# r9y9/gantts

Hardware: AMD Instinct MI355X
Metric: acoustic frames/sec per G+D GAN step (B=32,T=512) (higher is better)
Workload: dtype f32; 1 GPU; cfg2: TTS acoustic MLP G 425-512x3-187 + conditioned MLP D 483-256x3-1, Adagrad, MGE+ADV loss, global B=32 T=512 (32 sequences per GPU, strong scaling), fp32, dropout 0.5 (Philox); global_batch=32, per_gpu_batch=32, parallelism=dp1

## Files before the change

gantts_amd/_lib.py:

```python
import ctypes as C
import os

import torch

_HERE = os.path.dirname(os.path.abspath(__file__))
LIB_PATH = os.environ.get("GT_HIP_LIB") or os.path.join(_HERE, "libgantts_hip.so")

GT_OK, GT_ERR_INVALID, GT_ERR_HIP, GT_ERR_STATE, GT_ERR_DIM = 0, 1, 2, 3, 4
ROLE_G, ROLE_D = 0, 1
OPT_LSTM_PERSISTENT, OPT_LSTM_FWD_UNITS, OPT_LSTM_XCD_LOCAL, OPT_MATMUL_BF16, OPT_SPLIT_FIRST_LAYER, OPT_FUSED_OPTIMIZER = 2, 3, 4, 5, 6, 7
OPT_SIDE_OVERLAP, OPT_LSTM_SIDE, OPT_COMM_D_ONE_MSG, OPT_COMM_EARLY_G, OPT_COMM_GROUP, OPT_COMM_FORCE = 8, 9, 10, 11, 12, 13
OPT_LAUNCH_RIDERS, OPT_COMM_CLOSE_INLINE, OPT_POLL_RESULTS = 14, 15, 16
OPT_COMM_TV_IN_SUMS, OPT_COMM_IPC, OPT_FUSED_DSTACK = 17, 18, 19
IPC_HANDLE_BYTES, IPC_MAX_WORLD = 64, 8
PROFILE_SLOTS = 16
LSTM_PATH_SLOTS, LSTM_PATH_STEPS, LSTM_PATH_DECLINED = 34, 32, 33
GEMM_PATH_SLOTS = 588
GEMM_ROUTE_FORWARD, GEMM_ROUTE_FORWARD_SEG, GEMM_ROUTE_BACKWARD_DATA, GEMM_ROUTE_WEIGHT_GRAD, GEMM_ROUTE_WEIGHT_GRAD_SPLIT = 0, 1, 2, 3, 4
ARCH_MLP, ARCH_IN2OUT, ARCH_LSTM, ARCH_SRU, ARCH_IN2OUT_RNN = 0, 1, 2, 3, 4
OPT_ADAGRAD, OPT_ADAM = 0, 1
MAX_STREAMS = 8
COMM_ID_BYTES = 128


class StreamConfig(C.Structure):
    _fields_ = [("n_streams", C.c_int32),
                ("stream_sizes", C.c_int32 * MAX_STREAMS),
                ("has_dynamic_features", C.c_int32 * MAX_STREAMS),
                ("num_windows", C.c_int32),
                ("adversarial_streams", C.c_int32 * MAX_STREAMS),
                ("mask_nth_mgc_for_adv_loss", C.c_int32),
                ("discriminator_linguistic_condition", C.c_int32),
                ("cond_dim", C.c_int32)]


class ModelDesc(C.Structure):
    _fields_ = [("arch", C.c_int32), ("in_dim", C.c_int32), ("out_dim", C.c_int32),
                ("num_hidden", C.c_int32), ("hidden_dim", C.c_int32), ("static_dim", C.c_int32),
                ("dropout", C.c_float), ("last_sigmoid", C.c_int32),
                ("bidirectional", C.c_int32), ("use_relu", C.c_int32),
                ("rnn_dropout", C.c_float), ("reserved_", C.c_int32),
                ("params", C.c_void_p), ("grads", C.c_void_p), ("n_params", C.c_int64)]


class OptimDesc(C.Structure):
    _fields_ = [("kind", C.c_int32), ("lr", C.c_float), ("weight_decay", C.c_float), ("eps", C.c_float),
                ("lr_decay", C.c_float), ("beta1", C.c_float), ("beta2", C.c_float),
                ("max_grad_norm", C.c_float), ("step", C.c_int64),
                ("state0", C.c_void_p), ("state1", C.c_void_p)]


class DResult(C.Structure):
    _fields_ = [("loss_d", C.c_float), ("loss_fake_d", C.c_float), ("loss_real_d", C.c_float),
                ("real_correct_count", C.c_float), ("fake_correct_count", C.c_float), ("grad_norm", C.c_float)]


class GResult(C.Structure):
    _fields_ = [("loss_mse", C.c_float), ("loss_mge", C.c_float), ("loss_adv", C.c_float),
                ("loss_g", C.c_float), ("grad_norm", C.c_float)]


class GemmCase(C.Structure):
    _fields_ = ([(n, C.c_int32) for n in ("route", "prec", "rows", "in_dim", "out_dim", "act", "drop")] + [("p", C.c_float)]
                + [("key0", C.c_uint32), ("key1", C.c_uint32)]
                + [(n, C.c_int32) for n in ("accumulate", "col0", "ncols", "wrap", "cd", "rider", "defer", "ldx", "ldw", "ldy", "ld_dy",
                                            "ldh", "ld_mask", "ld_addm", "ld_adv", "ld_dx")]
                + [(n, C.c_void_p) for n in ("x", "w", "bias", "y", "dy", "h", "mask", "addm", "adv", "dx", "dw", "db")])

# ... 131 lines not shown
```

gantts_amd/csrc/eng_core.hip:

```cpp
#include "engine_internal.hip.h"

using namespace gt;
static thread_local char g_err[512] = "";
int fail(int code, const char* fmt, ...) {
  va_list ap;
  va_start(ap, fmt);
  vsnprintf(g_err, sizeof(g_err), fmt, ap);
  va_end(ap);
  return code;
}
extern "C" const char* gt_last_error(void) { return g_err; }
extern "C" const char* gt_version(void) { return "gantts_hip 0.1 (gfx950, f32 MFMA)"; }

int ensure_dyn_lds(const void* kernel, size_t bytes) {
  static std::mutex mu;
  static std::map<std::pair<const void*, int>, size_t> done;
  int dev = 0;
  HIPCHK(hipGetDevice(&dev));
  std::lock_guard<std::mutex> lk(mu);
  size_t& cur = done[std::make_pair(kernel, dev)];
  if (bytes > cur) {
    HIPCHK(hipFuncSetAttribute(kernel, hipFuncAttributeMaxDynamicSharedMemorySize, (int)bytes));
    cur = bytes;
  }
  return GT_OK;
}

GemmProfiler g_prof;

extern "C" int gt_profile_enable(int on) {
  g_prof.on = on != 0;
  g_prof.only_kind = on >= 2 ? on - 2 : -1;
  return GT_OK;
}
extern "C" int gt_profile_read(double* out_ms, double* out_flops, int64_t* out_count) {
  for (int v = 0; v < GT_PROFILE_SLOTS; ++v) { out_ms[v] = 0; out_flops[v] = 0; out_count[v] = 0; g_prof.last_bytes[v] = 0; }
  for (auto& r : g_prof.recs) {
    if (hipEventSynchronize(r.e1) != hipSuccess) return fail(GT_ERR_HIP, "hipEventSynchronize failed");
    float ms = 0.f;
    if (hipEventElapsedTime(&ms, r.e0, r.e1) != hipSuccess) return fail(GT_ERR_HIP, "hipEventElapsedTime failed");
    int v = r.kind * 2 + (r.bn == 128 ? 1 : 0);
    if (r.kind == 5) v = 8;
    else if (r.kind == 6) v = 12;
    else if (r.kind == 7) v = 14;
    else if (r.kind == GEMM_NT && r.am == GEMM_A_NONE) v = 6;
    else if (r.kind == GEMM_NT && r.am == GEMM_A_LEAKY_PHILOX) v = 7;
    else if (r.kind == GEMM_NT && r.am == GEMM_A_LEAKY_PHILOX_ADDM) v = 9;
    else if (r.kind == GEMM_NT && r.am == GEMM_A_LEAKY_PHILOX_SEG) v = 13;
    else if (r.kind == GEMM_NN && r.am == GEMM_A_NONE) v = 10;
    else if (r.kind == GEMM_NN && r.am == GEMM_A_LEAKY_PHILOX) v = 11;
    if (v < 0 || v >= GT_PROFILE_SLOTS) v = GT_PROFILE_SLOTS - 1;
    out_ms[v] += ms; out_flops[v] += r.flops; out_count[v] += 1; g_prof.last_bytes[v] += r.bytes;
    g_prof.pool.push_back(r.e0); g_prof.pool.push_back(r.e1);
  }
  g_prof.recs.clear();
  return GT_OK;
}
extern "C" int gt_profile_bytes(double* out_bytes) {
  for (int v = 0; v < GT_PROFILE_SLOTS; ++v) out_bytes[v] = g_prof.last_bytes[v];
  return GT_OK;
}

static int upload_ints(const std::vector<int>& v, int** dptr) {
  if (*dptr) { (void)hipFree(*dptr); *dptr = nullptr; }
  if (v.empty()) return GT_OK;
  HIPCHK(hipMalloc((void**)dptr, v.size() * sizeof(int)));
  HIPCHK(hipMemcpy(*dptr, v.data(), v.size() * sizeof(int), hipMemcpyHostToDevice));
  return GT_OK;
}

extern "C" int gt_engine_create(const gt_stream_config* cfg, gt_engine** out) {
  if (!cfg || !out) return fail(GT_ERR_INVALID, "null argument");
  if (cfg->n_streams < 1 || cfg->n_streams > GT_MAX_STREAMS) return fail(GT_ERR_INVALID, "n_streams out of range");
  if (cfg->num_windows < 1 || cfg->num_windows > MLPG_MAXW) return fail(GT_ERR_INVALID, "num_windows must be in [1,%d]", MLPG_MAXW);
  gt_engine* e = new gt_engine();
  e->cfg = *cfg;
  int col = 0, scol_out = 0;
  std::vector<int> static_start, static_size;
  for (int s = 0; s < cfg->n_streams; ++s) {
    const int sz = cfg->stream_sizes[s];
    const bool dyn = cfg->has_dynamic_features[s] != 0;
    const int ss = dyn ? sz / cfg->num_windows : sz;
    static_start.push_back(scol_out);
    static_size.push_back(ss);
    for (int c = 0; c < ss; ++c) {
      e->h_scol.push_back(col + c);
      e->h_sstride.push_back(dyn ? ss : 0);
    }
    col += sz;
    scol_out += ss;
  }
  e->Dout_cfg = col;
  e->Ds = scol_out;
  if (cfg->adversarial_streams[0] < 0) {
    for (int c = 0; c < e->Ds; ++c) e->h_adv_cols.push_back(c);
  } else {
    for (int s = 0; s < cfg->n_streams; ++s)
      if (cfg->adversarial_streams[s])
        for (int c = 0; c < static_size[s]; ++c) e->h_adv_cols.push_back(static_start[s] + c);
    if (cfg->mask_nth_mgc_for_adv_loss > 0) {
      if ((size_t)cfg->mask_nth_mgc_for_adv_loss >= e->h_adv_cols.size()) { delete e; return fail(GT_ERR_INVALID, "mask_nth_mgc_for_adv_loss too large"); }
      e->h_adv_cols.erase(e->h_adv_cols.begin(), e->h_adv_cols.begin() + cfg->mask_nth_mgc_for_adv_loss);
    }
  }
  e->Da = (int)e->h_adv_cols.size();
  e->h_adv_inv.assign(e->Ds, -1);
  for (int j = 0; j < e->Da; ++j) e->h_adv_inv[e->h_adv_cols[j]] = j;
  int r;
// ... 197 lines not shown
  n.step = od->step;
  n.has_opt = true;
  return GT_OK;
}
extern "C" int gt_set_training(gt_engine* e, int role, int training) {
  if (!e || role < 0 || role > 1) return fail(GT_ERR_INVALID, "bad argument");
  e->net[role].training = training != 0;
  return GT_OK;
}
extern "C" int gt_set_lr(gt_engine* e, int role, float lr) {
  if (!e || role < 0 || role > 1 || !e->net[role].has_opt) return fail(GT_ERR_INVALID, "no optimizer bound");
  e->net[role].od.lr = lr;
  return GT_OK;
}
extern "C" int gt_get_optimizer_step(gt_engine* e, int role, int64_t* step) {
  if (!e || role < 0 || role > 1 || !step) return fail(GT_ERR_INVALID, "bad argument");
  *step = e->net[role].step;
  return GT_OK;
}
extern "C" int gt_set_seed(gt_engine* e, uint64_t seed) {
  if (!e) return fail(GT_ERR_INVALID, "null engine");
  e->seed = seed;
  e->step_counter = 0;
  return GT_OK;
}
extern "C" int gt_set_dropout_mask(gt_engine* e, int role, int pass, int layer, const float* mask) {
  if (!e || role < 0 || role > 1 || pass < 0 || pass > 2 || layer < 0 || layer > 15) return fail(GT_ERR_INVALID, "bad argument");
  e->net[role].inj[pass][layer] = mask;
  return GT_OK;
}
extern "C" int gt_set_option(gt_engine* e, int option, int value) {
  if (!e) return fail(GT_ERR_INVALID, "null engine");
  switch (option) {
    case GT_OPT_LSTM_PERSISTENT: e->lstm_persistent = value != 0; return GT_OK;
    case GT_OPT_LSTM_FWD_UNITS: e->lstm_fwd_upc = value; return GT_OK;
    case GT_OPT_LSTM_XCD_LOCAL: e->lstm_xcd_local = value != 0; return GT_OK;
    case GT_OPT_SPLIT_FIRST_LAYER:
      if (e->opt_split_first != (value != 0)) { e->fake_cat_valid = false; e->adv2_fake_ok = false; }
      e->opt_split_first = value != 0;
      return GT_OK;
    case GT_OPT_FUSED_OPTIMIZER: e->opt_fused_optimizer = value != 0; return GT_OK;
    case GT_OPT_SIDE_OVERLAP: e->opt_side_overlap = value != 0; return GT_OK;
    case GT_OPT_LSTM_SIDE: return value ? fail(GT_ERR_INVALID, "GT_OPT_LSTM_SIDE: removed in round 6 (measured: no gain); the value must be 0") : GT_OK;
    case GT_OPT_COMM_D_ONE_MSG: e->opt_comm_d_one_msg = value != 0; return GT_OK;
    case GT_OPT_COMM_EARLY_G: e->opt_comm_early_g = value != 0; return GT_OK;
    case GT_OPT_COMM_GROUP: e->opt_comm_group = value != 0; return GT_OK;
    case GT_OPT_COMM_FORCE: e->opt_comm_force = value != 0; return GT_OK;
    case GT_OPT_COMM_CLOSE_INLINE: e->opt_comm_close_inline = value != 0; return GT_OK;
    case GT_OPT_COMM_IPC: e->opt_comm_ipc = value != 0; return GT_OK;
    case GT_OPT_FUSED_DSTACK: e->opt_fused_dstack = value < 0 ? 0 : value > 2 ? 2 : value; return GT_OK;
    case GT_OPT_COMM_TV_IN_SUMS: e->opt_comm_tv_in_sums = value != 0; return GT_OK;
    case GT_OPT_POLL_RESULTS: e->opt_poll_results = value != 0; return GT_OK;
    case GT_OPT_LAUNCH_RIDERS: e->opt_launch_riders = value != 0; return GT_OK;
    case GT_OPT_MATMUL_BF16:
      if (e->matmul_bf16 != (value != 0)) {
        e->g_pass_valid = false; e->fake_cat_valid = false; e->dcat_b_ok = false; e->adv2_fake_ok = false; e->leak_pending = false; e->cxd_src = nullptr;
        e->d_begin_done = false; e->g_begin_done = false;
      }
      e->matmul_bf16 = value != 0;
      return GT_OK;
  }
  return fail(GT_ERR_INVALID, "unknown option %d", option);
}
GtTuning& gt_tuning() {
  static GtTuning t = [] {
    GtTuning v;
    auto geti = [](const char* n, int d) { const char* s = getenv(n); return s && s[0] ? atoi(s) : d; };
    v.gemm_pair = geti("GT_GEMM_PAIR", v.gemm_pair); v.pair_order = geti("GT_PAIR_ORDER", v.pair_order);
    { const char* s = getenv("GT_GEMM_TILES"); v.gemm_tiles_big = s && !strcmp(s, "big") ? 1 : 0; }
    v.gemm_unaligned = geti("GT_GEMM_UNALIGNED", v.gemm_unaligned); v.tn_wgs = geti("GT_TN_WGS", v.tn_wgs); v.tn_split_wgs = geti("GT_TN_SPLIT_WGS", v.tn_split_wgs); v.split_fused = geti("GT_SPLIT_FUSED", v.split_fused);
    v.b16_tiles = geti("GT_B16_TILES", v.b16_tiles); v.b16_wg_tile = geti("GT_B16_WG_TILE", v.b16_wg_tile); v.b16_dma = geti("GT_B16_DMA", v.b16_dma);
    v.mlpg_fpl = geti("GT_MLPG_FPL", v.mlpg_fpl); v.mlpg_tt = geti("GT_MLPG_TT", v.mlpg_tt); v.sru_lw = geti("GT_SRU_LW", v.sru_lw); v.sru_cs_waves = geti("GT_SRU_CS_WAVES", v.sru_cs_waves); v.leak_rider = geti("GT_LEAK_RIDER", v.leak_rider);
    v.head_vec = geti("GT_HEAD_VEC", v.head_vec);
    v.mlpg_small16 = geti("GT_MLPG_SMALL16", v.mlpg_small16);
    v.lstm_bt = geti("GT_LSTM_BT", v.lstm_bt);
    if (v.lstm_bt != 8 && v.lstm_bt != 16) v.lstm_bt = 0;
    return v;
  }();
  return t;
}
extern "C" int gt_set_tuning(const char* name, int value) {
  if (!name) return fail(GT_ERR_INVALID, "null name");
  GtTuning& t = gt_tuning();
  struct { const char* n; int* p; } tab[] = {
      {"gemm_pair", &t.gemm_pair}, {"pair_order", &t.pair_order}, {"gemm_tiles_big", &t.gemm_tiles_big}, {"gemm_unaligned", &t.gemm_unaligned},
      {"tn_wgs", &t.tn_wgs}, {"tn_split_wgs", &t.tn_split_wgs}, {"split_fused", &t.split_fused}, {"b16_tiles", &t.b16_tiles},
      {"b16_wg_tile", &t.b16_wg_tile}, {"b16_dma", &t.b16_dma}, {"mlpg_fpl", &t.mlpg_fpl}, {"mlpg_tt", &t.mlpg_tt}, {"sru_lw", &t.sru_lw}, {"sru_cs_waves", &t.sru_cs_waves}, {"leak_rider", &t.leak_rider}, {"head_vec", &t.head_vec}, {"mlpg_small16", &t.mlpg_small16}};
  if (!strcmp(name, "lstm_bt")) {
    if (value != 0 && value != 8 && value != 16) return fail(GT_ERR_INVALID, "lstm_bt must be 0 (by shape), 8 or 16, not %d", value);
    t.lstm_bt = value;
    return GT_OK;
  }
  for (auto& e : tab) if (!strcmp(e.n, name)) { *e.p = value; return GT_OK; }
  return fail(GT_ERR_INVALID, "unknown tuning knob '%s'", name);
}
extern "C" int gt_set_x_pitch(gt_engine* e, int ld_generator_input, int ld_condition) {
  if (!e || ld_generator_input < 0 || ld_condition < 0) return fail(GT_ERR_INVALID, "bad argument");
  e->ld_gx = ld_generator_input; e->ld_cx = ld_condition;
  return GT_OK;
}
extern "C" int gt_set_loss_normalizer(gt_engine* e, float tv) {
  if (!e) return fail(GT_ERR_INVALID, "null engine");
  e->tv_override = tv;
  e->tv_dev = nullptr;
  return GT_OK;
}
// ... 87 lines not shown
    return d;
  }
  return philox_site_spec(e, role, pass, layer, e->step_counter, n.d.dropout, half_rows);
}

extern "C" int gt_op_philox_mask(gt_engine* e, int role, int pass, int layer, int64_t steps_ahead, float p, int64_t rows, int cols,
                                 float* mask, void* stream) {
  if (!e || !mask || role < 0 || role > 1 || pass < 0 || pass > 2 || layer < 0 || layer > 15 || rows < 1 || cols < 1 ||
      steps_ahead < 0 || !(p > 0.f && p < 1.f) || rows > 0x7fffffffL)
    return fail(GT_ERR_INVALID, "bad argument");
  const DropoutSpec d = philox_site_spec(e, role, pass, layer, e->step_counter + (uint64_t)steps_ahead, p,
                                         rows == 2L * e->chk_B * e->chk_T ? (long)e->chk_B * e->chk_T : 0L);
  hipLaunchKernelGGL(philox_mask_kernel, dim3(cdiv(rows * cols, 256)), dim3(256), 0, (hipStream_t)stream, d, rows, cols, mask);
  LAUNCH_CHECK();
  return GT_OK;
}

int fault_seen(gt_engine* e) {
  const unsigned int f = e->h_fault ? (e->h_fault[0] | e->h_fault[1]) : 0u;
  if (f & 0xffu)
    return fail(GT_ERR_HIP, "persistent LSTM kernel fault %u: a workgroup timed out waiting for its peers (results of that "
                "step are invalid and its optimizer updates were skipped; gt_clear_faults() re-arms the engine, "
                "GT_OPT_LSTM_PERSISTENT=0 / GT_LSTM_STEPS=1 selects the per-step kernels)", f);
  if (f) return fail(GT_ERR_HIP, "device fault word 0x%x: results of that step are invalid", f);
  return GT_OK;
}
extern "C" int gt_clear_faults(gt_engine* e, void* stream) {
  if (!e) return fail(GT_ERR_INVALID, "null engine");
  HIPCHK(hipStreamSynchronize((hipStream_t)stream));
  HIPCHK(hipDeviceSynchronize());
  HIPCHK(hipMemset(e->d_fault, 0, 64));
  if (e->opt_bar.p) { HIPCHK(hipMemset(e->opt_bar.p, 0, 64)); e->opt_bar_count = 0; }
  for (int r = 0; r < 2; ++r) { e->net[r].step -= (long)e->h_fault[2 + r]; if (e->net[r].step < 0) e->net[r].step = 0; }
  for (int i = 0; i < 4; ++i) e->h_fault[i] = 0;
  e->g_pass_valid = false; e->leak_pending = false; e->fake_cat_valid = false; e->adv2_fake_ok = false; e->cxd_src = nullptr;
  e->d_begin_done = e->g_begin_done = false; e->early_done = false;
  return GT_OK;
}
extern "C" int gt_lstm_path_counts(gt_engine* e, int64_t* counts, int reset) {
  if (!e) return fail(GT_ERR_INVALID, "null engine");
  if (counts) memcpy(counts, e->lstm_paths, sizeof(e->lstm_paths));
  if (reset) memset(e->lstm_paths, 0, sizeof(e->lstm_paths));
  return GT_OK;
}
extern "C" int gt_check_faults(gt_engine* e, void* stream) {
  if (!e) return fail(GT_ERR_INVALID, "null engine");
  HIPCHK(hipMemcpyAsync(e->h_fault, e->d_fault, sizeof(unsigned int), hipMemcpyDeviceToHost, (hipStream_t)stream));
  HIPCHK(hipStreamSynchronize((hipStream_t)stream));
  return fault_seen(e);
}
int check_common(gt_engine* e, int B, int T) {
  if (!e) return fail(GT_ERR_INVALID, "null engine");
  tl_gemm_prec = e->matmul_bf16 ? PREC_BF16 : PREC_F32;
  if (B < 1 || T < 1) return fail(GT_ERR_INVALID, "B and T must be positive");
  if ((long)B * T > 0x3fffffffL) return fail(GT_ERR_INVALID, "B*T too large");
  e->chk_B = B; e->chk_T = T;
  return GT_OK;
}
```

gantts_amd/csrc/eng_gemm_f32.hip:

```cpp
#include "engine_internal.hip.h"
#include <atomic>

using namespace gt;
int launch_gemm_nt(const GemmArgs& g, int bm, int bn, hipStream_t s);
int launch_gemm_nn(const GemmArgs& g, int bm, int bn, hipStream_t s);
int launch_gemm_tn(const GemmArgs& g, int bm, int bn, int nslab, hipStream_t s);
int launch_gemm_pair(const GemmArgs& nn_in, const GemmArgs& tn_in, int nslab, hipStream_t s);
int launch_gemm_tn_pair(const GemmArgs& g1_in, const GemmArgs& g2_in, int nslab1, int nslab2, hipStream_t s, const GemmArgs* rider, bool* rode);
int gemm_cu_count() {
  static std::map<int, int> cus;
  int dev = 0;
  if (hipGetDevice(&dev) != hipSuccess) return 256;
  auto it = cus.find(dev);
  if (it != cus.end()) return it->second;
  hipDeviceProp_t prop;
  const int n = hipGetDeviceProperties(&prop, dev) == hipSuccess ? prop.multiProcessorCount : 256;
  cus[dev] = n;
  return n;
}
thread_local int tl_gemm_prec = PREC_F32;

static std::atomic<int64_t> g_gemm_paths[GT_GEMM_PATH_SLOTS];
void gemm_path_count(int slot) { g_gemm_paths[slot].fetch_add(1, std::memory_order_relaxed); }
extern "C" int gt_gemm_path_counts(int64_t* counts, int reset) {
  for (int i = 0; i < GT_GEMM_PATH_SLOTS; ++i) {
    const int64_t v = reset ? g_gemm_paths[i].exchange(0, std::memory_order_relaxed) : g_gemm_paths[i].load(std::memory_order_relaxed);
    if (counts) counts[i] = v;
  }
  return GT_OK;
}

static int pick_bn(int N) { return (cdiv(N, 64) * 64 < cdiv(N, 128) * 128) ? 64 : 128; }

static int gemm_tile_mode() { return gt_tuning().gemm_tiles_big; }
static bool gemm_unaligned_ok() { return gt_tuning().gemm_unaligned != 0; }
bool gemm_vec_ok(const float* p, int ld, bool k_contiguous) {
  if (k_contiguous && gemm_unaligned_ok()) return true;
  return (ld % 4 == 0) && (((uintptr_t)p) % 16 == 0);
}
bool gemm_wide_store_ok(int kind, const GemmArgs& g) {
  if (kind == GEMM_TN) return false;
  if (gemm_unaligned_ok()) return true;
  return (g.ldc % 4 == 0) && (((uintptr_t)g.C) % 16 == 0) &&
         (kind != GEMM_NN || g.act == ACT_NONE || ((g.ldh % 4 == 0) && (((uintptr_t)g.H) % 16 == 0)));
}
bool gemm_small_tiles_ok() { return gemm_tile_mode() == 0; }


int launch_gemm(int kind, const GemmArgs& g, int nslab, hipStream_t s) {
  if (g.M <= 0 || g.N <= 0 || g.K <= 0) return fail(GT_ERR_INVALID, "empty GEMM");
  const int bn = pick_bn(g.N);
  const bool vec = gemm_vec_ok(g.A, g.lda, kind != GEMM_TN) && gemm_vec_ok(g.B, g.ldb, kind == GEMM_NT);
  if (kind != GEMM_TN && vec && g.M > 64 && gemm_small_tiles_ok())
    return kind == GEMM_NT ? launch_gemm_nt(g, 64, 64, s) : launch_gemm_nn(g, 64, 64, s);
  bool small = false;
  if (kind != GEMM_TN && g.M > 64) {
    const long t128 = (long)cdiv(g.M, 128) * cdiv(g.N, bn), t64 = (long)cdiv(g.M, 64) * cdiv(g.N, bn);
    const double c128 = (double)cdiv(t128, 512), c64 = 0.55 * (double)cdiv(t64, bn == 64 ? 1024 : 768);
    small = c64 < c128;
  }
  switch (kind) {
    case GEMM_NT:
      if (small) return bn == 64 ? launch_gemm_nt(g, 64, 64, s) : launch_gemm_nt(g, 64, 128, s);
      return bn == 64 ? launch_gemm_nt(g, 128, 64, s) : launch_gemm_nt(g, 128, 128, s);
    case GEMM_NN:
      if (small) return bn == 64 ? launch_gemm_nn(g, 64, 64, s) : launch_gemm_nn(g, 64, 128, s);
      return bn == 64 ? launch_gemm_nn(g, 128, 64, s) : launch_gemm_nn(g, 128, 128, s);
    default:
      if (g.n_tiles_m == 64) return launch_gemm_tn(g, 64, 64, nslab, s);
      return bn == 64 ? launch_gemm_tn(g, 128, 64, nslab, s) : launch_gemm_tn(g, 128, 128, nslab, s);
  }
}

// ... 211 lines not shown
```

gantts_amd/csrc/eng_gemm_f32_pair.hip:

```cpp
#include "gemm_f32_launch.hip.h"

int launch_gemm_pair(const GemmArgs& nn_in, const GemmArgs& tn_in, int nslab, hipStream_t s) {
  GemmArgs nn = nn_in, tn = tn_in;
  nn.wide_store = gemm_wide_store_ok(GEMM_NN, nn) ? 1 : 0;
  tn.wide_store = 0;
  nn.n_tiles_m = cdiv(nn.M, 64); nn.n_tiles_n = cdiv(nn.N, 64);
  tn.n_tiles_m = cdiv(tn.M, 64); tn.n_tiles_n = cdiv(tn.N, 64);
  const int n1 = nn.n_tiles_m * nn.n_tiles_n, n2 = tn.n_tiles_m * tn.n_tiles_n * nslab;
  const bool bf16 = tl_gemm_prec == PREC_BF16;
  const size_t lds = bf16 ? std::max(gemm_lds_bytes<GEMM_NN, 64, 64, PREC_BF16>(), gemm_lds_bytes<GEMM_TN, 64, 64, PREC_BF16>())
                          : std::max(gemm_lds_bytes<GEMM_NN, 64, 64>(), gemm_lds_bytes<GEMM_TN, 64, 64>());
  const int am = bf16 ? GEMM_A_RUNTIME : (nn.act == ACT_NONE ? GEMM_A_NONE : ((nn.act == ACT_LEAKY_DROPOUT && nn.drop.mode == DROP_PHILOX) ? GEMM_A_LEAKY_PHILOX : GEMM_A_RUNTIME));
  const void* kern = bf16 ? (const void*)gemm_pair_kernel<PREC_BF16> : (am == GEMM_A_NONE ? (const void*)gemm_pair_kernel<PREC_F32, GEMM_A_NONE> :
                     (am == GEMM_A_LEAKY_PHILOX ? (const void*)gemm_pair_kernel<PREC_F32, GEMM_A_LEAKY_PHILOX> : (const void*)gemm_pair_kernel<PREC_F32>));
  CHK(ensure_dyn_lds(kern, lds));
  GemmProfiler::Rec rec;
  if (g_prof.wants(5)) {
    rec.kind = 5; rec.bn = 64; rec.am = -1; rec.flops = 2.0 * nn.M * nn.N * nn.K + 2.0 * tn.M * tn.N * tn.K;
    rec.bytes = gemm_algorithmic_bytes(GEMM_NN, nn) + gemm_algorithmic_bytes(GEMM_TN, tn);
    rec.e0 = g_prof.get(); rec.e1 = g_prof.get();
    HIPCHK(hipEventRecord(rec.e0, s));
  }
  const int tn_first = gt_tuning().pair_order;
  const int grid = n1 + n2;
  gemm_path_count(GEMM_PATH_PAIR + (bf16 ? 3 : am == GEMM_A_NONE ? 0 : am == GEMM_A_LEAKY_PHILOX ? 1 : 2));
  if (bf16) hipLaunchKernelGGL(gemm_pair_kernel<PREC_BF16>, dim3(grid), dim3(GEMM_THREADS), lds, s, nn, tn, n1, tn_first);
  else if (am == GEMM_A_NONE) hipLaunchKernelGGL((gemm_pair_kernel<PREC_F32, GEMM_A_NONE>), dim3(grid), dim3(GEMM_THREADS), lds, s, nn, tn, n1, tn_first);
  else if (am == GEMM_A_LEAKY_PHILOX) hipLaunchKernelGGL((gemm_pair_kernel<PREC_F32, GEMM_A_LEAKY_PHILOX>), dim3(grid), dim3(GEMM_THREADS), lds, s, nn, tn, n1, tn_first);
  else      hipLaunchKernelGGL(gemm_pair_kernel<PREC_F32>, dim3(grid), dim3(GEMM_THREADS), lds, s, nn, tn, n1, tn_first);
  LAUNCH_CHECK();
  if (g_prof.wants(5)) { HIPCHK(hipEventRecord(rec.e1, s)); g_prof.recs.push_back(rec); }
  return GT_OK;
}

int launch_gemm_tn_pair(const GemmArgs& g1_in, const GemmArgs& g2_in, int nslab1, int nslab2, hipStream_t s, const GemmArgs* rider, bool* rode) {
  GemmArgs g1 = g1_in, g2 = g2_in, g3;
  memset(&g3, 0, sizeof(g3));
  int n3 = 0;
  if (rode) *rode = false;
  if (rider && rider->act == ACT_NONE && !rider->accumulate && rider->M > 0 && gemm_vec_ok(rider->A, rider->lda, true) && tl_gemm_prec == PREC_F32 &&
      gemm_small_tiles_ok()) {
    g3 = *rider;
    g3.wide_store = gemm_wide_store_ok(GEMM_NN, g3) ? 1 : 0;
    g3.n_tiles_m = cdiv(g3.M, 64); g3.n_tiles_n = cdiv(g3.N, 64);
    n3 = g3.n_tiles_m * g3.n_tiles_n;
    if (rode) *rode = true;
  }
  g1.wide_store = g2.wide_store = 0;
  g1.n_tiles_m = cdiv(g1.M, 64); g1.n_tiles_n = cdiv(g1.N, 64);
  g2.n_tiles_m = cdiv(g2.M, 64); g2.n_tiles_n = cdiv(g2.N, 64);
  const int n1 = g1.n_tiles_m * g1.n_tiles_n * nslab1, n2 = g2.n_tiles_m * g2.n_tiles_n * nslab2;
  const size_t lds = std::max(gemm_lds_bytes<GEMM_TN, 64, 64>(), gemm_lds_bytes<GEMM_NN, 64, 64>());
  CHK(ensure_dyn_lds((const void*)gemm_tn_pair_kernel<PREC_F32>, lds));
  GemmProfiler::Rec rec;
  if (g_prof.wants(6)) {
    rec.kind = 6; rec.bn = 64; rec.am = -1; rec.flops = 2.0 * g1.M * g1.N * g1.K + 2.0 * g2.M * g2.N * g2.K + (n3 ? 2.0 * g3.M * g3.N * g3.K : 0.0);
    rec.bytes = gemm_algorithmic_bytes(GEMM_TN, g1) + 4.0 * (double)g1.M * g1.K + gemm_algorithmic_bytes(GEMM_TN, g2) + (n3 ? gemm_algorithmic_bytes(GEMM_NN, g3) : 0.0);
    rec.e0 = g_prof.get(); rec.e1 = g_prof.get();
    HIPCHK(hipEventRecord(rec.e0, s));
  }
  gemm_path_count(GEMM_PATH_TN_PAIR + (n3 > 0 ? 1 : 0));
  hipLaunchKernelGGL(gemm_tn_pair_kernel<PREC_F32>, dim3(n1 + n2 + n3), dim3(GEMM_THREADS), lds, s, g1, g2, n1, g3, n3);
  LAUNCH_CHECK();
  if (g_prof.wants(6)) { HIPCHK(hipEventRecord(rec.e1, s)); g_prof.recs.push_back(rec); }
  return GT_OK;
}
```

gantts_amd/csrc/eng_step.hip:

```cpp
#include "engine_internal.hip.h"
#include "dstack_f32.hip.h"

using namespace gt;
int ensure_band(gt_engine* e, const float* R, int T, hipStream_t s) {
  MlpgCache& m = e->mlpg;
  ++m.tick;
  for (auto* b : m.entries)
    if (b->R == R && b->T == T) { b->last_use = m.tick; m.cur = b; return GT_OK; }
  const int nW = e->cfg.num_windows;
  CHK(m.tmp.ensure((size_t)(2 * T - 1) * sizeof(float)));
  hipLaunchKernelGGL(mlpg_offset_max_kernel, dim3(2 * T - 1), dim3(256), 0, s, R, T, nW, m.tmp.as<float>());
  LAUNCH_CHECK();
  std::vector<float> off(2 * T - 1);
  HIPCHK(hipMemcpyAsync(off.data(), m.tmp.p, off.size() * sizeof(float), hipMemcpyDeviceToHost, s));
  HIPCHK(hipStreamSynchronize(s));
  float peak = 0.f;
  for (float v : off) peak = fmaxf(peak, v);
  if (!(peak > 0.f) || !isfinite(peak)) return fail(GT_ERR_INVALID, "MLPG matrix R is empty or not finite");
  int kb = 0;
  for (int o = -(T - 1); o <= T - 1; ++o)
    if (off[o + T - 1] > 1e-9f * peak) kb = std::max(kb, abs(o));
  if (kb > 63 || (kb > 48 && kb > T / 4))
    return fail(GT_ERR_INVALID, "MLPG matrix R is not banded (half-width %d of T=%d): only window sets whose "
                "R = (W^T W)^-1 W^T decays (hparams.py:22-26) are supported", kb, T);
// ... 12 lines not shown
  CHK(b->band.ensure((size_t)T * nW * nb * sizeof(float)));
  hipLaunchKernelGGL(mlpg_extract_band_kernel, dim3(cdiv((long)T * nW * nb, 256)), dim3(256), 0, s, R, T, nW, kb, b->band.as<float>());
  LAUNCH_CHECK();
  b->R = R; b->T = T; b->kb = kb; b->last_use = m.tick;
  m.cur = b;
  return GT_OK;
}
extern "C" int gt_invalidate_mlpg_cache(gt_engine* e) {
  if (!e) return fail(GT_ERR_INVALID, "null engine");
  HIPCHK(hipDeviceSynchronize());
  e->mlpg.clear();
  return GT_OK;
}

static int mlpg_tile_frames(gt_engine* e, int B, int T) {
  (void)e;
  const int tt = gt_tuning().mlpg_tt;
  if (tt == 16) return 16;
  if (tt == 0 && gt_tuning().mlpg_small16 && (long)B * cdiv(T, 32) * 2 <= gemm_cu_count()) return 16;
  return 32;
}
int mlpg_forward(gt_engine* e, const float* y, int ldy, const int* scol, const int* sstride, int Ds,
                 float* ys, int ldys, int B, int T, hipStream_t s) {
  const int nW = e->cfg.num_windows, kb = e->mlpg.cur->kb;
  auto lds_of = [&](int tt) { return ((size_t)(tt + 2 * kb) * nW * MLPG_CC + (size_t)tt * nW * (2 * kb + 1 + 2 * MLPG_PAD)) * sizeof(float); };
  const int tt = mlpg_tile_frames(e, B, T);
  const size_t lds = lds_of(tt);
  dim3 grid(B * cdiv(T, tt), cdiv(Ds, MLPG_CC));
  const int fpl = gt_tuning().mlpg_fpl;
#define GT_MLPG_FWD(F, TTV) { CHK(ensure_dyn_lds((const void*)mlpg_forward_kernel<F, TTV>, lds)); \
    hipLaunchKernelGGL((mlpg_forward_kernel<F, TTV>), grid, dim3(MLPG_THREADS), lds, s, y, ldy, e->mlpg.cur->band.as<float>(), kb, nW, scol, sstride, Ds, ys, ldys, B, T); }
  if (tt == 16) GT_MLPG_FWD(2, 16)
  else { if (fpl == 1) GT_MLPG_FWD(1, 32) else if (fpl == 2) GT_MLPG_FWD(2, 32) else GT_MLPG_FWD(4, 32) }
#undef GT_MLPG_FWD
  LAUNCH_CHECK();
  return GT_OK;
}
int mlpg_backward(gt_engine* e, const float* gs, int ldgs, const int* scol, const int* sstride, int Ds,
                  float* gy, int ldgy, int B, int T, float mse_w, const float* yhat, const float* ytgt, int ldt,
                  const float* mask, hipStream_t s) {
  const int nW = e->cfg.num_windows, kb = e->mlpg.cur->kb;
  auto lds_of = [&](int tt) { return ((size_t)(tt + 2 * kb) * MLPG_CC + (size_t)(tt + 2 * kb) * nW * (2 * kb + 1 + 2 * MLPG_PAD)) * sizeof(float); };
  const int tt = mlpg_tile_frames(e, B, T);
  const size_t lds = lds_of(tt);
  dim3 grid(B * cdiv(T, tt), cdiv(Ds, MLPG_CC));
  const int fpl = gt_tuning().mlpg_fpl;
#define GT_MLPG_BWD(F, TTV) { CHK(ensure_dyn_lds((const void*)mlpg_backward_kernel<F, TTV>, lds)); \
    hipLaunchKernelGGL((mlpg_backward_kernel<F, TTV>), grid, dim3(MLPG_THREADS), lds, s, gs, ldgs, e->mlpg.cur->band.as<float>(), kb, nW, scol, sstride, Ds, \
                       gy, ldgy, B, T, mse_w, yhat, ytgt, ldt, mask, e->sc()); }
  if (tt == 16) GT_MLPG_BWD(2, 16)
  else { if (fpl == 1) GT_MLPG_BWD(1, 32) else if (fpl == 2) GT_MLPG_BWD(2, 32) else GT_MLPG_BWD(4, 32) }
#undef GT_MLPG_BWD
  LAUNCH_CHECK();
  return GT_OK;
}

static int stage_injected(gt_engine* e, int role, int layer, const int* passes, int npass, long rows_each, int width,
                          const float** out, hipStream_t s) {
  Net& n = e->net[role];
  *out = nullptr;
  if (!n.training || n.d.dropout <= 0.f) return GT_OK;
  bool any = false, all = true;
  for (int i = 0; i < npass; ++i) { any |= n.inj[passes[i]][layer] != nullptr; all &= n.inj[passes[i]][layer] != nullptr; }
  if (!any) return GT_OK;
  if (!all) return fail(GT_ERR_INVALID, "injected dropout masks must be given for every pass of a step or for none");
  if (npass == 1) { *out = n.inj[passes[0]][layer]; return GT_OK; }
  const size_t per_layer = (size_t)npass * rows_each * width * sizeof(float);
  CHK(e->dmask.ensure(per_layer * n.d.num_hidden));
  float* base = (float*)((char*)e->dmask.p + per_layer * layer);
  for (int i = 0; i < npass; ++i)
    HIPCHK(hipMemcpyAsync(base + (size_t)i * rows_each * width, n.inj[passes[i]][layer], (size_t)rows_each * width * sizeof(float),
                          hipMemcpyDeviceToDevice, s));
  *out = base;
  return GT_OK;
}

struct FirstSplit {
  const float* x; int ldx; int cd;
  const float* xp; int ldxp;
  const float* adv; int ld_adv;
  long wrap;
};
static int pitched_rows(gt_engine* e, int slot, const float* p, int ld, int cols, long rows, const float** out, int* ldo, hipStream_t s) {
  if (gemm_vec_ok(p, ld)) { *out = p; *ldo = ld; return GT_OK; }
  gt_engine::Pitched& P = e->pitched[slot];
  const int ldp = (cols + 3) & ~3;
  if (!(P.src == p && P.ld == ld && P.cols == cols && P.rows == rows && P.step == e->step_counter)) {
    CHK(P.buf.ensure((size_t)rows * ldp * sizeof(float)));
    hipLaunchKernelGGL(repitch_kernel, dim3(cdiv(rows * (ldp / 4), 256)), dim3(256), 0, s, p, ld, cols, rows, P.buf.as<float>(), ldp);
    LAUNCH_CHECK();
    P.src = p; P.ld = ld; P.cols = cols; P.rows = rows; P.step = e->step_counter;
  }
  *out = P.buf.as<float>(); *ldo = ldp;
  return GT_OK;
}

static int stack_forward(gt_engine* e, int role, const float* in, int ld_in, long rows, std::vector<Scratch>& acts,
                         const int* passes, int npass, long rows_each, std::vector<DropoutSpec>& specs, hipStream_t s,
                         const FirstSplit* fs = nullptr, int max_layers = 1 << 30 ) {
  Net& n = e->net[role];
  specs.resize(n.hidden.size());
  const float* cur = in;
  int ld = ld_in;
  for (size_t l = 0; l < n.hidden.size(); ++l) {
    const Lin& L = n.hidden[l];
    CHK(acts[l].ensure((size_t)rows * L.out * sizeof(float)));
// ... 277 lines not shown
      hipLaunchKernelGGL(gather_cols_kernel, dim3(cdiv(N * G.d.out_dim, 256)), dim3(256), 0, s, y_hat, G.d.out_dim, 0,
                         (const int*)nullptr, y_hat_static, G.d.out_dim, 0, (int)N, G.d.out_dim);
      LAUNCH_CHECK();
    }
  }
  return GT_OK;
}

extern "C" int gt_apply_generator(gt_engine* e, const float* x, const float* R, int B, int T, float* y_hat,
                                  float* y_hat_static, void* stream) {
  CHK(check_common(e, B, T));
  Net& G = e->net[GT_ROLE_G];
  if (!G.bound) return fail(GT_ERR_STATE, "generator not bound");
  if (!x || !y_hat || !y_hat_static) return fail(GT_ERR_INVALID, "null tensor");
  hipStream_t s = (hipStream_t)stream;
  CHK(fault_seen(e));
  e->step_counter++;
  e->B = B; e->T = T; e->N = (long)B * T;
  e->g_pass_valid = false;
  e->fake_cat_valid = false; e->dcat_b_ok = false; e->adv2_fake_ok = false; e->cxd_src = nullptr;
  e->tv_mask = nullptr; e->tv_inflight = false;
  CHK(generator_forward(e, x, R, B, T, y_hat, y_hat_static, true, s, e->g_specs));
  e->last_x = e->gx_dense_on ? e->gx_dense.as<float>() : x;
  e->last_yhat = y_hat; e->last_yhs = y_hat_static;
  e->g_pass_valid = true;
  return GT_OK;
}

int cond_dim(gt_engine* e) {
  if (!e->cfg.discriminator_linguistic_condition) return 0;
  if (e->cfg.cond_dim > 0) return e->cfg.cond_dim;
  return e->net[GT_ROLE_D].bound ? e->net[GT_ROLE_D].d.in_dim - e->Da : 0;
}
static int d_in_dim(gt_engine* e) { return e->Da + cond_dim(e); }

static int build_cat(gt_engine* e, const float* x, const float* feats, int ld_feats, long row0, long N, int ldc, hipStream_t s) {
  float* dst = e->dcat.as<float>() + row0 * ldc;
  int off = 0;
  if (e->cfg.discriminator_linguistic_condition) {
    if (!x) return fail(GT_ERR_INVALID, "discriminator_linguistic_condition is set but x is null");
    const int cd = cond_dim(e);
    if (cd <= 0) return fail(GT_ERR_DIM, "discriminator in_dim too small for linguistic conditioning");
    hipLaunchKernelGGL(gather_cols_kernel, dim3(cdiv(N * cd, 256)), dim3(256), 0, s, x, cd, 0, (const int*)nullptr, dst, ldc, 0,
                       (int)N, cd);
    LAUNCH_CHECK();
    off = cd;
  }
  hipLaunchKernelGGL(gather_cols_kernel, dim3(cdiv(N * e->Da, 256)), dim3(256), 0, s, feats, ld_feats, 0, e->d_adv_cols, dst, ldc,
                     off, (int)N, e->Da);
  LAUNCH_CHECK();
  return GT_OK;
}

static int head_finalize(gt_engine* e, int mode, int nblk, int K, bool w, hipStream_t s, StepResults* early_res, int* defer_scalars, unsigned ticket) {
  Net& D = e->net[GT_ROLE_D];
  if (defer_scalars && !w) { *defer_scalars = nblk; return GT_OK; }
  const int cgw = (w && nblk >= 512) ? 16 : 64;
  const int n_dw = cdiv(K, cgw), extra = cgw == 16 ? 1 : 0;
  hipLaunchKernelGGL(d_head_finalize_kernel, dim3(n_dw + extra), dim3(1024), 0, s, e->headp.as<HeadPartials>(), e->headw.as<float>(),
                     nblk, K, mode, e->sc(), w ? D.last.dW : (float*)nullptr, w ? D.last.db : (float*)nullptr, D.grads_dirty ? 1 : 0,
                     early_res, ticket ? e->ticket_dev() : (unsigned*)nullptr, ticket, cgw, extra ? n_dw : 0);
  LAUNCH_CHECK();
  return GT_OK;
}

static bool d_fused_ok(gt_engine* e, bool b16, long rows) {
  Net& D = e->net[GT_ROLE_D];
  if (e->opt_fused_dstack < 2 && dstack_panels(rows) < gemm_cu_count()) return false;
  if (!e->opt_fused_dstack || b16 || D.d.arch != GT_ARCH_MLP || tl_gemm_prec != PREC_F32 || !dstack_hidden_ok(D.d.hidden_dim)) return false;
  if (D.hidden.empty() || (int)D.hidden.size() > DS_MAXL || D.last.out != 1 || e->Da < 1 || e->Da > 64) return false;
  for (size_t l = 0; l < D.hidden.size(); ++l)
    if (D.hidden[l].out != D.d.hidden_dim || (l > 0 && D.hidden[l].in != D.d.hidden_dim)) return false;
  return true;
}
static int run_dstack(gt_engine* e, int mode, long rows, long n_real, const float* mask, long n_mask, float eps, bool want_grad,
                      float* gadv, hipStream_t s, StepResults* early_res, int* defer_scalars, const double* tv_dev, unsigned ticket, bool unit_tv) {
  Net& D = e->net[GT_ROLE_D];
  const int H = D.d.hidden_dim, L = (int)D.hidden.size();
  const int nblk = dstack_panels(rows);
  CHK(e->headp.ensure((size_t)nblk * sizeof(HeadPartials)));
  CHK(e->dout.ensure((size_t)rows * sizeof(float)));
  DStackArgs a;
  memset(&a, 0, sizeof(a));
  a.mode = mode; a.L = L; a.rows = (int)rows; a.n_real = (int)n_real;
  a.H0 = e->d_act[0].as<float>();
  for (int l = 0; l < L; ++l) {
    a.W[l] = D.hidden[l].W; a.b[l] = D.hidden[l].b; a.drop[l] = e->d_specs[l];
    if (a.drop[l].mode == DROP_BUFFER && a.drop[l].ld_mask != H) return fail(GT_ERR_INVALID, "injected dropout mask pitch");
  }
  a.w_last = D.last.W; a.b_last = D.last.b; a.mask = mask; a.n_mask = (int)n_mask; a.eps = eps; a.unit_tv = unit_tv ? 1 : 0; a.tv_dev = tv_dev;
  a.sc = e->sc(); a.want_grad = want_grad ? 1 : 0; a.Dout = e->dout.as<float>(); a.hp = e->headp.as<HeadPartials>();
  if (mode == DSTACK_D_STEP) {
    for (int l = 1; l + 1 < L; ++l) a.Hout[l] = e->d_act[l].as<float>();
    a.dZtop = e->dzA.as<float>();
    if (want_grad) { CHK(e->headw.ensure((size_t)nblk * H * sizeof(float))); a.dw_partial = e->headw.as<float>(); }
  } else {
    a.W0 = D.hidden[0].W; a.ldw0 = D.hidden[0].in; a.col0 = cond_dim(e); a.Da = e->Da; a.gadv = gadv; a.ld_gadv = e->Da;
    if (want_grad && !gadv) return fail(GT_ERR_INVALID, "fused discriminator stack: no gradient buffer");
  }
  CHK(launch_dstack(a, H, s));
  return head_finalize(e, mode == DSTACK_D_STEP ? HEAD_D_STEP : HEAD_G_ADV, nblk, H, mode == DSTACK_D_STEP && want_grad, s, early_res, defer_scalars, ticket);
}

static int run_head(gt_engine* e, int mode, const void* H, int K, long n_rows, long n_real, const float* mask, long n_mask,
                    float eps, bool want_grad, float* dH, const DropoutSpec& spec, bool want_w, hipStream_t s,
                    StepResults* early_res = nullptr, int h_ld = 0, B16Img* dz_img = nullptr, bool dz_t = false,
                    int* defer_scalars = nullptr ,
                    const double* tv_dev = nullptr ,
                    unsigned ticket = 0 ,
                    bool unit_tv = false ,
                    bool has_act = true ) {
// ... 276 lines not shown
  CHK(e->dzA.ensure((size_t)2 * N * std::max(H, 1) * sizeof(float)));
  CHK(e->dzB.ensure((size_t)2 * N * std::max(H, 1) * sizeof(float)));
  const bool plain_early = e->early && !comm_on(e), comm_early = e->early && comm_on(e);
  if (tv_side) CHK(side_join(e, s));
  const unsigned d_ticket = plain_early ? take_ticket(e) : 0;
  const double* head_tv = nullptr;
  if (unnorm) {
    e->tv_mask = mask; e->tv_n = N; e->tv_ovr = e->tv_override;
  } else if (comm_on(e) && e->opt_launch_riders && e->tv_inflight && !tv_known) {
    CHK(comm_tv_join(e, s));
    head_tv = e->comm_tv.as<double>();
    e->tv_mask = mask; e->tv_n = N; e->tv_ovr = e->tv_override;
  } else CHK(ensure_tv(e, mask, N, s));
  if (b16 && tr) CHK(e->dz_b[0].ensure(2 * N, H, true));
  if (d_rec)
    CHK(run_head(e, HEAD_D_STEP, (const void*)rec_top, H, 2 * N, N, mask, N, eps, tr, e->dl_dout.as<float>(), no_drop(), true, s,
                 plain_early ? early_res_target(e) : nullptr, 0, nullptr, true, nullptr, head_tv, d_ticket, unnorm, false));
  else if (fused)
    CHK(run_dstack(e, DSTACK_D_STEP, 2 * N, N, mask, N, eps, tr, nullptr, s, plain_early ? early_res_target(e) : nullptr, nullptr, head_tv, d_ticket, unnorm));
  else
  CHK(run_head(e, HEAD_D_STEP, b16 ? (const void*)e->d_actb.back().r() : (const void*)e->d_act.back().as<float>(), H, 2 * N, N, mask, N, eps, tr,
               e->dzA.as<float>(), e->d_specs.back(), true, s, plain_early ? early_res_target(e) : nullptr, b16 ? e->d_actb.back().ld : 0,
               (b16 && tr) ? &e->dz_b[0] : nullptr, true, nullptr, head_tv, d_ticket, unnorm));
  e->early_done = false;
  if (plain_early) CHK(post_early_results(e, s, d_ticket));
  if (comm_early) CHK(comm_early_results(e, GT_ROLE_D, unnorm ? &e->sc()->tv_sum : &e->sc()->s_real, unnorm ? 5 : 4, 0.f, 0.f, 0.f, s));
  if (tr) {
    CHK(comm_grads_ready(e, GT_ROLE_D, D.last.dW, (long)D.last.in * D.last.out + D.last.out, s));
    Net& G = e->net[GT_ROLE_G];
    const bool want_leak = G.bound && G.d.grads && e->g_pass_valid && y_hat_static == e->last_yhs && e->N == N;
    if (want_leak && e->leak_pending)
      return fail(GT_ERR_STATE, "update_discriminator called twice without optimizer_g.zero_grad() (train.py:538)");
    float* leak = nullptr;
    if (want_leak) { CHK(e->leak.ensure((size_t)N * e->Da * sizeof(float))); leak = e->leak.as<float>(); }
    const int col0 = cond_dim(e);
    if (d_rec) {
      float* dx0 = nullptr;
      if (leak) { CHK(e->d_dx0.ensure((size_t)2 * N * K0 * sizeof(float))); dx0 = e->d_dx0.as<float>(); }
      CHK(lstm_stack_backward(e, GT_ROLE_D, e->dcat.as<float>(), ldc, 2 * B, T, passes, 2, true, dx0, s));
      if (leak) {
        hipLaunchKernelGGL(gather_cols_kernel, dim3(cdiv(N * e->Da, 256)), dim3(256), 0, s, dx0 + N * K0, K0, col0, (const int*)nullptr, leak, e->Da, 0,
                           (int)N, e->Da);
        LAUNCH_CHECK();
      }
    } else if (b16) {
      CHK(stack_backward_b16(e, GT_ROLE_D, e->dcat_b.t(), e->dcat_b.ldt, 2 * N, e->d_actb, e->d_specs, 0, true, leak, e->Da, col0, e->Da, N, N, s));
    } else {
      CHK(stack_backward(e, GT_ROLE_D, split ? nullptr : e->dcat.as<float>(), ldc, 2 * N, e->d_act, e->d_specs, e->dzA.as<float>(),
                         e->dzB.as<float>(), true, leak, e->Da, col0, e->Da, N, N, s, split ? &fs : nullptr));
    }
    D.grads_dirty = true;
    if (want_leak) { e->leak_pending = true; e->leak_unnorm = unnorm; }
  }
  CHK(comm_finish_step(e, GT_ROLE_D, tr, &e->sc()->s_real, comm_early ? 0 : 4, s));
  e->d_begin_done = true;
  return GT_OK;
}

static void fill_d_result(const StepResults* h, gt_d_result* out) {
  out->loss_d = h->loss_d; out->loss_fake_d = h->loss_fake_d; out->loss_real_d = h->loss_real_d;
  out->real_correct_count = h->real_correct; out->fake_correct_count = h->fake_correct;
  out->grad_norm = h->gnorm_d;
}
static void fill_g_result(const StepResults* h, gt_g_result* out) {
  out->loss_mse = h->loss_mse; out->loss_mge = h->loss_mge; out->loss_adv = h->loss_adv;
  out->loss_g = h->loss_g; out->grad_norm = h->gnorm_g;
}

extern "C" int gt_update_discriminator_end(gt_engine* e, int train, gt_d_result* out, void* stream) {
  if (!e) return fail(GT_ERR_INVALID, "null argument");
  if (!e->d_begin_done) return fail(GT_ERR_STATE, "gt_update_discriminator_end without _begin");
  hipStream_t s = (hipStream_t)stream;
  e->d_begin_done = false;
  if (!out) {
    if (e->early_done) return fail(GT_ERR_STATE, "deferred results are a split-phase feature");
    if (train) CHK(optimizer_step(e, GT_ROLE_D, &e->sc()->gnorm2_d, s));
    hipLaunchKernelGGL(finalize_d_kernel, dim3(1), dim3(1), 0, s, e->sc(), e->res(), train ? 0 : 1);
    LAUNCH_CHECK();
    return post_deferred_results(e, GT_ROLE_D, s);
  }
  if (e->early_done) {
    if (train) CHK(optimizer_step(e, GT_ROLE_D, &e->sc()->gnorm2_d, s));
    CHK(wait_early_results(e));
    e->early_done = false;
  } else {
    if (train) CHK(optimizer_step(e, GT_ROLE_D, &e->sc()->gnorm2_d, s));
    hipLaunchKernelGGL(finalize_d_kernel, dim3(1), dim3(1), 0, s, e->sc(), e->res(), train ? 0 : 1);
    LAUNCH_CHECK();
    CHK(fetch_results(e, s));
  }
  fill_d_result(e->h_res, out);
  return GT_OK;
}
extern "C" int gt_update_discriminator_result(gt_engine* e, gt_d_result* out) {
  if (!e || !out) return fail(GT_ERR_INVALID, "null argument");
  if (!e->def_pending[GT_ROLE_D]) return fail(GT_ERR_STATE, "no deferred discriminator result pending");
  HIPCHK(hipEventSynchronize(e->ev_def[GT_ROLE_D]));
  e->def_pending[GT_ROLE_D] = false;
  fill_d_result(e->h_def[GT_ROLE_D], out);
  return GT_OK;
}

extern "C" int gt_update_discriminator(gt_engine* e, const float* x, const float* y_static, const float* y_hat_static,
                                       const float* mask, int B, int T, int train, float eps, gt_d_result* out, void* stream) {
  if (!e) return fail(GT_ERR_INVALID, "null engine");
  e->early = true;
  int r = gt_update_discriminator_begin(e, x, y_static, y_hat_static, mask, B, T, train, eps, stream);
  e->early = false;
  if (r != GT_OK) { e->early_done = false; e->d_unnorm = false; e->ticket_wait = 0; return r; }
  return gt_update_discriminator_end(e, train, out, stream);
}

static int sum_sqerr(gt_engine* e, const float* a, int lda, const float* b, int ldb, const float* mask, long rows, int D,
                     double* out, float* g, int ldg, float gscale, hipStream_t s, int* deferred_blocks = nullptr) {
  const int nblk = (int)std::min<long>(1024, cdiv(rows * D, RED_THREADS * 4));
  CHK(e->partial.ensure(4096 * sizeof(double)));
  double* part = e->partial.as<double>() + 1024;
  hipLaunchKernelGGL(masked_sqerr_kernel, dim3(nblk), dim3(RED_THREADS), 0, s, a, lda, b, ldb, mask, rows, D, part, g, ldg, gscale, e->sc());
  LAUNCH_CHECK();
  if (deferred_blocks) { *deferred_blocks = nblk; return GT_OK; }
  hipLaunchKernelGGL(sum_partials_kernel, dim3(1), dim3(256), 0, s, part, nblk, out);
  LAUNCH_CHECK();
  return GT_OK;
}

static int generator_backward(gt_engine* e, const float* x, const float* y, const float* y_hat, const float* mask,
                              float mse_w, hipStream_t s) {
  Net& G = e->net[GT_ROLE_G];
  const long N = e->N;
  const int B = e->B, T = e->T, Do = G.d.out_dim;
  const bool mlp_body = !(has_lstm_body(G.d.arch) || G.d.arch == GT_ARCH_SRU);
  const int ldgy = mlp_body && (is_i2o(G.d.arch) || e->g_used_mlpg) ? (Do + 3) & ~3 : Do;
  CHK(e->gy.ensure((size_t)N * ldgy * sizeof(float)));
  float* gy = e->gy.as<float>();
  const float* gs = e->gs.as<float>();
  if (is_i2o(G.d.arch)) {
    const int sd = G.d.static_dim;
    if (G.d.arch == GT_ARCH_IN2OUT_RNN) mse_w = 0.f;
    CHK(e->dgx.ensure((size_t)N * sd * sizeof(float)));
    CHK(e->dtz.ensure((size_t)N * sd * sizeof(float)));
    hipLaunchKernelGGL(highway_backward_kernel, dim3(cdiv(N * sd, 256)), dim3(256), 0, s, gs, sd, e->tx.as<float>(), sd,
                       e->gx.as<float>(), sd, e->dgx.as<float>(), sd, e->dtz.as<float>(), sd, N, sd);
    LAUNCH_CHECK();
    CHK(linear_backward_weight(e->dtz.as<float>(), sd, x, G.d.in_dim, N, sd, sd, G.gate.dW, G.gate.db, G.grads_dirty, e->slabs,
                               e->colp, s, &e->sdefer[GT_ROLE_G]));
    CHK(comm_grads_ready(e, GT_ROLE_G, G.gate.dW, (long)sd * sd + sd, s));
    CHK(mlpg_backward(e, e->dgx.as<float>(), sd, e->d_scol_i2o, e->d_sstride_i2o, sd, gy, ldgy, B, T, mse_w, y_hat, y, Do, mask, s));
  } else if (e->g_used_mlpg) {
    CHK(mlpg_backward(e, gs, e->Ds, e->d_scol, e->d_sstride, e->Ds, gy, ldgy, B, T, mse_w, y_hat, y, Do, mask, s));
  } else {
    if (mse_w != 0.f) CHK(sum_sqerr(e, y_hat, Do, y, Do, mask, N, Do, &e->sc()->s_mse, gy, Do, mse_w, s));
    hipLaunchKernelGGL(slab_reduce_kernel, dim3(cdiv(N * Do, 256)), dim3(256), 0, s, gs, 0L, 1, N * Do, gy, mse_w != 0.f ? 1 : 0);
    LAUNCH_CHECK();
  }
  if (G.d.last_sigmoid && !is_i2o(G.d.arch)) {
    hipLaunchKernelGGL(sigmoid_grad_kernel, dim3(cdiv(N * Do, 256)), dim3(256), 0, s, gy, ldgy, y_hat, Do, N, Do);
    LAUNCH_CHECK();
  }
  if (has_lstm_body(G.d.arch) || G.d.arch == GT_ARCH_SRU) {
    CHK(has_lstm_body(G.d.arch) ? lstm_backward(e, x, gy, B, T, s) : sru_backward(e, x, gy, B, T, s));
    G.grads_dirty = true;
    return GT_OK;
  }
  if (use_b16(e, GT_ROLE_G)) {
    const int H = G.d.hidden_dim;
    CHK(e->gy_b.ensure(N, Do, true));
    CHK(cast_transpose(gy, ldgy, N, Do, e->gy_b.r(), e->gy_b.ld, e->gy_b.t(), e->gy_b.ldt, nullptr, false, &e->colp, s));
    B16Img& top = e->g_actb.back();
    CHK(weight_grad_b16(e->gy_b.t(), e->gy_b.ldt, top.t(), top.ldt, N, Do, G.last.in, G.last.dW, G.last.db, G.grads_dirty, e->slabs, s,
                        &e->sdefer[GT_ROLE_G]));
    CHK(comm_grads_ready(e, GT_ROLE_G, G.last.dW, (long)Do * G.last.in + Do, s));
    const LinShadow& ws = e->wsh[GT_ROLE_G][G.hidden.size()];
    CHK(e->dz_b[0].ensure(N, H, true));
    GemmB16Args g = b16_args();
    g.A = e->gy_b.r(); g.lda = e->gy_b.ld; g.B = ws.wt.as<__bf16>(); g.ldb = ws.ldwt; g.M = (int)N; g.N = H; g.K = Do;
    g.epi = B16_BWD_DATA; g.act = ACT_LEAKY_DROPOUT; g.H = top.r(); g.ldh = top.ld; g.drop = e->g_specs.back();
    g.Cb = e->dz_b[0].r(); g.ldcb = e->dz_b[0].ld; g.CbT = e->dz_b[0].t(); g.ldcbt = (int)e->dz_b[0].ldt;
    CHK(launch_gemm_b16(g, 1, s));
    CHK(stack_backward_b16(e, GT_ROLE_G, e->xin_b.t(), e->xin_b.ldt, N, e->g_actb, e->g_specs, 0, true, nullptr, 0, 0, 0, 0, 0, s));
    G.grads_dirty = true;
    return GT_OK;
  }
  const Lin& Lt = G.hidden.back();
  const int H = G.d.hidden_dim;
  CHK(e->dzA.ensure((size_t)2 * N * H * sizeof(float)));
  CHK(e->dzB.ensure((size_t)2 * N * H * sizeof(float)));
  const GemmArgs nn_last = backward_data_args(gy, ldgy, G.last.W, G.last.in, 0, e->dzA.as<float>(), H, N, Do, H, ACT_LEAKY_DROPOUT,
                                              e->g_act.back().as<float>(), H, e->g_specs.back());
  bool rode = false;
  CHK(linear_backward_weight(gy, ldgy, e->g_act.back().as<float>(), Lt.out, N, Do, G.last.in, G.last.dW, G.last.db, G.grads_dirty,
                             e->slabs, e->colp, s, &e->sdefer[GT_ROLE_G], &nn_last, &rode));
  CHK(comm_grads_ready(e, GT_ROLE_G, G.last.dW, (long)Do * G.last.in + Do, s));
  if (!rode) CHK(launch_gemm(GEMM_NN, nn_last, 1, s));
  const float* xin = x;
  int ldxin = gx_pitch(e);
  if (!gemm_vec_ok(x, ldxin) && tl_gemm_prec == PREC_F32) {
    if (e->fake_cat_valid && e->fake_cat_x == x && e->cfg.discriminator_linguistic_condition && cond_dim(e) == G.d.in_dim && e->dcat.p) {
      ldxin = (d_in_dim(e) + 3) & ~3;
      xin = e->dcat.as<float>() + N * ldxin;
    } else {
      const int slot = (e->pitched[0].src == x && e->pitched[0].ld == gx_pitch(e) && e->pitched[0].cols == G.d.in_dim && e->pitched[0].step == e->step_counter) ? 0 : 1;
      CHK(pitched_rows(e, slot, x, gx_pitch(e), G.d.in_dim, N, &xin, &ldxin, s));
    }
  }
  CHK(stack_backward(e, GT_ROLE_G, xin, ldxin, N, e->g_act, e->g_specs, e->dzA.as<float>(), e->dzB.as<float>(), true,
                     nullptr, 0, 0, 0, 0, 0, s));
  G.grads_dirty = true;
  return GT_OK;
}

extern "C" int gt_update_generator_begin(gt_engine* e, const float* x, const float* y, const float* y_hat, const float* y_static,
                                         const float* y_hat_static, float adv_w, const float* mask, int B, int T, int train,
                                         float mse_w, float mge_w, float eps, void* stream) {
  CHK(check_common(e, B, T));
  Net& G = e->net[GT_ROLE_G];
  Net& D = e->net[GT_ROLE_D];
  if (!G.bound) return fail(GT_ERR_STATE, "generator not bound");
  if (!y || !y_hat || !y_static || !y_hat_static || !mask) return fail(GT_ERR_INVALID, "null tensor");
  hipStream_t s = (hipStream_t)stream;
  const long N = (long)B * T;
  const bool tr = train != 0;
  if (tr) {
    if (!e->g_pass_valid || y_hat != e->last_yhat || y_hat_static != e->last_yhs || N != e->N)
      return fail(GT_ERR_STATE, "update_generator(phase=\"train\") needs the y_hat / y_hat_static returned by the last apply_generator");
    if (!G.d.grads) return fail(GT_ERR_STATE, "phase == \"train\" but the generator was bound without grads");
  }
  const int Do = G.d.out_dim;
  const int Ds = is_i2o(G.d.arch) ? G.d.static_dim : e->Ds;
  if (comm_on(e) && tr && G.grads_dirty)
    return fail(GT_ERR_STATE, "data-parallel step: optimizer_g.zero_grad() must precede update_generator");
  { SlabDefer& sd = e->sdefer[GT_ROLE_G]; sd.jobs.n = 0; sd.blocks = 0; sd.used = 0; sd.active = e->early && tr && G.has_opt; }
  CHK(ensure_tv(e, mask, N, s));
  const bool direct = !is_i2o(G.d.arch) && !e->g_used_mlpg;
  const bool early_fold = e->early && !comm_on(e) && !(tr && direct && mse_w != 0.f);
  int mse_blocks = 0, mge_pre_blocks = 0;
  const bool mse_side = early_fold && e->opt_side_overlap && adv_w > 0.f;
  const bool riders = early_fold && e->opt_launch_riders && !mse_side;
  const bool riders_dp = e->early && comm_on(e) && e->opt_launch_riders && !(tr && direct && mse_w != 0.f);
  if (riders || riders_dp) {
    mse_blocks = (int)std::min<long>(1024, cdiv(N * Do, RED_THREADS * 4));
    mge_pre_blocks = (int)std::min<long>(1024, cdiv(N * Ds, RED_THREADS * 4));
    CHK(e->partial.ensure(4096 * sizeof(double)));
    hipLaunchKernelGGL(g_losses_kernel, dim3(mse_blocks + mge_pre_blocks), dim3(RED_THREADS), 0, s, y_hat, Do, y, Do, Do, mse_blocks,
                       e->partial.as<double>() + 1024, y_hat_static, Ds, y_static, Ds, Ds, e->partial.as<double>(), mask, N);
    LAUNCH_CHECK();
  } else if (!(tr && direct && mse_w != 0.f)) {
    if (mse_side) CHK(side_fork(e, s));
    CHK(sum_sqerr(e, y_hat, Do, y, Do, mask, N, Do, &e->sc()->s_mse, nullptr, 0, 0.f, mse_side ? e->side : s, early_fold ? &mse_blocks : nullptr));
  }
  e->g_has_adv = adv_w > 0.f;
  float* gadv = nullptr;
  int head_blocks = 0;
  if (adv_w > 0.f) {
    if (!D.bound) return fail(GT_ERR_STATE, "adv_w > 0 but no discriminator bound");
    if (D.d.in_dim != d_in_dim(e)) return fail(GT_ERR_DIM, "discriminator in_dim mismatch");
    const int K0 = D.d.in_dim, ldc = (K0 + 3) & ~3;
    const int passes[1] = {2};
    const bool b16 = use_b16(e, GT_ROLE_D);
    const float* cat = nullptr;
    const bool split = d_split_ok(e, x, b16);
    if (!split) CHK(dense_cx(e, &x, N, s));
    FirstSplit fs;
    memset(&fs, 0, sizeof(fs));
    if (split) {
      e->ld_adv2 = (e->Da + 3) & ~3;
      CHK(e->adv2.ensure((size_t)2 * N * e->ld_adv2 * sizeof(float)));
      float* fake = e->adv2.as<float>() + N * e->ld_adv2;
      if (!(e->adv2_fake_ok && e->adv2_yhs == y_hat_static)) {
        hipLaunchKernelGGL(build_adv_kernel, dim3(cdiv(N * (e->ld_adv2 / 4), 256)), dim3(256), 0, s, y_hat_static, y_hat_static, Ds, e->d_adv_cols, e->Da,
                           fake, e->ld_adv2, N, N, (const float*)nullptr, 0, 0.f, (StepScalars*)nullptr, (double*)nullptr);
        LAUNCH_CHECK();
        e->adv2_fake_ok = true; e->adv2_yhs = y_hat_static;
      }
      fs.x = x; fs.ldx = cx_pitch(e); fs.cd = cond_dim(e); fs.adv = fake; fs.ld_adv = e->ld_adv2; fs.wrap = N;
    } else if (!b16) {
      CHK(e->dcat.ensure((size_t)2 * N * ldc * sizeof(float)));
      if (!(e->fake_cat_valid && e->fake_cat_x == x && e->fake_cat_yhs == y_hat_static)) {
        CHK(build_cat(e, x, y_hat_static, Ds, N, N, ldc, s));
        e->fake_cat_valid = true; e->fake_cat_x = x; e->fake_cat_yhs = y_hat_static;
      }
      cat = e->dcat.as<float>() + N * ldc;
    }
    const bool d_rec = has_lstm_body(D.d.arch);
    const bool fused = !d_rec && d_fused_ok(e, b16, N);
    const float* rec_top = nullptr;
    int rec_ld = 0;
    if (d_rec) {
      CHK(lstm_check_lengths(e, B, T));
      CHK(lstm_stack_forward(e, GT_ROLE_D, cat, ldc, B, T, passes, 1, s, &rec_top, &rec_ld));
    } else
    if (b16) {
      CHK(e->dcat_b.ensure(2 * N, K0, false));
      if (!(e->dcat_b_ok && e->dcat_b_x == x && e->dcat_b_yhs == y_hat_static)) {
        if (e->cfg.discriminator_linguistic_condition && (!x || cond_dim(e) <= 0))
          return fail(GT_ERR_INVALID, "discriminator_linguistic_condition is set but x is null");
        CatSrc src;
        src.x = x; src.cd = cond_dim(e); src.fa = y_hat_static; src.fb = y_hat_static; src.ldf = Ds; src.idx = e->d_adv_cols; src.N = N; src.row_off = N;
        hipLaunchKernelGGL(cat_cast_transpose_kernel, dim3(cdiv(N, 64), cdiv(K0, 64)), dim3(256), 0, s, src, N, K0,
                           e->dcat_b.r() + N * e->dcat_b.ld, e->dcat_b.ld, (__bf16*)nullptr, 0L);
        LAUNCH_CHECK();
        e->dcat_b_ok = true; e->dcat_b_x = x; e->dcat_b_yhs = y_hat_static;
      }
      CHK(refresh_shadows(e, GT_ROLE_D, false, s));
      CHK(stack_forward_b16(e, GT_ROLE_D, e->dcat_b.r() + N * e->dcat_b.ld, e->dcat_b.ld, N, e->d_actb, passes, 1, N, e->d_specs, false, s));
    } else {
      CHK(stack_forward(e, GT_ROLE_D, cat, ldc, N, e->d_act, passes, 1, N, e->d_specs, s, split ? &fs : nullptr, fused ? 1 : 1 << 30));
    }
    const int H = d_rec ? rec_ld : D.d.hidden_dim;
    CHK(e->dzA.ensure((size_t)2 * N * H * sizeof(float)));
    CHK(e->dzB.ensure((size_t)2 * N * H * sizeof(float)));
    if (b16 && tr) CHK(e->dz_b[0].ensure(N, H, false));
    if (fused) {
      if (tr) { CHK(e->gadv.ensure((size_t)N * e->Da * sizeof(float))); gadv = e->gadv.as<float>(); }
      CHK(run_dstack(e, DSTACK_G_ADV, N, N, mask, N, eps, tr, gadv, s, nullptr, riders || riders_dp ? &head_blocks : nullptr, nullptr, 0, false));
    } else
    if (d_rec) {
      CHK(e->dl_dout.ensure((size_t)2 * N * H * sizeof(float)));
      CHK(run_head(e, HEAD_G_ADV, (const void*)rec_top, H, N, N, mask, N, eps, tr, e->dl_dout.as<float>(), no_drop(), false, s, nullptr, 0, nullptr,
                   false, riders || riders_dp ? &head_blocks : nullptr, nullptr, 0, false, false));
    } else
    CHK(run_head(e, HEAD_G_ADV, b16 ? (const void*)e->d_actb.back().r() : (const void*)e->d_act.back().as<float>(), H, N, N, mask, N, eps, tr,
                 e->dzA.as<float>(), e->d_specs.back(), false, s, nullptr, b16 ? e->d_actb.back().ld : 0, (b16 && tr) ? &e->dz_b[0] : nullptr, false,
                 riders || riders_dp ? &head_blocks : nullptr));
    if (tr && !fused) {
      CHK(e->gadv.ensure((size_t)N * e->Da * sizeof(float)));
      gadv = e->gadv.as<float>();
      const int col0 = cond_dim(e);
      if (d_rec) {
        CHK(e->d_dx0.ensure((size_t)2 * N * K0 * sizeof(float)));
        float* dx0 = e->d_dx0.as<float>();
        CHK(lstm_stack_backward(e, GT_ROLE_D, cat, ldc, B, T, passes, 1, false, dx0, s));
        hipLaunchKernelGGL(gather_cols_kernel, dim3(cdiv(N * e->Da, 256)), dim3(256), 0, s, dx0, K0, col0, (const int*)nullptr, gadv, e->Da, 0, (int)N,
                           e->Da);
        LAUNCH_CHECK();
      } else if (b16) {
        CHK(stack_backward_b16(e, GT_ROLE_D, nullptr, 0, N, e->d_actb, e->d_specs, 0, false, gadv, e->Da, col0, e->Da, 0, N, s));
      } else {
        CHK(stack_backward(e, GT_ROLE_D, cat, ldc, N, e->d_act, e->d_specs, e->dzA.as<float>(), e->dzB.as<float>(), false, gadv,
                           e->Da, col0, e->Da, 0, N, s));
      }
    }
  }
  const bool early_ok = e->early && !(tr && direct && mse_w != 0.f);
  const bool early_now = early_ok && !comm_on(e), comm_early = early_ok && comm_on(e) && e->opt_comm_early_g;
  int mge_blocks = 0;
  e->early_done = false;
  {
    const int nblk = (int)std::min<long>(1024, cdiv(N * Ds, RED_THREADS * 4));
    CHK(e->partial.ensure(4096 * sizeof(double)));
    float* gs = nullptr;
    if (tr) { CHK(e->gs.ensure((size_t)N * Ds * sizeof(float))); gs = e->gs.as<float>(); }
    const float* leak = (tr && e->leak_pending) ? e->leak.as<float>() : nullptr;
    GFinalize fin;
    memset(&fin, 0, sizeof(fin));
    const bool rid = riders || riders_dp;
    if (rid) {
      fin.on = 1; fin.sc = e->sc(); fin.out = riders ? early_res_target(e) : (StepResults*)nullptr; fin.adv_w = adv_w; fin.mse_w = mse_w; fin.mge_w = mge_w;
      fin.has_adv = e->g_has_adv ? 1 : 0;
      fin.part_mge = e->partial.as<double>(); fin.n_mge = mge_pre_blocks;
      fin.part_mse = e->partial.as<double>() + 1024; fin.n_mse = mse_blocks;
      fin.hp = head_blocks ? e->headp.as<HeadPartials>() : (const HeadPartials*)nullptr; fin.n_hp = head_blocks;
      if (riders) { fin.ticket_value = take_ticket(e); fin.ticket = fin.ticket_value ? e->ticket_dev() : (unsigned*)nullptr; }
    }
    if (tr || !rid)
      hipLaunchKernelGGL(static_grad_kernel, dim3(nblk + (rid ? 1 : 0)), dim3(RED_THREADS), 0, s, y_hat_static, Ds,
                         y_static, Ds, mask, N, Ds, mge_w, e->d_adv_inv, leak, e->Da, gadv, e->Da, adv_w, gs, Ds,
                         rid ? (double*)nullptr : e->partial.as<double>(), e->sc(), fin, leak && e->leak_unnorm ? 1 : 0);
    else
      hipLaunchKernelGGL(finalize_g_rider_kernel, dim3(1), dim3(RED_THREADS), 0, s, fin);
    LAUNCH_CHECK();
    mge_blocks = nblk;
    if (riders) CHK(post_early_results(e, s, fin.ticket_value));
    else if (!early_now && !riders_dp) {
      hipLaunchKernelGGL(sum_partials_kernel, dim3(1), dim3(256), 0, s, e->partial.as<double>(), nblk, &e->sc()->s_mge);
      LAUNCH_CHECK();
    }
  }
  if (mse_side && mse_blocks) CHK(side_join(e, s));
  if (early_now && !riders) {
    hipLaunchKernelGGL(finalize_g_kernel, dim3(1), dim3(256), 0, s, e->sc(), early_res_target(e), adv_w, mse_w, mge_w, e->g_has_adv ? 1 : 0, 1,
                       (const double*)e->partial.as<double>(), mge_blocks,
                       mse_blocks ? (const double*)(e->partial.as<double>() + 1024) : (const double*)nullptr, mse_blocks);
    LAUNCH_CHECK();
    CHK(post_early_results(e, s));
  }
  if (comm_early) CHK(comm_early_results(e, GT_ROLE_G, &e->sc()->s_adv, 3, adv_w, mse_w, mge_w, s));
  if (tr) {
    CHK(generator_backward(e, e->last_x, y, y_hat, mask, mse_w, s));
    e->leak_pending = false; e->leak_unnorm = false;
  }
  CHK(comm_finish_step(e, GT_ROLE_G, tr, &e->sc()->s_adv, comm_early ? 0 : 3, s));
  e->g_begin_done = true;
  return GT_OK;
}

extern "C" int gt_update_generator_end(gt_engine* e, int train, float adv_w, float mse_w, float mge_w, gt_g_result* out,
                                       void* stream) {
  if (!e) return fail(GT_ERR_INVALID, "null argument");
  if (!e->g_begin_done) return fail(GT_ERR_STATE, "gt_update_generator_end without _begin");
  hipStream_t s = (hipStream_t)stream;
  e->g_begin_done = false;
  if (!out) {
    if (e->early_done) return fail(GT_ERR_STATE, "deferred results are a split-phase feature");
    if (train) CHK(optimizer_step(e, GT_ROLE_G, &e->sc()->gnorm2_g, s));
    hipLaunchKernelGGL(finalize_g_kernel, dim3(1), dim3(1), 0, s, e->sc(), e->res(), adv_w, mse_w, mge_w, e->g_has_adv ? 1 : 0,
                       train ? 0 : 1, (const double*)nullptr, 0, (const double*)nullptr, 0);
    LAUNCH_CHECK();
    return post_deferred_results(e, GT_ROLE_G, s);
  }
  if (e->early_done) {
    if (train) CHK(optimizer_step(e, GT_ROLE_G, &e->sc()->gnorm2_g, s));
    CHK(wait_early_results(e));
    e->early_done = false;
  } else {
    if (train) CHK(optimizer_step(e, GT_ROLE_G, &e->sc()->gnorm2_g, s));
    hipLaunchKernelGGL(finalize_g_kernel, dim3(1), dim3(1), 0, s, e->sc(), e->res(), adv_w, mse_w, mge_w, e->g_has_adv ? 1 : 0,
                       train ? 0 : 1, (const double*)nullptr, 0, (const double*)nullptr, 0);
    LAUNCH_CHECK();
    CHK(fetch_results(e, s));
  }
  fill_g_result(e->h_res, out);
  return fault_seen(e);
}
extern "C" int gt_update_generator_result(gt_engine* e, gt_g_result* out) {
  if (!e || !out) return fail(GT_ERR_INVALID, "null argument");
  if (!e->def_pending[GT_ROLE_G]) return fail(GT_ERR_STATE, "no deferred generator result pending");
  HIPCHK(hipEventSynchronize(e->ev_def[GT_ROLE_G]));
  e->def_pending[GT_ROLE_G] = false;
  fill_g_result(e->h_def[GT_ROLE_G], out);
  return GT_OK;
}

extern "C" int gt_update_generator(gt_engine* e, const float* x, const float* y, const float* y_hat, const float* y_static,
                                   const float* y_hat_static, float adv_w, const float* mask, int B, int T, int train,
                                   float mse_w, float mge_w, float eps, gt_g_result* out, void* stream) {
  if (!e) return fail(GT_ERR_INVALID, "null engine");
  e->early = true;
  int r = gt_update_generator_begin(e, x, y, y_hat, y_static, y_hat_static, adv_w, mask, B, T, train, mse_w, mge_w, eps, stream);
  e->early = false;
  if (r != GT_OK) { e->early_done = false; return r; }
  return gt_update_generator_end(e, train, adv_w, mse_w, mge_w, out, stream);
}

extern "C" int gt_flush_generator_grads(gt_engine* e, void* stream) {
  if (!e) return fail(GT_ERR_INVALID, "null engine");
  Net& G = e->net[GT_ROLE_G];
  if (!G.bound || !G.d.grads || !e->g_pass_valid) return fail(GT_ERR_STATE, "no generator pass to back-propagate");
  hipStream_t s = (hipStream_t)stream;
  tl_gemm_prec = e->matmul_bf16 ? PREC_BF16 : PREC_F32;
  CHK(fault_seen(e));
  { SlabDefer& sd = e->sdefer[GT_ROLE_G]; sd.active = false; sd.jobs.n = 0; sd.blocks = 0; sd.used = 0; }
  const long N = e->N;
  const int Ds = is_i2o(G.d.arch) ? G.d.static_dim : e->Ds;
  CHK(e->gs.ensure((size_t)N * Ds * sizeof(float)));
  HIPCHK(hipMemsetAsync(e->gs.p, 0, (size_t)N * Ds * sizeof(float), s));
  if (e->leak_pending) {
    std::vector<int>& cols = e->h_adv_cols;
    for (int j = 0; j < e->Da; ++j) {
      hipLaunchKernelGGL(gather_cols_kernel, dim3(cdiv(N, 256)), dim3(256), 0, s, e->leak.as<float>(), e->Da, j, (const int*)nullptr,
                         e->gs.as<float>(), Ds, cols[j], (int)N, 1);
    }
    if (e->leak_unnorm) hipLaunchKernelGGL(scale_by_inv_tv_kernel, dim3(cdiv(N * Ds, 256)), dim3(256), 0, s, e->gs.as<float>(), N * Ds, e->sc());
    LAUNCH_CHECK();
  }
  CHK(generator_backward(e, e->last_x, e->last_yhat, e->last_yhat, (const float*)nullptr, 0.f, s));
  e->leak_pending = false; e->leak_unnorm = false;
  HIPCHK(hipStreamSynchronize(s));
  return GT_OK;
}

extern "C" int gt_model_forward(gt_engine* e, int role, const float* x, const float* R, int B, int T, float* out, float* out2,
                                void* stream) {
  CHK(check_common(e, B, T));
  if (role < 0 || role > 1 || !e->net[role].bound) return fail(GT_ERR_STATE, "model not bound");
  if (!x || !out) return fail(GT_ERR_INVALID, "null tensor");
  hipStream_t s = (hipStream_t)stream;
  Net& n = e->net[role];
  const long N = (long)B * T;
  e->step_counter++;
  std::vector<DropoutSpec> specs;
  if (role == GT_ROLE_G && is_i2o(n.d.arch)) {
    if (!out2) return fail(GT_ERR_INVALID, "In2OutHighwayNet forward returns two tensors");
    e->g_pass_valid = false;
    return generator_forward(e, x, R, B, T, out, out2, false, s, specs);
  }
  const int pass0d[1] = {0};
  if (n.d.arch == GT_ARCH_LSTM || n.d.arch == GT_ARCH_SRU) {
    if (role != GT_ROLE_G) {
      if (n.d.arch != GT_ARCH_LSTM) return fail(GT_ERR_INVALID, "the discriminator slot takes MLP and LSTMRNN networks");
      CHK(lstm_check_lengths(e, B, T));
      const float* top = nullptr;
      int ld = 0;
      CHK(lstm_stack_forward(e, role, x, n.d.in_dim, B, T, pass0d, 1, s, &top, &ld));
      return linear_forward(top, ld, n.last.W, n.last.in, n.last.b, out, n.d.out_dim, N, n.last.in, n.last.out,
                            n.d.last_sigmoid ? ACT_SIGMOID : ACT_NONE, no_drop(), s);
    }
    e->g_pass_valid = false;
    return n.d.arch == GT_ARCH_LSTM ? lstm_forward(e, x, B, T, out, s) : sru_forward(e, x, B, T, out, s);
  }
  const int pass0[1] = {0};
  auto& acts = role == GT_ROLE_G ? e->g_act : e->d_act;
  if (role == GT_ROLE_G) e->g_pass_valid = false;
// ... 19 lines not shown
```

gantts_amd/csrc/engine_internal.hip.h:

```cpp
#pragma once
#include <hip/hip_runtime.h>
#include <math.h>
#include <stdarg.h>
#include <stdio.h>
#include <stdlib.h>
#include <string.h>
#include <algorithm>
#include <map>
#include <mutex>
#include <string>
#include <vector>

#pragma GCC visibility push(default)
#include "../../include/gantts_hip.h"
#pragma GCC visibility pop
#include "frame_kernels.hip.h"
#include "gemm_f32.hip.h"
#include "gemm_bf16s.hip.h"

using namespace gt;

int fail(int code, const char* fmt, ...);
#define HIPCHK(expr)                                                                         \
  do {                                                                                       \
    hipError_t _e = (expr);                                                                  \
    if (_e != hipSuccess)                                                                    \
      return fail(GT_ERR_HIP, "%s failed: %s (%s:%d)", #expr, hipGetErrorString(_e), __FILE__, __LINE__); \
  } while (0)
#define CHK(expr)            \
  do {                       \
    int _r = (expr);         \
    if (_r != GT_OK) return _r; \
  } while (0)
#define LAUNCH_CHECK() HIPCHK(hipGetLastError())

static inline bool env_flag(const char* name, bool dflt) { const char* v = getenv(name); return v && v[0] ? v[0] != '0' : dflt; }
static inline int cdiv(long a, long b) { return (int)((a + b - 1) / b); }
static inline int pad8(long n) { return (int)((n + 7) & ~7L); }

int ensure_dyn_lds(const void* kernel, size_t bytes);
int gemm_cu_count();

struct GtTuning {
  int gemm_pair = 1;
  int pair_order = 1;
  int gemm_tiles_big = 0;
  int gemm_unaligned = 1;
  int tn_wgs = 512;
  int split_fused = 1;
  int tn_split_wgs = 1024;
  int b16_tiles = 0;
  int b16_wg_tile = 0;
  int b16_dma = 1;
  int mlpg_fpl = 2;
  int head_vec = 0;
  int mlpg_small16 = 0;
  int mlpg_tt = 0;
  int leak_rider = 1;
  int sru_cs_waves = 0;
  int sru_lw = 2;
  int lstm_bt = 0;
};
GtTuning& gt_tuning();

struct GemmProfiler {
  bool on = false;
  int only_kind = -1;
  bool wants(int kind) const { return on && (only_kind < 0 || only_kind == kind); }
  struct Rec { int kind, bn, am; double flops, bytes; hipEvent_t e0, e1; };
  double last_bytes[GT_PROFILE_SLOTS] = {};
  std::vector<Rec> recs;
  std::vector<hipEvent_t> pool;
  hipEvent_t get() {
    if (!pool.empty()) { hipEvent_t e = pool.back(); pool.pop_back(); return e; }
    hipEvent_t e; (void)hipEventCreate(&e); return e;
  }
};
extern GemmProfiler g_prof;

struct Scratch {
  void* p = nullptr;
  size_t bytes = 0;
  int ensure(size_t need) {
    if (need <= bytes) return GT_OK;
    if (p) { HIPCHK(hipDeviceSynchronize()); HIPCHK(hipFree(p)); p = nullptr; bytes = 0; }
    const size_t cap = need + need / 8;
    HIPCHK(hipMalloc(&p, cap));
    bytes = cap;
    return GT_OK;
  }
  void release() { if (p) { (void)hipFree(p); p = nullptr; bytes = 0; } }
  template <typename T> T* as() const { return (T*)p; }
};

struct SlabDefer {
  Scratch pool;
  size_t used = 0;
  SlabJobs jobs;
  int blocks = 0;
  bool active = false;
  SlabDefer() { jobs.n = 0; jobs.pad_ = 0; }
};

struct Lin { float *W, *b, *dW, *db; int in, out; };
struct B16Img {
  Scratch rm, tr;
  int ld = 0; long ldt = 0;
  __bf16* r() { return rm.as<__bf16>(); }
  __bf16* t() { return tr.as<__bf16>(); }
  int ensure(long rows, int cols, bool want_t) {
    ld = pad8(cols); ldt = pad8(rows);
    CHK(rm.ensure((size_t)rows * ld * 2 + 64));
    if (want_t) CHK(tr.ensure((size_t)cols * ldt * 2 + 64));
    return GT_OK;
  }
  void release() { rm.release(); tr.release(); }
};
struct LinShadow { Scratch w, wt; int ldw = 0, ldwt = 0; };
static inline bool is_i2o(int arch) { return arch == GT_ARCH_IN2OUT || arch == GT_ARCH_IN2OUT_RNN; }
static inline bool has_lstm_body(int arch) { return arch == GT_ARCH_LSTM || arch == GT_ARCH_IN2OUT_RNN; }
struct LstmDirP { float *Wih, *Whh, *bih, *bhh, *dWih, *dWhh, *dbih, *dbhh; };
struct LstmLayerP { int in; LstmDirP d[2]; };
struct SruLayerP { int in, k; float *W, *b, *dW, *db; };

struct Net {
  bool bound = false;
  gt_model_desc d;
  std::vector<Lin> hidden;
  Lin last, gate;
  std::vector<LstmLayerP> lstm;
  std::vector<SruLayerP> sru;
// ... 47 lines not shown
  bool early = false, early_done = false;
  hipEvent_t ev_res = nullptr;
  unsigned ticket_next = 0, ticket_wait = 0;
  unsigned* ticket_dev() { return h_res_dev ? (unsigned*)((char*)h_res_dev + 64) : nullptr; }
  volatile unsigned* ticket_host() { return (volatile unsigned*)((char*)h_res + 64); }
  StepResults* h_def[2] = {nullptr, nullptr}; hipEvent_t ev_def[2] = {nullptr, nullptr}; bool def_pending[2] = {false, false};
  std::vector<DropoutSpec> g_specs, d_specs;
  std::vector<Scratch> l_xproj, l_gates, l_cst, l_out, l_outd;
  Scratch i2o_gout;
  Scratch l_state, l_dout, l_hshift;
  std::vector<Scratch> dl_xproj, dl_gates, dl_cst, dl_out, dl_outd;
  Scratch dl_dout, dl_hshift, d_dx0;
  Scratch l_xch;
  struct GtComm* comm = nullptr;
  struct GtIpc* ipc = nullptr;
  bool opt_comm_ipc = env_flag("GT_COMM_IPC", true);
  int dp_rank = 0, dp_world = 1;
  int chk_B = 0, chk_T = 0;
  std::vector<std::pair<long, long>> comm_done[2];
  std::vector<std::pair<long, long>> comm_pending[2];
  Scratch comm_tv;
  bool tv_inflight = false;
  std::vector<B16Img> g_actb, d_actb;
  B16Img xin_b, dcat_b, gy_b, dz_b[2], fwd_b;
  std::vector<B16Img> l_in_b;
  std::vector<B16Img> s_in_b;
  B16Img s_du_b;
  std::vector<LinShadow> ssh;
  std::vector<B16Img> l_dg_b;
  B16Img l_hs_b;
  hipStream_t side = nullptr;
  hipEvent_t ev_side_go = nullptr, ev_side_done = nullptr;
  std::vector<LinShadow> lsh;
  bool dcat_b_ok = false;
  const float* dcat_b_x = nullptr; const float* dcat_b_yhs = nullptr;
  std::vector<LinShadow> wsh[2];
  SlabDefer sdefer[2];
  Scratch d_pre;
  Scratch adv2; int ld_adv2 = 0;
  bool adv2_fake_ok = false; const float* adv2_yhs = nullptr;
  struct Pitched { Scratch buf; const float* src = nullptr; int ld = 0, cols = 0; long rows = 0; uint64_t step = ~0ULL; };
  Pitched pitched[2];
  int opt_fused_dstack = getenv("GT_FUSED_DSTACK") ? atoi(getenv("GT_FUSED_DSTACK")) : 1;
  bool opt_split_first = env_flag("GT_D_SPLIT", true);
  bool opt_fused_optimizer = env_flag("GT_OPT_FUSED", false);
  bool opt_side_overlap = env_flag("GT_SIDE_OVERLAP", false);
  bool opt_comm_d_one_msg = env_flag("GT_COMM_D_ONE_MSG", true), opt_comm_early_g = env_flag("GT_COMM_EARLY_G", true),
       opt_comm_group = env_flag("GT_COMM_GROUP", false), opt_comm_force = getenv("GT_COMM_FORCE_COLLECTIVES") != nullptr;
  bool opt_comm_close_inline = env_flag("GT_COMM_CLOSE_INLINE", true);
  bool opt_comm_tv_in_sums = env_flag("GT_COMM_TV_IN_SUMS", true);
  bool d_unnorm = false, leak_unnorm = false;
  bool opt_poll_results = env_flag("GT_POLL_RESULTS", true);
  bool opt_launch_riders = env_flag("GT_LAUNCH_RIDERS", true);
  int ld_gx = 0, ld_cx = 0;
  Scratch gx_dense, cx_dense;
  bool gx_dense_on = false;
  const float* cxd_src = nullptr; uint64_t cxd_step = ~0ull; long cxd_rows = 0; int cxd_ld = 0, cxd_cols = 0;
  Scratch opt_bar; unsigned long long opt_bar_count = 0;
  Scratch w0pad[2];
  unsigned int* h_fault_dev = nullptr;
  unsigned int* d_fault = nullptr;
  unsigned int* h_fault = nullptr;
  bool lstm_persistent = getenv("GT_LSTM_STEPS") == nullptr;
  int lstm_fwd_upc = 0;
  bool lstm_xcd_local = getenv("GT_LSTM_NO_XCD_LOCAL") == nullptr;
  int64_t lstm_paths[GT_LSTM_PATH_SLOTS] = {};
  bool matmul_bf16 = false;
  static constexpr int LEN_RING = 4;
  int* len_host[LEN_RING] = {nullptr, nullptr, nullptr, nullptr};
  Scratch len_dev[LEN_RING];
  hipEvent_t len_ev[LEN_RING] = {nullptr, nullptr, nullptr, nullptr};
  int len_cap = 0, len_slot = -1;
  int* d_lengths() { return len_slot < 0 ? nullptr : len_dev[len_slot].as<int>(); }
  std::vector<Scratch> s_wt;
  std::vector<Scratch> s_u, s_h, s_c, s_xdrop, s_xmask;
  Scratch s_du, s_dx, s_dbias;
  std::vector<int> h_lengths;
  StepScalars* sc() { return scal.as<StepScalars>(); }
  StepResults* res() { return (StepResults*)((char*)scal.p + 256); }
};


int check_common(gt_engine* e, int B, int T);
int fault_seen(gt_engine* e);
gt::DropoutSpec philox_site_spec(gt_engine* e, int role, int pass, int layer, uint64_t step, float p, long half_rows = 0);
gt::DropoutSpec drop_spec(gt_engine* e, int role, int pass, int layer, const float* stacked_mask, int ld, long half_rows = 0);

extern thread_local int tl_gemm_prec;
enum { GEMM_PATH_PAIR = 576, GEMM_PATH_TN_PAIR = 580, GEMM_PATH_REDUCE4 = 582, GEMM_PATH_REDUCE = 583, GEMM_PATH_REDUCE_SMALL = 584,
       GEMM_PATH_COLSUM_PARTIAL = 585, GEMM_PATH_COLSUM_FINALIZE = 586, GEMM_PATH_REDUCE_MULTI = 587 };
static_assert(GEMM_PATH_REDUCE_MULTI + 1 == GT_GEMM_PATH_SLOTS, "gt_gemm_path_counts slots");
constexpr int gemm_path_slot(int kind, int bm, int bn, bool va, bool vb, int prec, int amode) {
  return (((((kind * 2 + (bm == 128)) * 2 + (bn == 128)) * 2 + va) * 2 + vb) * 2 + (prec == gt::PREC_BF16)) * 6 + (amode + 1);
}
void gemm_path_count(int slot);
bool gemm_vec_ok(const float* p, int ld, bool k_contiguous = false);
bool gemm_wide_store_ok(int kind, const gt::GemmArgs& g);
bool gemm_small_tiles_ok();
namespace gt { struct DStackArgs; }
bool dstack_hidden_ok(int hidden_dim);
int dstack_panels(long rows);
int launch_dstack(const gt::DStackArgs& a, int hidden_dim, hipStream_t s);
gt::DropoutSpec no_drop();
int launch_gemm(int kind, const gt::GemmArgs& g, int nslab, hipStream_t s);
int linear_forward(const float* X, int ldx, const float* W, int ldw, const float* b, float* Y, int ldy,
                   long rows, int in, int out, int act, const gt::DropoutSpec& drop, hipStream_t s);
gt::GemmArgs backward_data_args(const float* dZ, int lddz, const float* W, int ldw, int col0, float* dX, int lddx,
                                long rows, int out, int ncols, int act_prev, const float* H, int ldh, const gt::DropoutSpec& drop);
int linear_backward_data(const float* dZ, int lddz, const float* W, int ldw, int col0, float* dX, int lddx,
                         long rows, int out, int ncols, int act_prev, const float* H, int ldh, const gt::DropoutSpec& drop, hipStream_t s);
int slab_defer_flush(SlabDefer& d, hipStream_t s);
int linear_backward_weight(const float* dZ, int lddz, const float* X, int ldx, long rows, int out, int in,
                           float* dW, float* db, bool accumulate, Scratch& slabs, Scratch& colp, hipStream_t s,
                           SlabDefer* defer = nullptr, const gt::GemmArgs* ride_along = nullptr, bool* rode = nullptr);

int linear_backward_weight_split(const float* dZ, int lddz, long rows, long wrap, const float* xp, int ldxp, int cd,
                                 const float* adv, int ld_adv, int Da, int out, float* dW, float* db, bool accumulate,
                                 Scratch& slabs, hipStream_t s, SlabDefer* defer, const GemmArgs* rider = nullptr, bool* rode = nullptr);

gt::GemmB16Args b16_args();
int launch_gemm_b16(const gt::GemmB16Args& g, int nslab, hipStream_t s, int tile = 0);
int cast_transpose(const float* in, int ld_in, long rows, int cols, __bf16* out, int ldo, __bf16* outT, long ldt,
                   float* colsum, bool colsum_accumulate, Scratch* colp, hipStream_t s);
int cast_transpose(const __bf16* in, int ld_in, long rows, int cols, __bf16* out, int ldo, __bf16* outT, long ldt,
                   float* colsum, bool colsum_accumulate, Scratch* colp, hipStream_t s);
int weight_grad_b16(const __bf16* dZT, long lddzt, const __bf16* XT, long ldxt, long rows, int out, int in, float* dW, float* db,
                    bool accumulate, Scratch& slabs, hipStream_t s, SlabDefer* defer = nullptr);

int ensure_band(gt_engine* e, const float* R, int T, hipStream_t s);
int mlpg_forward(gt_engine* e, const float* y, int ldy, const int* scol, const int* sstride, int Ds,
                 float* ys, int ldys, int B, int T, hipStream_t s);
int mlpg_backward(gt_engine* e, const float* gs, int ldgs, const int* scol, const int* sstride, int Ds,
                  float* gy, int ldgy, int B, int T, float mse_w, const float* yhat, const float* ytgt, int ldt,
                  const float* mask, hipStream_t s);
int post_early_results(gt_engine* e, hipStream_t s, unsigned ticket = 0);
int cond_dim(gt_engine* e);

struct GtComm {
  void* comm = nullptr;
  int rank = 0, world = 1;
  hipStream_t stream = nullptr;
// ... 31 lines not shown
```

gantts_amd/csrc/frame_kernels.hip.h:

```cpp
#pragma once
#include <hip/hip_runtime.h>
#include <stdint.h>
#include "gemm_f32.hip.h"

namespace gt {

constexpr int RED_THREADS = 256;

__device__ __forceinline__ float wave_sum(float v) {
#pragma unroll
  for (int o = 32; o > 0; o >>= 1) v += __shfl_xor(v, o, 64);
  return v;
}
__device__ __forceinline__ double wave_sum_d(double v) {
#pragma unroll
  for (int o = 32; o > 0; o >>= 1) v += __shfl_xor(v, o, 64);
  return v;
}
__device__ __forceinline__ float block_sum(float v, float* sh) {
  v = wave_sum(v);
  const int lane = threadIdx.x & 63, w = threadIdx.x >> 6;
  __syncthreads();
  if (lane == 0) sh[w] = v;
  __syncthreads();
  float r = 0.f;
  if (threadIdx.x == 0) for (int i = 0; i < (int)(blockDim.x >> 6); ++i) r += sh[i];
  return r;
}
__device__ __forceinline__ double block_sum_d(double v, double* sh) {
  v = wave_sum_d(v);
  const int lane = threadIdx.x & 63, w = threadIdx.x >> 6;
  __syncthreads();
  if (lane == 0) sh[w] = v;
  __syncthreads();
  double r = 0.0;
  if (threadIdx.x == 0) for (int i = 0; i < (int)(blockDim.x >> 6); ++i) r += sh[i];
  return r;
}

__device__ __forceinline__ bool dropout_keep(const DropoutSpec& d, int row, int col) {
  if (d.mode == DROP_PHILOX) return philox_keep_spec(d, row, col);
  if (d.mode == DROP_BUFFER) return d.mask[(long)row * d.ld_mask + col] != 0.f;
  return true;
}

static __global__ void philox_mask_kernel(const DropoutSpec d, long rows, int cols, float* __restrict__ mask) {
  const long e = (long)blockIdx.x * blockDim.x + threadIdx.x;
  if (e >= rows * cols) return;
  const int r = (int)(e / cols), c = (int)(e - (long)r * cols);
  mask[e] = philox_keep_spec(d, r, c) ? 1.f : 0.f;
}

struct StepScalars {
  float tv;
  float inv_tv;
  double tv_sum;
  double s_real, s_fake;
  double n_real_ok, n_fake_ok;
  double s_adv;
  double s_mge, s_mse;
  double gnorm2_d, gnorm2_g;
};
struct StepResults {
  float loss_d, loss_fake_d, loss_real_d, real_correct, fake_correct;
  float loss_mse, loss_mge, loss_adv, loss_g;
  float gnorm_d, gnorm_g, tv;
};
__device__ __forceinline__ void publish_ticket(unsigned* ticket, unsigned value) {
  if (!ticket) return;
  __threadfence_system();
  __hip_atomic_store(ticket, value, __ATOMIC_RELEASE, __HIP_MEMORY_SCOPE_SYSTEM);
}

__device__ __forceinline__ double mask_total_body(const float* __restrict__ mask, int n, double* sh ) {
  float p[8];
#pragma unroll
  for (int u = 0; u < 8; ++u) p[u] = 0.f;
  const int bd = blockDim.x;
  int i = threadIdx.x;
  if ((reinterpret_cast<uintptr_t>(mask) & 15) == 0) {
    const f32x4* m4 = reinterpret_cast<const f32x4*>(mask);
    const int n4 = n >> 2;
    int j = threadIdx.x;
    for (; j + 7 * bd < n4; j += 8 * bd) {
      f32x4 v[8];
#pragma unroll
      for (int u = 0; u < 8; ++u) v[u] = m4[j + u * bd];
#pragma unroll
      for (int u = 0; u < 8; ++u) p[u] += (v[u][0] + v[u][1]) + (v[u][2] + v[u][3]);
// ... 256 lines not shown
        float v[8];
#pragma unroll
        for (int q = 0; q < 8; ++q) {
          const long row = (long)t0 * nW + tw0 + q * nwv;
          const float x = band[min(row, src_rows - 1) * nb + jc];
          v[q] = (j_ok && row < src_rows) ? x : 0.f;
        }
#pragma unroll
        for (int q = 0; q < 8; ++q) {
          const int tw = tw0 + q * nwv;
          if (tw < nrow) sb[tw * nbp + jp] = v[q];
        }
      }
    }
  }
  __syncthreads();
  static_assert(FPL >= 1 && FPL <= MLPG_PAD + 1, "the band rows are padded for at most MLPG_PAD + 1 frames per lane");
  if (threadIdx.x >= TT * 32 / FPL) return;
  const int cp = threadIdx.x & 31, fg = threadIdx.x >> 5;
  const int tl0 = fg * FPL;
  float acc[FPL][2];
#pragma unroll
  for (int i = 0; i < FPL; ++i) acc[i][0] = acc[i][1] = 0.f;
  const int ntap = (FPL - 1) + nb;
  for (int w = 0; w < nW; ++w) {
    const float* dcol = sm + (tl0 * nW + w) * MLPG_CC + 2 * cp;
    const float* cf = sb + (tl0 * nW + w) * nbp + MLPG_PAD;
#pragma unroll 8
    for (int j0 = 0; j0 < ntap; ++j0) {
      const float2 d = *reinterpret_cast<const float2*>(dcol + j0 * nW * MLPG_CC);
#pragma unroll
      for (int i = 0; i < FPL; ++i) {
        const float cfi = cf[i * nW * nbp + j0 - i];
        acc[i][0] = fmaf(cfi, d.x, acc[i][0]);
        acc[i][1] = fmaf(cfi, d.y, acc[i][1]);
      }
    }
  }
#pragma unroll
  for (int q = 0; q < 2; ++q) {
    const int c = 2 * cp + q;
    if (c >= nc) continue;
    const bool pass = sstride[c0 + c] == 0;
#pragma unroll
    for (int i = 0; i < FPL; ++i) {
      const int t = t0 + tl0 + i;
      if (t >= T) continue;
      const float out = pass ? sm[((tl0 + i + kb) * nW + 0) * MLPG_CC + c] : acc[i][q];
      ys[((long)b * T + t) * ldys + c0 + c] = out;
    }
  }
}

template <int FPL, int TT = MLPG_TT>
__global__ __launch_bounds__(MLPG_THREADS) __attribute__((amdgpu_waves_per_eu(FPL <= 2 ? 8 : 4)))
void mlpg_backward_kernel(
    const float* __restrict__ gs, int ldgs, const float* __restrict__ band, int kb, int nW,
    const int* __restrict__ scol, const int* __restrict__ sstride, int Ds,
    float* __restrict__ gy, int ldgy, int B, int T,
    float mse_w, const float* __restrict__ yhat, const float* __restrict__ ytgt, int ldt,
    const float* __restrict__ mask, const StepScalars* __restrict__ sc) {
  extern __shared__ __attribute__((aligned(16))) float sm[];
  const int nb = 2 * kb + 1, nbp = nb + 2 * MLPG_PAD;
  const int tiles_t = (T + TT - 1) / TT;
  const int b = blockIdx.x / tiles_t, t0 = (blockIdx.x % tiles_t) * TT;
  const int c0 = blockIdx.y * MLPG_CC;
  const int nc = min(MLPG_CC, Ds - c0);
  const int rows = TT + 2 * kb;
  float* sb = sm + rows * MLPG_CC;
  const float* gb = gs + (long)b * T * ldgs;
  const int lane = threadIdx.x & 63, wv = threadIdx.x >> 6, nwv = MLPG_THREADS / 64;
  float vb0[16];
  {
    const long src_rows = (long)T * nW, base = (long)(t0 - kb) * nW;
    const int jc = min(max(lane - MLPG_PAD, 0), nb - 1);
#pragma unroll
    for (int q = 0; q < 16; ++q) vb0[q] = band[min(max(base + wv + q * nwv, 0L), src_rows - 1) * nb + jc];
  }
  {
    const bool c_ok = lane < nc;
    const int ccl = c_ok ? c0 + lane : c0;
    for (int r0 = wv; r0 < rows; r0 += 8 * nwv) {
      float v[8];
#pragma unroll
      for (int q = 0; q < 8; ++q) {
        const int t = t0 - kb + r0 + q * nwv;
        const int tc = min(max(t, 0), T - 1);
        const float x = gb[(long)tc * ldgs + ccl];
        v[q] = (c_ok && t >= 0 && t < T) ? x : 0.f;
      }
#pragma unroll
      for (int q = 0; q < 8; ++q) {
        const int r = r0 + q * nwv;
        if (r < rows) sm[r * MLPG_CC + lane] = v[q];
      }
    }
  }
  {
    const int nrow = rows * nW;
    const long src_rows = (long)T * nW, base = (long)(t0 - kb) * nW;
    if (lane < nbp) {
      const int j = lane - MLPG_PAD;
      const bool j_ok = j >= 0 && j < nb;
#pragma unroll
      for (int q = 0; q < 16; ++q) {
        const int rw = wv + q * nwv;
        const long row = base + rw;
        if (rw < nrow) sb[rw * nbp + lane] = (j_ok && row >= 0 && row < src_rows) ? vb0[q] : 0.f;
      }
    }
    for (int jp = lane; jp < nbp; jp += 64) {
      const int j = jp - MLPG_PAD;
      const bool j_ok = j >= 0 && j < nb;
      const int jc = min(max(j, 0), nb - 1);
      for (int rw0 = jp == lane ? wv + 16 * nwv : wv; rw0 < nrow; rw0 += 8 * nwv) {
        float v[8];
#pragma unroll
        for (int q = 0; q < 8; ++q) {
          const long row = base + rw0 + q * nwv;
          const float x = band[min(max(row, 0L), src_rows - 1) * nb + jc];
          v[q] = (j_ok && row >= 0 && row < src_rows) ? x : 0.f;
        }
#pragma unroll
        for (int q = 0; q < 8; ++q) {
          const int rw = rw0 + q * nwv;
          if (rw < nrow) sb[rw * nbp + jp] = v[q];
        }
      }
    }
  }
  __syncthreads();
  static_assert(FPL >= 1 && FPL <= MLPG_PAD + 1, "the band rows are padded for at most MLPG_PAD + 1 frames per lane");
  if (threadIdx.x >= TT * 32 / FPL) return;
  const int cp = threadIdx.x & 31, fg = threadIdx.x >> 5;
  const int tl0 = fg * FPL;
  float acc[MLPG_MAXW][FPL][2];
#pragma unroll
  for (int w = 0; w < MLPG_MAXW; ++w)
#pragma unroll
    for (int i = 0; i < FPL; ++i) acc[w][i][0] = acc[w][i][1] = 0.f;
  const int ntap = (FPL - 1) + nb;
  const float* drow = sm + tl0 * MLPG_CC + 2 * cp;
  const float* cfrow = sb + (long)tl0 * nW * nbp + MLPG_PAD + (nb - 1);
#pragma unroll 4
  for (int j0 = 0; j0 < ntap; ++j0) {
    const float2 d = *reinterpret_cast<const float2*>(drow + j0 * MLPG_CC);
    const float* cf = cfrow + (long)j0 * nW * nbp - j0;
#pragma unroll
    for (int w = 0; w < MLPG_MAXW; ++w) {
      if (w >= nW) break;
#pragma unroll
      for (int i = 0; i < FPL; ++i) {
        const float cfi = cf[w * nbp + i];
        acc[w][i][0] = fmaf(cfi, d.x, acc[w][i][0]);
        acc[w][i][1] = fmaf(cfi, d.y, acc[w][i][1]);
      }
    }
  }
  const float msk_scale = mse_w != 0.f ? 2.f * mse_w * sc->inv_tv : 0.f;
#pragma unroll
  for (int q = 0; q < 2; ++q) {
    const int c = 2 * cp + q;
    if (c >= nc) continue;
    const int col0 = scol[c0 + c], st = sstride[c0 + c];
#pragma unroll
    for (int i = 0; i < FPL; ++i) {
      const int tp = t0 + tl0 + i;
      if (tp >= T) continue;
      const long row = (long)b * T + tp;
      const float m = msk_scale != 0.f ? mask[row] : 0.f;
#pragma unroll
      for (int w = 0; w < MLPG_MAXW; ++w) {
        if (w >= nW || (st == 0 && w > 0)) break;
        float out = st == 0 ? sm[(tl0 + i + kb) * MLPG_CC + c] : acc[w][i][q];
        const int col = col0 + w * st;
        if (msk_scale != 0.f) out += msk_scale * (yhat[row * ldt + col] * m - ytgt[row * ldt + col] * m) * m;
        gy[row * ldgy + col] = out;
      }
    }
  }
}

__device__ __forceinline__ double masked_sqerr_body(
    const float* __restrict__ a, int lda, const float* __restrict__ b, int ldb,
    const float* __restrict__ mask, long rows, int D, float* __restrict__ g, int ldg, float gs, int blk, int nblk) {
  double acc = 0.0;
  const long total = rows * D;
  const long stride = (long)nblk * blockDim.x;
  const long sr = stride / D;
  const int sd = (int)(stride - sr * D);
  long e = (long)blk * blockDim.x + threadIdx.x;
  long r = e / D;
  int d = (int)(e - r * D);
  for (; e < total; e += 4 * stride) {
    long rr[4];
    int dd[4];
    bool ok[4];
#pragma unroll
    for (int u = 0; u < 4; ++u) {
      rr[u] = r; dd[u] = d; ok[u] = e + u * stride < total;
      r += sr; d += sd;
      if (d >= D) { d -= D; ++r; }
    }
    float m[4], av[4], bv[4];
#pragma unroll
    for (int u = 0; u < 4; ++u) {
      m[u] = ok[u] ? mask[rr[u]] : 0.f; av[u] = ok[u] ? a[rr[u] * lda + dd[u]] : 0.f; bv[u] = ok[u] ? b[rr[u] * ldb + dd[u]] : 0.f;
    }
#pragma unroll
    for (int u = 0; u < 4; ++u) {
      if (!ok[u]) continue;
      const float diff = av[u] * m[u] - bv[u] * m[u];
      acc += (double)diff * (double)diff;
      if (g) g[rr[u] * ldg + dd[u]] = gs * diff * m[u];
    }
  }
  return acc;
}
static __global__ __launch_bounds__(RED_THREADS) void masked_sqerr_kernel(
    const float* __restrict__ a, int lda, const float* __restrict__ b, int ldb,
    const float* __restrict__ mask, long rows, int D, double* __restrict__ partial,
    float* __restrict__ g, int ldg, float gscale, const StepScalars* __restrict__ sc) {
  __shared__ double sh[16];
  const float gs = g ? 2.f * gscale * sc->inv_tv : 0.f;
  const double acc = masked_sqerr_body(a, lda, b, ldb, mask, rows, D, g, ldg, gs, blockIdx.x, gridDim.x);
  const double tot = block_sum_d(acc, sh);
  if (threadIdx.x == 0) partial[blockIdx.x] = tot;
}
static __global__ __launch_bounds__(RED_THREADS) void g_losses_kernel(
    const float* __restrict__ a1, int lda1, const float* __restrict__ b1, int ldb1, int D1, int n1, double* __restrict__ partial1,
    const float* __restrict__ a2, int lda2, const float* __restrict__ b2, int ldb2, int D2, double* __restrict__ partial2,
    const float* __restrict__ mask, long rows) {
  __shared__ double sh[16];
// ... 203 lines not shown
  __shared__ float shw[1024];
  __shared__ double shd[16];
  const int nparts = (int)blockDim.x / cgw;
  const int kl = threadIdx.x % cgw, part = threadIdx.x / cgw;
  const int k = blockIdx.x * cgw + kl;
  if (dw) {
    float sa[16];
#pragma unroll
    for (int u = 0; u < 16; ++u) sa[u] = 0.f;
    if (k < K) {
      int i = part;
      for (; i + 15 * nparts < nblk; i += 16 * nparts) {
#pragma unroll
        for (int u = 0; u < 16; ++u) sa[u] += dw_partial[(long)(i + nparts * u) * K + k];
      }
      for (; i < nblk; i += nparts) sa[0] += dw_partial[(long)i * K + k];
    }
#pragma unroll
    for (int u = 0; u < 8; ++u) sa[u] += sa[u + 8];
#pragma unroll
    for (int u = 0; u < 4; ++u) sa[u] += sa[u + 4];
    shw[part * cgw + kl] = (sa[0] + sa[1]) + (sa[2] + sa[3]);
    __syncthreads();
    if (part == 0 && k < K) {
      float tot = 0.f;
      for (int q = 0; q < nparts; ++q) tot += shw[q * cgw + kl];
      dw[k] = accumulate ? dw[k] + tot : tot;
    }
  }
  if ((int)blockIdx.x == scal_blk) {
    double v[5] = {0, 0, 0, 0, 0};
    for (int i = threadIdx.x; i < nblk; i += blockDim.x) {
      v[0] += hp[i].s_real; v[1] += hp[i].s_fake; v[2] += hp[i].n_real_ok; v[3] += hp[i].n_fake_ok; v[4] += hp[i].db;
    }
    double r[5];
    for (int q = 0; q < 5; ++q) r[q] = block_sum_d(v[q], shd);
    if (threadIdx.x == 0) {
      if (mode == HEAD_D_STEP) {
        sc->s_real = r[0]; sc->s_fake = r[1]; sc->n_real_ok = r[2]; sc->n_fake_ok = r[3];
        if (early_res) {
          const float T = sc->tv;
          const float lr = -((float)r[0]) / T, lf = -((float)r[1]) / T;
          early_res->loss_real_d = lr; early_res->loss_fake_d = lf; early_res->loss_d = lr + lf;
          early_res->real_correct = (float)r[2]; early_res->fake_correct = (float)r[3];
          early_res->gnorm_d = 0.f; early_res->tv = T;
          publish_ticket(ticket, ticket_value);
        }
      } else sc->s_adv = r[0];
      if (db) db[0] = accumulate ? db[0] + (float)r[4] : (float)r[4];
    }
  }
}


struct GFinalize {
  int on;
  StepScalars* sc;
  StepResults* out;
  float adv_w, mse_w, mge_w;
  int has_adv;
  const double* part_mge; int n_mge;
  const double* part_mse; int n_mse;
  const HeadPartials* hp; int n_hp;
  unsigned* ticket; unsigned ticket_value;
};
__device__ __forceinline__ void finalize_g_body(StepScalars* sc, StepResults* out, float adv_w, float mse_w, float mge_w, int has_adv,
                                                int zero_gnorm, const double* __restrict__ part_mge, int n_mge,
                                                const double* __restrict__ part_mse, int n_mse,
                                                const HeadPartials* __restrict__ hp, int n_hp, double* shp ,
                                                unsigned* ticket = nullptr, unsigned ticket_value = 0) {
  if (part_mge || part_mse || hp) {
    if (part_mge) {
      double v = 0.0;
      for (int i = threadIdx.x; i < n_mge; i += blockDim.x) v += __builtin_nontemporal_load(part_mge + i);
      const double t = block_sum_d(v, shp);
      if (threadIdx.x == 0) sc->s_mge = t;
    }
    if (part_mse) {
      double v = 0.0;
      for (int i = threadIdx.x; i < n_mse; i += blockDim.x) v += __builtin_nontemporal_load(part_mse + i);
      const double t = block_sum_d(v, shp);
      if (threadIdx.x == 0) sc->s_mse = t;
    }
    if (hp) {
      double v = 0.0;
      for (int i = threadIdx.x; i < n_hp; i += blockDim.x) v += hp[i].s_real;
      const double t = block_sum_d(v, shp);
      if (threadIdx.x == 0) sc->s_adv = t;
    }
    __syncthreads();
  }
  if (threadIdx.x || !out) return;
  const float T = sc->tv;
  const float mse = (float)sc->s_mse / T, mge = (float)sc->s_mge / T;
  const float adv = has_adv ? -((float)sc->s_adv) / T : 0.f;
  out->loss_mse = mse; out->loss_mge = mge; out->loss_adv = adv;
  out->loss_g = (mse_w * mse + mge_w * mge) + adv_w * adv;
  out->gnorm_g = zero_gnorm ? 0.f : (float)sqrt(sc->gnorm2_g); out->tv = T;
  publish_ticket(ticket, ticket_value);
}

static __global__ __launch_bounds__(RED_THREADS) void static_grad_kernel(
    const float* __restrict__ yhs, int ld1, const float* __restrict__ ys, int ld2,
    const float* __restrict__ mask, long rows, int Ds, float mge_w,
    const int* __restrict__ adv_inv , const float* __restrict__ leak, int ldl,
    const float* __restrict__ gadv, int lda, float adv_w,
    float* __restrict__ gs, int ldg, double* __restrict__ partial, StepScalars* __restrict__ sc, const GFinalize fin,
    int leak_unnorm ) {
  __shared__ double sh[16];
  int nblk = gridDim.x;
  const int blk = blockIdx.x;
  if (fin.on) {
    if (blockIdx.x == gridDim.x - 1) {
      finalize_g_body(fin.sc, fin.out, fin.adv_w, fin.mse_w, fin.mge_w, fin.has_adv, 1, fin.part_mge, fin.n_mge, fin.part_mse, fin.n_mse,
                      fin.hp, fin.n_hp, sh, fin.ticket, fin.ticket_value);
      return;
    }
    --nblk;
  }
  double acc = 0.0;
  const long total = rows * Ds;
  const float sc2 = 2.f * mge_w * sc->inv_tv;
  const float leak_s = leak_unnorm ? sc->inv_tv : 1.f;
  const long stride = (long)nblk * blockDim.x;
  const long sr = stride / Ds;
  const int sd = (int)(stride - sr * Ds);
  long e = (long)blk * blockDim.x + threadIdx.x;
  long r = e / Ds;
  int c = (int)(e - r * Ds);
  for (; e + 3 * stride < total; e += 4 * stride) {
    long rr[4];
    int cc[4];
#pragma unroll
    for (int u = 0; u < 4; ++u) {
      if (c >= Ds) { c -= Ds; ++r; }
      rr[u] = r; cc[u] = c;
      r += sr; c += sd;
    }
    float m[4], yv[4], tv[4], lk[4], ga[4];
    int jj[4];
#pragma unroll
    for (int u = 0; u < 4; ++u) {
      m[u] = mask[rr[u]]; yv[u] = yhs[rr[u] * ld1 + cc[u]]; tv[u] = ys[rr[u] * ld2 + cc[u]];
      jj[u] = (gs && adv_inv) ? adv_inv[cc[u]] : -1;
    }
#pragma unroll
    for (int u = 0; u < 4; ++u) {
      lk[u] = (jj[u] >= 0 && leak) ? leak[rr[u] * ldl + jj[u]] : 0.f;
      ga[u] = (jj[u] >= 0 && gadv) ? gadv[rr[u] * lda + jj[u]] : 0.f;
    }
#pragma unroll
    for (int u = 0; u < 4; ++u) {
      const float diff = yv[u] * m[u] - tv[u] * m[u];
      if (partial) acc += (double)diff * (double)diff;
      if (gs) {
        float v = sc2 * diff * m[u];
        if (jj[u] >= 0) {
          if (leak) v += leak_s * lk[u];
          if (gadv) v += adv_w * ga[u];
        }
        gs[rr[u] * ldg + cc[u]] = v;
      }
    }
  }
  for (; e < total; e += stride, r += sr, c += sd) {
    if (c >= Ds) { c -= Ds; ++r; }
    const float m = mask[r];
    const float diff = yhs[r * ld1 + c] * m - ys[r * ld2 + c] * m;
    if (partial) acc += (double)diff * (double)diff;
    if (gs) {
      float v = sc2 * diff * m;
      const int j = adv_inv ? adv_inv[c] : -1;
      if (j >= 0) {
        if (leak) v += leak_s * leak[r * ldl + j];
        if (gadv) v += adv_w * gadv[r * lda + j];
      }
      gs[r * ldg + c] = v;
    }
  }
  if (partial) {
    const double tot = block_sum_d(acc, sh);
    if (threadIdx.x == 0) partial[blk] = tot;
  }
}

static __global__ __launch_bounds__(RED_THREADS) void finalize_g_rider_kernel(const GFinalize fin) {
  __shared__ double sh[16];
  finalize_g_body(fin.sc, fin.out, fin.adv_w, fin.mse_w, fin.mge_w, fin.has_adv, 1, fin.part_mge, fin.n_mge, fin.part_mse, fin.n_mse,
                  fin.hp, fin.n_hp, sh, fin.ticket, fin.ticket_value);
}

static __global__ void scale_by_inv_tv_kernel(float* __restrict__ g, long n, const StepScalars* __restrict__ sc) {
  const long i = (long)blockIdx.x * blockDim.x + threadIdx.x;
  if (i < n) g[i] *= sc->inv_tv;
}

static __global__ __launch_bounds__(256) void sum_partials_kernel(const double* __restrict__ partial, int n, double* __restrict__ out) {
  __shared__ double sh[16];
  double v = 0.0;
  for (int i = threadIdx.x; i < n; i += blockDim.x) v += partial[i];
  const double tot = block_sum_d(v, sh);
  if (threadIdx.x == 0) *out = tot;
}

static __global__ __launch_bounds__(256) void colsum_partial_kernel(const float* __restrict__ X, int ldx, long rows, int cols,
                                                             int rows_per_blk, float* __restrict__ partial) {
  __shared__ float sh[4][64];
  const int cl = threadIdx.x & 63, rl = threadIdx.x >> 6;
  const int c = blockIdx.y * 64 + cl;
  const long r0 = (long)blockIdx.x * rows_per_blk;
  const long r1 = min(rows, r0 + rows_per_blk);
  float s = 0.f;
  if (c < cols) for (long r = r0 + rl; r < r1; r += 4) s += X[r * ldx + c];
  sh[rl][cl] = s;
  __syncthreads();
  if (rl == 0 && c < cols) partial[(long)blockIdx.x * cols + c] = (sh[0][cl] + sh[1][cl]) + (sh[2][cl] + sh[3][cl]);
}
static __global__ void colsum_finalize_kernel(const float* __restrict__ partial, int nblk, int cols, float* __restrict__ out, int accumulate) {
  const int c = blockIdx.x * blockDim.x + threadIdx.x;
  if (c >= cols) return;
  float s = 0.f;
  for (int i = 0; i < nblk; ++i) s += partial[(long)i * cols + c];
  out[c] = accumulate ? out[c] + s : s;
}

__device__ __forceinline__ void slab_reduce4_body(int blk, const float* __restrict__ slabs, long slab_stride, int nslab, long n4,
                                                  float* __restrict__ out, int accumulate,
                                                  const float* __restrict__ bslabs, int nb, float* __restrict__ bout, int main_blocks) {
  if (blk >= main_blocks) {
    const int c = (blk - main_blocks) * blockDim.x + threadIdx.x;
    if (c >= nb) return;
    float s0 = 0.f, s1 = 0.f, s2 = 0.f, s3 = 0.f;
    int k = 0;
    for (; k + 4 <= nslab; k += 4) {
      s0 += bslabs[(long)k * nb + c];       s1 += bslabs[(long)(k + 1) * nb + c];
      s2 += bslabs[(long)(k + 2) * nb + c]; s3 += bslabs[(long)(k + 3) * nb + c];
    }
    for (; k < nslab; ++k) s0 += bslabs[(long)k * nb + c];
    const float tot = (s0 + s1) + (s2 + s3);
    bout[c] = accumulate ? bout[c] + tot : tot;
    return;
  }
// ... 440 lines not shown
```

gantts_amd/csrc/gemm_f32.hip.h:

```cpp
#pragma once
#include <hip/hip_runtime.h>
#include <stdint.h>
#include <type_traits>

namespace gt {

typedef float f32x16 __attribute__((ext_vector_type(16)));
typedef float f32x4 __attribute__((ext_vector_type(4)));
typedef __bf16 bf16x8 __attribute__((ext_vector_type(8)));
typedef __bf16 bf16x4 __attribute__((ext_vector_type(4)));

struct __attribute__((packed, aligned(4))) F4U { float v[4]; };
__device__ __forceinline__ f32x4 ld4u(const float* p) {
  const F4U t = *reinterpret_cast<const F4U*>(p);
  f32x4 r; r[0] = t.v[0]; r[1] = t.v[1]; r[2] = t.v[2]; r[3] = t.v[3];
  return r;
}
__device__ __forceinline__ void st4u(float* p, const f32x4& r) {
  F4U t; t.v[0] = r[0]; t.v[1] = r[1]; t.v[2] = r[2]; t.v[3] = r[3];
  *reinterpret_cast<F4U*>(p) = t;
}

enum GemmPrec { PREC_F32 = 0, PREC_BF16 = 1 };
constexpr int GEMM_KP = 40;
// ... 672 lines not shown
#pragma unroll
    for (int i = 0; i < TM; ++i)
#pragma unroll
      for (int j = 0; j < TN_; ++j)
#pragma unroll
        for (int r = 0; r < 16; ++r) v += acc[i][j][r];
    g.C[(long)(m0 + wm * WM + l31) * g.ldc + n0 + wn * WN + half] = v;
    return;
  }
#endif
  if constexpr (KIND == GEMM_NT && AMODE == GEMM_A_LEAKY_PHILOX_SEG) {
    const int nh = g.dual_rows > 0 ? 2 : 1;
    f32x16 acc0[TM][TN_];
    if (nh > 1) {
#pragma unroll
      for (int i = 0; i < TM; ++i)
#pragma unroll
        for (int j = 0; j < TN_; ++j) acc0[i][j] = acc[i][j];
    }
    for (int h = 0; h < nh; ++h) {
      if (h > 0) {
        __syncthreads();
#pragma unroll
        for (int i = 0; i < TM; ++i)
#pragma unroll
          for (int j = 0; j < TN_; ++j) acc[i][j] = acc0[i][j];
      }
#pragma unroll
      for (int u = 0; u < UA; ++u) {
        int kk, mm; a_pos(u, kk, mm);
        offA[u] = (uint32_t)min(m0 + mm, mclamp) * (uint32_t)g.lda_seg + (uint32_t)kk;
      }
      pA = g.A_seg + (long)h * g.dual_rows * g.lda_seg;
      pB = g.B_seg;
      k_begin = 0; k_end = g.K_seg;
      nk = (k_end + GEMM_BK - 1) / GEMM_BK;
      has_tail = (k_end % GEMM_BK) != 0;
      gemm_kloop_prio(true);
      prologue();
      k_loop();
      gemm_kloop_prio(false);
      gemm_store_tile<KIND, BM, BN, PREC, BKT, AMODE>(g, slab, m0 + h * g.dual_rows, n0, acc, smem, nh > 1 ? (h + 1) * g.dual_rows : g.M);
    }
    return;
  }
  gemm_store_tile<KIND, BM, BN, PREC, BKT, AMODE>(g, slab, m0, n0, acc, smem, g.M);
}

__device__ __forceinline__ int gemm_xcd_order(int bid, int nwg) {
  const int q = nwg >> 3, r = nwg & 7, xcd = bid & 7, idx = bid >> 3;
  return (xcd < r ? xcd * (q + 1) : r * (q + 1) + (xcd - r) * q) + idx;
}

template <int PREC, int AMODE = GEMM_A_RUNTIME>
__global__ __launch_bounds__(GEMM_THREADS, 4) void gemm_pair_kernel(const GemmArgs g1, const GemmArgs g2, const int n1, const int tn_first) {
  extern __shared__ __attribute__((aligned(16))) float smem[];
  int bid = blockIdx.x;
  const int n2 = (int)gridDim.x - n1;
  const bool is_nn = tn_first ? bid >= n2 : bid < n1;
  if (is_nn) {
    bid = gemm_xcd_order(tn_first ? bid - n2 : bid, n1);
    const int tile_m = bid / g1.n_tiles_n, tile_n = bid - tile_m * g1.n_tiles_n;
    gemm_tile<GEMM_NN, 64, 64, true, true, PREC, 32, AMODE>(g1, 0, tile_m, tile_n, smem);
  } else {
    bid = gemm_xcd_order(tn_first ? bid : bid - n1, n2);
    const int tiles_mn = g2.n_tiles_m * g2.n_tiles_n;
    const int slab = bid / tiles_mn, t = bid - slab * tiles_mn;
    const int tile_m = t / g2.n_tiles_n, tile_n = t - tile_m * g2.n_tiles_n;
    gemm_tile<GEMM_TN, 64, 64, true, true, PREC>(g2, slab, tile_m, tile_n, smem);
  }
}

template <int PREC>
__global__ __launch_bounds__(GEMM_THREADS, 4) void gemm_tn_pair_kernel(const GemmArgs g1, const GemmArgs g2, const int n1, const GemmArgs g3, const int n3) {
  extern __shared__ __attribute__((aligned(16))) float smem[];
  int bid = blockIdx.x;
  if (bid >= (int)gridDim.x - n3) {
    bid -= (int)gridDim.x - n3;
    gemm_tile<GEMM_NN, 64, 64, true, false, PREC, 32, GEMM_A_NONE>(g3, 0, bid / g3.n_tiles_n, bid % g3.n_tiles_n, smem);
    return;
  }
  const int n2 = (int)gridDim.x - n3 - n1;
  if (bid >= n2) {
    bid = gemm_xcd_order(bid - n2, n1);
    const int tiles_mn = g1.n_tiles_m * g1.n_tiles_n;
    const int slab = bid / tiles_mn, t = bid - slab * tiles_mn;
    gemm_tile<GEMM_TN, 64, 64, true, true, PREC, 32, GEMM_A_TN_SUM2>(g1, slab, t / g1.n_tiles_n, t % g1.n_tiles_n, smem);
  } else {
    bid = gemm_xcd_order(bid, n2);
    const int tiles_mn = g2.n_tiles_m * g2.n_tiles_n;
    const int slab = bid / tiles_mn, t = bid - slab * tiles_mn;
    gemm_tile<GEMM_TN, 64, 64, true, true, PREC>(g2, slab, t / g2.n_tiles_n, t % g2.n_tiles_n, smem);
  }
}

#ifndef GT_SEG_WGS
#define GT_SEG_WGS 4
#endif
template <int BM, int BN, int AMODE> constexpr int gemm_min_wgs() { return (BM == 64 && BN == 64 && AMODE == GEMM_A_LEAKY_PHILOX_SEG) ? GT_SEG_WGS : 2; }
template <int KIND, int BM, int BN, bool VA, bool VB, int PREC = PREC_F32, int BKT = 32, int AMODE = GEMM_A_RUNTIME>
__global__ __launch_bounds__(GEMM_THREADS, (gemm_min_wgs<BM, BN, AMODE>())) void gemm_f32_kernel(const GemmArgs g) {
  extern __shared__ __attribute__((aligned(16))) float smem[];
  const int bid = gemm_xcd_order(blockIdx.x, gridDim.x);
  const int tiles_mn = g.n_tiles_m * g.n_tiles_n;
  const int slab = bid / tiles_mn;
  const int t = bid - slab * tiles_mn;
  const int tile_m = t / g.n_tiles_n, tile_n = t - tile_m * g.n_tiles_n;
  gemm_tile<KIND, BM, BN, VA, VB, PREC, BKT, AMODE>(g, slab, tile_m, tile_n, smem);
}

}
```

gantts_amd/csrc/gemm_f32_launch.hip.h:

```cpp
#pragma once
#include "engine_internal.hip.h"

static double gemm_algorithmic_bytes(int kind, const GemmArgs& g) {
  double b = 4.0 * ((double)g.M * g.K + (double)g.K * g.N + (double)g.M * g.N);
  if (kind == GEMM_NN && g.act != ACT_NONE && g.H) b += 4.0 * (double)g.M * g.N;
  return b;
}
template <int KIND, int BM, int BN, bool VA, bool VB, int PREC, int AM>
static int launch_gemm_impl(GemmArgs g, int nslab, hipStream_t s) {
  const size_t lds = gemm_lds_bytes<KIND, BM, BN, PREC>();
  CHK(ensure_dyn_lds((const void*)gemm_f32_kernel<KIND, BM, BN, VA, VB, PREC, 32, AM>, lds));
  g.n_tiles_m = cdiv(g.M, BM);
  g.n_tiles_n = cdiv(g.N, BN);
  const int grid = g.n_tiles_m * g.n_tiles_n * nslab;
  if (grid <= 0) return GT_OK;
  GemmProfiler::Rec rec;
  if (g_prof.wants(KIND)) {
    rec.kind = KIND; rec.bn = BN; rec.am = AM; rec.flops = 2.0 * g.M * g.N * g.K; rec.bytes = gemm_algorithmic_bytes(KIND, g);
    if (g.K_seg > 0) {
      const double halves = g.dual_rows > 0 ? 2.0 : 1.0;
      rec.flops += 2.0 * halves * g.M * g.N * g.K_seg;
      rec.bytes += 4.0 * (halves * g.M * g.K_seg + (double)g.K_seg * g.N + (halves - 1.0) * g.M * g.N);
    }
    rec.e0 = g_prof.get(); rec.e1 = g_prof.get();
    HIPCHK(hipEventRecord(rec.e0, s));
  }
  gemm_path_count(gemm_path_slot(KIND, BM, BN, VA, VB, PREC, AM));
  hipLaunchKernelGGL((gemm_f32_kernel<KIND, BM, BN, VA, VB, PREC, 32, AM>), dim3(grid), dim3(GEMM_THREADS), lds, s, g);
  LAUNCH_CHECK();
  if (g_prof.wants(KIND)) { HIPCHK(hipEventRecord(rec.e1, s)); g_prof.recs.push_back(rec); }
  return GT_OK;
}
template <int KIND, int BM, int BN, bool VA, bool VB, int PREC>
static int launch_gemm_t(const GemmArgs& g, int nslab, hipStream_t s) {
  if (g.K_seg > 0) {
    if constexpr (KIND == GEMM_NT && BM == 64 && BN == 64 && VA && VB && PREC == PREC_F32) {
      if (g.act == ACT_LEAKY_DROPOUT && g.drop.mode == DROP_PHILOX && g.addm == nullptr)
        return launch_gemm_impl<KIND, BM, BN, VA, VB, PREC, GEMM_A_LEAKY_PHILOX_SEG>(g, nslab, s);
    }
    return fail(GT_ERR_INVALID, "segmented forward product: float32, 64 x 64 tiles, 16-byte loadable operands, LeakyReLU + Philox only");
  }
  if constexpr (KIND != GEMM_TN && BM == 64 && BN == 64 && VA && VB && PREC == PREC_F32) {
    if (g.addm == nullptr) {
      if (g.act == ACT_NONE) return launch_gemm_impl<KIND, BM, BN, VA, VB, PREC, GEMM_A_NONE>(g, nslab, s);
      if (g.act == ACT_LEAKY_DROPOUT && g.drop.mode == DROP_PHILOX) return launch_gemm_impl<KIND, BM, BN, VA, VB, PREC, GEMM_A_LEAKY_PHILOX>(g, nslab, s);
    } else if constexpr (KIND == GEMM_NT) {
      if (g.act == ACT_LEAKY_DROPOUT && g.drop.mode == DROP_PHILOX) return launch_gemm_impl<KIND, BM, BN, VA, VB, PREC, GEMM_A_LEAKY_PHILOX_ADDM>(g, nslab, s);
    }
  }
  if constexpr (KIND == GEMM_TN) {
    if (g.A2 != nullptr) {
      if constexpr (BM == 64 && BN == 64 && VA && VB && PREC == PREC_F32) return launch_gemm_impl<KIND, BM, BN, VA, VB, PREC, GEMM_A_TN_SUM2>(g, nslab, s);
      else return fail(GT_ERR_INVALID, "weight gradient with a summed operand needs 64 x 64 tiles and 16-byte loadable operands");
    }
  } else if (g.A2 != nullptr) {
    return fail(GT_ERR_INVALID, "summed A operand: weight gradients only");
  }
  if (g.addm != nullptr && KIND != GEMM_NT) return fail(GT_ERR_INVALID, "added matrix: forward products only");
  return launch_gemm_impl<KIND, BM, BN, VA, VB, PREC, GEMM_A_RUNTIME>(g, nslab, s);
}
template <int KIND, int BM, int BN>
static int launch_gemm_v(const GemmArgs& g_in, int nslab, hipStream_t s) {
  GemmArgs g = g_in;
  g.wide_store = gemm_wide_store_ok(KIND, g) ? 1 : 0;
  const bool va = gemm_vec_ok(g.A, g.lda, KIND != GEMM_TN);
  const bool vb = gemm_vec_ok(g.B, g.ldb, KIND == GEMM_NT);
  if (tl_gemm_prec == PREC_BF16) {
    if (va && vb) return launch_gemm_t<KIND, BM, BN, true, true, PREC_BF16>(g, nslab, s);
    if (va) return launch_gemm_t<KIND, BM, BN, true, false, PREC_BF16>(g, nslab, s);
    if (vb) return launch_gemm_t<KIND, BM, BN, false, true, PREC_BF16>(g, nslab, s);
    return launch_gemm_t<KIND, BM, BN, false, false, PREC_BF16>(g, nslab, s);
  }
  if (va && vb) return launch_gemm_t<KIND, BM, BN, true, true, PREC_F32>(g, nslab, s);
  if (va) return launch_gemm_t<KIND, BM, BN, true, false, PREC_F32>(g, nslab, s);
  if (vb) return launch_gemm_t<KIND, BM, BN, false, true, PREC_F32>(g, nslab, s);
  return launch_gemm_t<KIND, BM, BN, false, false, PREC_F32>(g, nslab, s);
}
```

gantts_amd/engine.py:

```python
import ctypes as C
import weakref

import numpy as np
import torch

from . import _lib as L
from ._lib import check, lib, ptr


def stream_config_from_hp(hp):
    cfg = L.StreamConfig()
    ss = list(hp.stream_sizes)
    hd = list(hp.has_dynamic_features) if hp.has_dynamic_features is not None else [False] * len(ss)
    if len(ss) > L.MAX_STREAMS:
        raise ValueError("at most %d streams are supported" % L.MAX_STREAMS)
    cfg.n_streams = len(ss)
    for i, (s, d) in enumerate(zip(ss, hd)):
        cfg.stream_sizes[i] = int(s)
        cfg.has_dynamic_features[i] = int(bool(d))
    cfg.num_windows = len(hp.windows)
    adv = getattr(hp, "adversarial_streams", None)
    if adv is None:
        cfg.adversarial_streams[0] = -1
    else:
# ... 149 lines not shown

    def comm_trace_read(self):
        import numpy as np
        n = C.c_int()
        check(lib.gt_comm_trace_read(self._h, None, 0, C.byref(n)))
        out = np.zeros((max(n.value, 1), 5), dtype=np.float64)
        check(lib.gt_comm_trace_read(self._h, out.ctypes.data_as(C.POINTER(C.c_double)), n.value, C.byref(n)))
        return out[:n.value]

    def comm_info(self):
        r, w = C.c_int(), C.c_int()
        check(lib.gt_comm_info(self._h, C.byref(r), C.byref(w)))
        return r.value, w.value

    def check_faults(self):
        check(lib.gt_check_faults(self._h, L.current_stream()))

    def lstm_path_counts(self, reset=False):
        out = (C.c_int64 * L.LSTM_PATH_SLOTS)()
        check(lib.gt_lstm_path_counts(self._h, out, 1 if reset else 0))
        return list(out)

    def clear_faults(self):
        check(lib.gt_clear_faults(self._h, L.current_stream()))

    def invalidate_mlpg_cache(self):
        check(lib.gt_invalidate_mlpg_cache(self._h))

    def optimizer_step_count(self, role):
        n = C.c_int64()
        check(lib.gt_get_optimizer_step(self._h, role, C.byref(n)))
        return n.value

    def zero_grad(self, role):
        check(lib.gt_zero_grad(self._h, role))

    def set_seed(self, seed):
        check(lib.gt_set_seed(self._h, C.c_uint64(int(seed))))

    def philox_mask(self, role, pass_index, layer, p, rows, cols, steps_ahead=1):
        m = torch.empty(rows, cols, device="cuda", dtype=torch.float32)
        check(lib.gt_op_philox_mask(self._h, role, pass_index, layer, int(steps_ahead), float(p), int(rows), int(cols),
                                    ptr(m), L.current_stream()))
        return m

    def set_option(self, name, value):
        opts = {"lstm_persistent": L.OPT_LSTM_PERSISTENT,
                "lstm_fwd_units": L.OPT_LSTM_FWD_UNITS, "lstm_xcd_local": L.OPT_LSTM_XCD_LOCAL,
                "matmul_bf16": L.OPT_MATMUL_BF16, "split_first_layer": L.OPT_SPLIT_FIRST_LAYER,
                "fused_optimizer": L.OPT_FUSED_OPTIMIZER, "side_overlap": L.OPT_SIDE_OVERLAP, "lstm_side": L.OPT_LSTM_SIDE,
                "comm_d_one_msg": L.OPT_COMM_D_ONE_MSG, "comm_early_g": L.OPT_COMM_EARLY_G, "comm_group": L.OPT_COMM_GROUP,
                "comm_force": L.OPT_COMM_FORCE, "launch_riders": L.OPT_LAUNCH_RIDERS,
                "comm_close_inline": L.OPT_COMM_CLOSE_INLINE, "poll_results": L.OPT_POLL_RESULTS,
                "comm_tv_in_sums": L.OPT_COMM_TV_IN_SUMS, "comm_ipc": L.OPT_COMM_IPC, "fused_dstack": L.OPT_FUSED_DSTACK}
        if name not in opts:
            raise ValueError("unknown engine option %r" % (name,))
        check(lib.gt_set_option(self._h, opts[name], int(value)))
        if name == "matmul_bf16":
            self._opt_bf16 = bool(value)

    def set_loss_normalizer(self, tv):
        if isinstance(tv, torch.Tensor) and tv.is_cuda:
            if tv.dtype != torch.float64 or tv.numel() != 1:
                raise ValueError("device loss normaliser must be a 1-element float64 tensor")
            self._keep["tv"] = tv
            check(lib.gt_set_loss_normalizer_device(self._h, ptr(tv)))
        else:
            self._keep.pop("tv", None)
            check(lib.gt_set_loss_normalizer(self._h, float(tv)))

    def set_lengths(self, lengths, B, T):
        if lengths is None:
            vals = [T] * B
        elif isinstance(lengths, torch.Tensor):
            vals = [int(v) for v in lengths.detach().cpu().view(-1).tolist()]
        else:
            vals = [int(v) for v in lengths]
        if len(vals) != B:
            raise RuntimeError("lengths has %d entries for a batch of %d sequences" % (len(vals), B))
        arr = (C.c_int64 * B)(*vals)
        check(lib.gt_set_lengths(self._h, arr, B, L.current_stream()))

    def apply_generator(self, model_g, x, R, lengths=None):
        x, ld = _check_x(x, "x", model_g.in_dim)
        self._set_pitch(gx=ld)
        B, T, _ = x.shape
        model_g._check_masks(B, T)
        self.bind_model(L.ROLE_G, model_g, with_grads=True)
        if getattr(model_g, "needs_lengths", False):
            self.set_lengths(lengths, B, T)
        static_w = model_g.static_dim if model_g.include_parameter_generation() else self.static_dim
        y_hat = torch.empty(B, T, model_g.out_dim, device=x.device, dtype=torch.float32)
        y_hat_static = torch.empty(B, T, static_w, device=x.device, dtype=torch.float32)
        if R is not None:
            R = _check_frames(R, "R")
            if R.dim() != 2 or R.size(0) != T or R.size(1) != self.num_windows * T:
                raise RuntimeError("R must be (T, num_windows*T) = (%d, %d), got %s" % (T, self.num_windows * T, tuple(R.shape)))
        check(lib.gt_apply_generator(self._h, ptr(x), ptr(R), B, T, ptr(y_hat), ptr(y_hat_static), L.current_stream()))
        self._keep["g"] = (x, R, y_hat, y_hat_static)
        y_hat._gt_engine = y_hat_static._gt_engine = self
        return y_hat, y_hat_static

    def _set_pitch(self, gx=None, cx=None):
        if gx is not None:
            self._ld_gx = gx
        if cx is not None:
            self._ld_cx = cx
# ... 272 lines not shown
```

include/gantts_hip.h:

```cpp
#ifndef GANTTS_HIP_H_
#define GANTTS_HIP_H_

#include <stdint.h>

#ifdef __cplusplus
extern "C" {
#endif

#define GT_OK 0
#define GT_ERR_INVALID 1
#define GT_ERR_HIP 2
#define GT_ERR_STATE 3
#define GT_ERR_DIM 4

#define GT_ROLE_G 0
#define GT_ROLE_D 1

#define GT_ARCH_MLP 0
#define GT_ARCH_IN2OUT 1
#define GT_ARCH_LSTM 2
#define GT_ARCH_SRU 3
#define GT_ARCH_IN2OUT_RNN 4

#define GT_OPT_ADAGRAD 0
// ... 52 lines not shown

const char* gt_last_error(void);
const char* gt_version(void);
int gt_engine_create(const gt_stream_config* cfg, gt_engine** out);
void gt_engine_destroy(gt_engine* e);

int gt_bind_model(gt_engine* e, int role, const gt_model_desc* desc);
int gt_bind_optimizer(gt_engine* e, int role, const gt_optim_desc* desc);
int gt_set_training(gt_engine* e, int role, int training);
int gt_set_lr(gt_engine* e, int role, float lr);
int gt_get_optimizer_step(gt_engine* e, int role, int64_t* step);
int gt_set_seed(gt_engine* e, uint64_t seed);
int gt_set_dropout_mask(gt_engine* e, int role, int pass, int layer, const float* mask);
int gt_op_philox_mask(gt_engine* e, int role, int pass, int layer, int64_t steps_ahead, float p, int64_t rows, int cols,
                      float* mask, void* stream);

int gt_set_lengths(gt_engine* e, const int64_t* lengths_host, int B, void* stream);
int gt_invalidate_mlpg_cache(gt_engine* e);

int gt_zero_grad(gt_engine* e, int role);

int gt_apply_generator(gt_engine* e, const float* x, const float* R, int B, int T,
                       float* y_hat, float* y_hat_static, void* stream);

int gt_update_discriminator(gt_engine* e, const float* x, const float* y_static, const float* y_hat_static,
                            const float* mask, int B, int T, int train, float eps,
                            gt_d_result* out, void* stream);

int gt_update_generator(gt_engine* e, const float* x, const float* y, const float* y_hat,
                        const float* y_static, const float* y_hat_static, float adv_w,
                        const float* mask, int B, int T, int train, float mse_w, float mge_w, float eps,
                        gt_g_result* out, void* stream);

int gt_set_loss_normalizer(gt_engine* e, float tv_global);
int gt_set_loss_normalizer_device(gt_engine* e, const double* tv_global_dev);
#define GT_OPT_LSTM_PERSISTENT 2
#define GT_OPT_LSTM_FWD_UNITS 3
#define GT_OPT_LSTM_XCD_LOCAL 4
#define GT_OPT_MATMUL_BF16 5
#define GT_OPT_SPLIT_FIRST_LAYER 6
#define GT_OPT_FUSED_OPTIMIZER 7
#define GT_OPT_SIDE_OVERLAP 8
#define GT_OPT_LSTM_SIDE 9
#define GT_OPT_COMM_D_ONE_MSG 10
#define GT_OPT_COMM_EARLY_G 11
#define GT_OPT_COMM_GROUP 12
#define GT_OPT_COMM_FORCE 13
#define GT_OPT_LAUNCH_RIDERS 14
#define GT_OPT_COMM_CLOSE_INLINE 15
#define GT_OPT_POLL_RESULTS 16
#define GT_OPT_COMM_TV_IN_SUMS 17
#define GT_OPT_COMM_IPC 18
#define GT_OPT_FUSED_DSTACK 19
int gt_set_option(gt_engine* e, int option, int value);
int gt_set_tuning(const char* name, int value);
int gt_set_x_pitch(gt_engine* e, int ld_generator_input, int ld_condition);
int gt_check_faults(gt_engine* e, void* stream);
#define GT_LSTM_PATH_SLOTS 34
int gt_lstm_path_counts(gt_engine* e, int64_t* counts, int reset);
int gt_clear_faults(gt_engine* e, void* stream);
#define GT_COMM_ID_BYTES 128
int gt_comm_unique_id(void* id_out);
int gt_comm_init(gt_engine* e, int rank, int world, const void* id);
int gt_comm_destroy(gt_engine* e);
int gt_comm_info(gt_engine* e, int* rank, int* world);
int gt_comm_trace(gt_engine* e, int enable);
int gt_comm_trace_read(gt_engine* e, double* out, int max_records, int* n_records);
#define GT_IPC_HANDLE_BYTES 64
#define GT_IPC_MAX_WORLD 8
int gt_comm_ipc_export(gt_engine* e, void* handle_out);
int gt_comm_ipc_attach(gt_engine* e, int rank, int world, const void* handles);
int gt_comm_ipc_messages(gt_engine* e, long long* n);
int gt_set_shard(gt_engine* e, int rank, int world);

int gt_update_discriminator_begin(gt_engine* e, const float* x, const float* y_static, const float* y_hat_static,
                                  const float* mask, int B, int T, int train, float eps, void* stream);
int gt_update_discriminator_end(gt_engine* e, int train, gt_d_result* out, void* stream);
int gt_update_generator_begin(gt_engine* e, const float* x, const float* y, const float* y_hat,
                              const float* y_static, const float* y_hat_static, float adv_w,
                              const float* mask, int B, int T, int train, float mse_w, float mge_w, float eps,
                              void* stream);
int gt_update_generator_end(gt_engine* e, int train, float adv_w, float mse_w, float mge_w,
                            gt_g_result* out, void* stream);
int gt_update_discriminator_result(gt_engine* e, gt_d_result* out);
int gt_update_generator_result(gt_engine* e, gt_g_result* out);
int gt_scalar_buffer(gt_engine* e, double** dev_ptr, int* n_doubles);

int gt_model_forward(gt_engine* e, int role, const float* x, const float* R, int B, int T,
                     float* out, float* out2, void* stream);

int gt_flush_generator_grads(gt_engine* e, void* stream);

int gt_op_sequence_mask(const int64_t* lengths, int B, int T, float* mask, void* stream);
int gt_op_masked_mse(const float* input, const float* target, const float* mask, int B, int T, int D,
                     float* loss_out, float* grad_input, void* stream);
int gt_op_pad_sequences(const float* ragged, int D, const int64_t* start, const int64_t* len, int B, int T, float* out, int ld_out,
                        void* stream);
int gt_op_gather_cols(const float* in, int ld_in, const int32_t* idx, int n_idx, float* out, int ld_out,
                      int out_col_offset, int64_t rows, void* stream);
typedef struct gt_distortion_sums {
  double s_mcd;
  double s_bap;
  double s_f0;
  double n_voiced;
  double n_vuv_err;
  double s_mse;
// ... 64 lines not shown
```

Before: 12.80 million frames/s.

## Fold small tail kernels into neighbouring GEMM and MLPG launches

Introduces a deferred 'tail' descriptor that lets small follow-up kernels ride as extra workgroups inside an adjacent launch. The D head finalisation is appended to the next f32 pair-GEMM grid, the G loss reductions ride on the segmented leaky-Philox GEMM, and the static-gradient assembly plus the G finalisation are fused into the MLPG backward kernel, so the gs buffer is never materialised. The aim is to cut launch count and launch gaps in a launch-bound step. Because the riders are independent blocks inside the same grid, correctness depends on them not needing ordering against the GEMM tiles. Any tail that is not consumed is launched separately as a fallback.

```diff
diff --git a/gantts_amd/_lib.py b/gantts_amd/_lib.py
--- a/gantts_amd/_lib.py
+++ b/gantts_amd/_lib.py
@@ -11,9 +11,10 @@
 OPT_LSTM_PERSISTENT, OPT_LSTM_FWD_UNITS, OPT_LSTM_XCD_LOCAL, OPT_MATMUL_BF16, OPT_SPLIT_FIRST_LAYER, OPT_FUSED_OPTIMIZER = 2, 3, 4, 5, 6, 7
 OPT_SIDE_OVERLAP, OPT_LSTM_SIDE, OPT_COMM_D_ONE_MSG, OPT_COMM_EARLY_G, OPT_COMM_GROUP, OPT_COMM_FORCE = 8, 9, 10, 11, 12, 13
 OPT_LAUNCH_RIDERS, OPT_COMM_CLOSE_INLINE, OPT_POLL_RESULTS = 14, 15, 16
-OPT_COMM_TV_IN_SUMS, OPT_COMM_IPC, OPT_FUSED_DSTACK = 17, 18, 19
+OPT_COMM_TV_IN_SUMS, OPT_COMM_IPC, OPT_FUSED_DSTACK, OPT_TAIL_FOLD = 17, 18, 19, 20
 IPC_HANDLE_BYTES, IPC_MAX_WORLD = 64, 8
 PROFILE_SLOTS = 16
+PROFILE_TAIL_FOLD = 8
 LSTM_PATH_SLOTS, LSTM_PATH_STEPS, LSTM_PATH_DECLINED = 34, 32, 33
 GEMM_PATH_SLOTS = 588
 GEMM_ROUTE_FORWARD, GEMM_ROUTE_FORWARD_SEG, GEMM_ROUTE_BACKWARD_DATA, GEMM_ROUTE_WEIGHT_GRAD, GEMM_ROUTE_WEIGHT_GRAD_SPLIT = 0, 1, 2, 3, 4
diff --git a/gantts_amd/csrc/eng_core.hip b/gantts_amd/csrc/eng_core.hip
--- a/gantts_amd/csrc/eng_core.hip
+++ b/gantts_amd/csrc/eng_core.hip
@@ -54,6 +54,8 @@
     g_prof.pool.push_back(r.e0); g_prof.pool.push_back(r.e1);
   }
   g_prof.recs.clear();
+  if (g_prof.only_kind >= 8 && g_prof.only_kind <= 10) out_count[GT_PROFILE_SLOTS - 1] = g_prof.tail_fold_launches;
+  g_prof.tail_fold_launches = 0;
   return GT_OK;
 }
 extern "C" int gt_profile_bytes(double* out_bytes) {
@@ -357,6 +359,7 @@
     case GT_OPT_COMM_TV_IN_SUMS: e->opt_comm_tv_in_sums = value != 0; return GT_OK;
     case GT_OPT_POLL_RESULTS: e->opt_poll_results = value != 0; return GT_OK;
     case GT_OPT_LAUNCH_RIDERS: e->opt_launch_riders = value != 0; return GT_OK;
+    case GT_OPT_TAIL_FOLD: e->opt_tail_fold = value != 0; return GT_OK;
     case GT_OPT_MATMUL_BF16:
       if (e->matmul_bf16 != (value != 0)) {
         e->g_pass_valid = false; e->fake_cat_valid = false; e->dcat_b_ok = false; e->adv2_fake_ok = false; e->leak_pending = false; e->cxd_src = nullptr;
@@ -550,6 +553,7 @@
 int check_common(gt_engine* e, int B, int T) {
   if (!e) return fail(GT_ERR_INVALID, "null engine");
   tl_gemm_prec = e->matmul_bf16 ? PREC_BF16 : PREC_F32;
+  tl_gemm_tail.n = 0;
   if (B < 1 || T < 1) return fail(GT_ERR_INVALID, "B and T must be positive");
   if ((long)B * T > 0x3fffffffL) return fail(GT_ERR_INVALID, "B*T too large");
   e->chk_B = B; e->chk_T = T;
diff --git a/gantts_amd/csrc/eng_gemm_f32.hip b/gantts_amd/csrc/eng_gemm_f32.hip
--- a/gantts_amd/csrc/eng_gemm_f32.hip
+++ b/gantts_amd/csrc/eng_gemm_f32.hip
@@ -19,6 +19,7 @@
   return n;
 }
 thread_local int tl_gemm_prec = PREC_F32;
+thread_local GemmTail tl_gemm_tail = {};
 
 static std::atomic<int64_t> g_gemm_paths[GT_GEMM_PATH_SLOTS];
 void gemm_path_count(int slot) { g_gemm_paths[slot].fetch_add(1, std::memory_order_relaxed); }
diff --git a/gantts_amd/csrc/eng_gemm_f32_pair.hip b/gantts_amd/csrc/eng_gemm_f32_pair.hip
--- a/gantts_amd/csrc/eng_gemm_f32_pair.hip
+++ b/gantts_amd/csrc/eng_gemm_f32_pair.hip
@@ -22,12 +22,15 @@
     HIPCHK(hipEventRecord(rec.e0, s));
   }
   const int tn_first = gt_tuning().pair_order;
-  const int grid = n1 + n2;
+  GemmTail tail;
+  memset(&tail, 0, sizeof(tail));
+  if (!bf16 && tl_gemm_tail.n > 0 && tl_gemm_tail.kind == GEMM_TAIL_HEAD_FIN && lds >= (1024 + 32) * sizeof(float)) { tail = tl_gemm_tail; tl_gemm_tail.n = 0; tail_fold_count(1); }
+  const int grid = n1 + n2 + tail.n;
   gemm_path_count(GEMM_PATH_PAIR + (bf16 ? 3 : am == GEMM_A_NONE ? 0 : am == GEMM_A_LEAKY_PHILOX ? 1 : 2));
-  if (bf16) hipLaunchKernelGGL(gemm_pair_kernel<PREC_BF16>, dim3(grid), dim3(GEMM_THREADS), lds, s, nn, tn, n1, tn_first);
-  else if (am == GEMM_A_NONE) hipLaunchKernelGGL((gemm_pair_kernel<PREC_F32, GEMM_A_NONE>), dim3(grid), dim3(GEMM_THREADS), lds, s, nn, tn, n1, tn_first);
-  else if (am == GEMM_A_LEAKY_PHILOX) hipLaunchKernelGGL((gemm_pair_kernel<PREC_F32, GEMM_A_LEAKY_PHILOX>), dim3(grid), dim3(GEMM_THREADS), lds, s, nn, tn, n1, tn_first);
-  else      hipLaunchKernelGGL(gemm_pair_kernel<PREC_F32>, dim3(grid), dim3(GEMM_THREADS), lds, s, nn, tn, n1, tn_first);
+  if (bf16) hipLaunchKernelGGL(gemm_pair_kernel<PREC_BF16>, dim3(grid), dim3(GEMM_THREADS), lds, s, nn, tn, n1, tn_first, tail);
+  else if (am == GEMM_A_NONE) hipLaunchKernelGGL((gemm_pair_kernel<PREC_F32, GEMM_A_NONE>), dim3(grid), dim3(GEMM_THREADS), lds, s, nn, tn, n1, tn_first, tail);
+  else if (am == GEMM_A_LEAKY_PHILOX) hipLaunchKernelGGL((gemm_pair_kernel<PREC_F32, GEMM_A_LEAKY_PHILOX>), dim3(grid), dim3(GEMM_THREADS), lds, s, nn, tn, n1, tn_first, tail);
+  else      hipLaunchKernelGGL(gemm_pair_kernel<PREC_F32>, dim3(grid), dim3(GEMM_THREADS), lds, s, nn, tn, n1, tn_first, tail);
   LAUNCH_CHECK();
   if (g_prof.wants(5)) { HIPCHK(hipEventRecord(rec.e1, s)); g_prof.recs.push_back(rec); }
   return GT_OK;
diff --git a/gantts_amd/csrc/eng_step.hip b/gantts_amd/csrc/eng_step.hip
--- a/gantts_amd/csrc/eng_step.hip
+++ b/gantts_amd/csrc/eng_step.hip
@@ -88,6 +88,24 @@
   else { if (fpl == 1) GT_MLPG_BWD(1, 32) else if (fpl == 2) GT_MLPG_BWD(2, 32) else GT_MLPG_BWD(4, 32) }
 #undef GT_MLPG_BWD
   LAUNCH_CHECK();
+  return GT_OK;
+}
+static int mlpg_backward_fold(gt_engine* e, const GsAssemble& ga, const GFinalize& fin, const int* scol, const int* sstride, int Ds,
+                              float* gy, int ldgy, int B, int T, float mse_w, const float* yhat, const float* ytgt, int ldt, hipStream_t s) {
+  const int nW = e->cfg.num_windows, kb = e->mlpg.cur->kb;
+  const int tt = mlpg_tile_frames(e, B, T);
+  const size_t lds = ((size_t)(tt + 2 * kb) * MLPG_CC + (size_t)(tt + 2 * kb) * nW * (2 * kb + 1 + 2 * MLPG_PAD)) * sizeof(float);
+  if (lds < 16 * sizeof(double)) return fail(GT_ERR_STATE, "mlpg_backward_fold: the tile is smaller than the finalisation's workspace");
+  dim3 grid(B * cdiv(T, tt) + (fin.on ? 1 : 0), cdiv(Ds, MLPG_CC));
+  const int fpl = gt_tuning().mlpg_fpl;
+#define GT_MLPG_BWD(F, TTV) { CHK(ensure_dyn_lds((const void*)mlpg_backward_fold_kernel<F, TTV>, lds)); \
+    hipLaunchKernelGGL((mlpg_backward_fold_kernel<F, TTV>), grid, dim3(MLPG_THREADS), lds, s, ga, e->mlpg.cur->band.as<float>(), kb, nW, scol, sstride, Ds, \
+                       gy, ldgy, B, T, mse_w, yhat, ytgt, ldt, e->sc(), fin); }
+  if (tt == 16) GT_MLPG_BWD(2, 16)
+  else { if (fpl == 1) GT_MLPG_BWD(1, 32) else if (fpl == 2) GT_MLPG_BWD(2, 32) else GT_MLPG_BWD(4, 32) }
+#undef GT_MLPG_BWD
+  LAUNCH_CHECK();
+  tail_fold_count(0);
   return GT_OK;
 }
 
@@ -471,11 +489,37 @@
   return GT_OK;
 }
 
+#ifndef GT_TAIL_FOLD_PARTS
+#define GT_TAIL_FOLD_PARTS 7
+#endif
+static int run_tail_leftover(hipStream_t s) {
+  GemmTail& t = tl_gemm_tail;
+  if (t.n <= 0) return GT_OK;
+  if (t.kind == GEMM_TAIL_HEAD_FIN)
+    hipLaunchKernelGGL(d_head_finalize_kernel, dim3(t.n), dim3(1024), 0, s, t.hp, t.dw_partial, t.nblk, t.K, (int)HEAD_D_STEP, t.sc, t.dw, t.db,
+                       t.accumulate, t.early_res, t.ticket, t.ticket_value, t.cgw, t.scal_blk);
+  else
+    hipLaunchKernelGGL(g_losses_kernel, dim3(t.n), dim3(RED_THREADS), 0, s, t.a1, t.D1, t.b1, t.D1, t.D1, t.n1, t.partial1,
+                       t.a2, t.D2, t.b2, t.D2, t.D2, t.partial2, t.mask, t.rows);
+  t.n = 0;
+  LAUNCH_CHECK();
+  return GT_OK;
+}
 static int head_finalize(gt_engine* e, int mode, int nblk, int K, bool w, hipStream_t s, StepResults* early_res, int* defer_scalars, unsigned ticket) {
   Net& D = e->net[GT_ROLE_D];
   if (defer_scalars && !w) { *defer_scalars = nblk; return GT_OK; }
   const int cgw = (w && nblk >= 512) ? 16 : 64;
   const int n_dw = cdiv(K, cgw), extra = cgw == 16 ? 1 : 0;
+  if ((GT_TAIL_FOLD_PARTS & 2) && e->opt_tail_fold && e->early && !comm_on(e) && mode == HEAD_D_STEP && w && early_res && ticket &&
+      tl_gemm_prec == PREC_F32) {
+    GemmTail& t = tl_gemm_tail;
+    memset(&t, 0, sizeof(t));
+    t.kind = GEMM_TAIL_HEAD_FIN; t.n = n_dw + extra;
+    t.hp = e->headp.as<HeadPartials>(); t.dw_partial = e->headw.as<float>(); t.nblk = nblk; t.K = K; t.sc = e->sc();
+    t.dw = D.last.dW; t.db = D.last.db; t.accumulate = D.grads_dirty ? 1 : 0; t.early_res = early_res;
+    t.ticket = e->ticket_dev(); t.ticket_value = ticket; t.cgw = cgw; t.scal_blk = extra ? n_dw : 0;
+    return GT_OK;
+  }
   hipLaunchKernelGGL(d_head_finalize_kernel, dim3(n_dw + extra), dim3(1024), 0, s, e->headp.as<HeadPartials>(), e->headw.as<float>(),
                      nblk, K, mode, e->sc(), w ? D.last.dW : (float*)nullptr, w ? D.last.db : (float*)nullptr, D.grads_dirty ? 1 : 0,
                      early_res, ticket ? e->ticket_dev() : (unsigned*)nullptr, ticket, cgw, extra ? n_dw : 0);
@@ -858,6 +902,7 @@
     D.grads_dirty = true;
     if (want_leak) { e->leak_pending = true; e->leak_unnorm = unnorm; }
   }
+  CHK(run_tail_leftover(s));
   CHK(comm_finish_step(e, GT_ROLE_D, tr, &e->sc()->s_real, comm_early ? 0 : 4, s));
   e->d_begin_done = true;
   return GT_OK;
@@ -930,8 +975,9 @@
   return GT_OK;
 }
 
+struct TailFold { GsAssemble ga; GFinalize fin; };
 static int generator_backward(gt_engine* e, const float* x, const float* y, const float* y_hat, const float* mask,
-                              float mse_w, hipStream_t s) {
+                              float mse_w, hipStream_t s, const TailFold* fold = nullptr) {
   Net& G = e->net[GT_ROLE_G];
   const long N = e->N;
   const int B = e->B, T = e->T, Do = G.d.out_dim;
@@ -952,6 +998,9 @@
                                e->colp, s, &e->sdefer[GT_ROLE_G]));
     CHK(comm_grads_ready(e, GT_ROLE_G, G.gate.dW, (long)sd * sd + sd, s));
     CHK(mlpg_backward(e, e->dgx.as<float>(), sd, e->d_scol_i2o, e->d_sstride_i2o, sd, gy, ldgy, B, T, mse_w, y_hat, y, Do, mask, s));
+  } else if (e->g_used_mlpg && fold) {
+    CHK(mlpg_backward_fold(e, fold->ga, fold->fin, e->d_scol, e->d_sstride, e->Ds, gy, ldgy, B, T, mse_w, y_hat, y, Do, s));
+    CHK(post_early_results(e, s, fold->fin.ticket_value));
   } else if (e->g_used_mlpg) {
     CHK(mlpg_backward(e, gs, e->Ds, e->d_scol, e->d_sstride, e->Ds, gy, ldgy, B, T, mse_w, y_hat, y, Do, mask, s));
   } else {
@@ -1047,9 +1096,12 @@
     mse_blocks = (int)std::min<long>(1024, cdiv(N * Do, RED_THREADS * 4));
     mge_pre_blocks = (int)std::min<long>(1024, cdiv(N * Ds, RED_THREADS * 4));
     CHK(e->partial.ensure(4096 * sizeof(double)));
-    hipLaunchKernelGGL(g_losses_kernel, dim3(mse_blocks + mge_pre_blocks), dim3(RED_THREADS), 0, s, y_hat, Do, y, Do, Do, mse_blocks,
-                       e->partial.as<double>() + 1024, y_hat_static, Ds, y_static, Ds, Ds, e->partial.as<double>(), mask, N);
-    LAUNCH_CHECK();
+    GemmTail& t = tl_gemm_tail;
+    memset(&t, 0, sizeof(t));
+    t.kind = GEMM_TAIL_G_LOSSES; t.n = mse_blocks + mge_pre_blocks;
+    t.a1 = y_hat; t.b1 = y; t.D1 = Do; t.n1 = mse_blocks; t.partial1 = e->partial.as<double>() + 1024;
+    t.a2 = y_hat_static; t.b2 = y_static; t.D2 = Ds; t.partial2 = e->partial.as<double>(); t.mask = mask; t.rows = N;
+    if (!((GT_TAIL_FOLD_PARTS & 4) && riders && e->opt_tail_fold && adv_w > 0.f && tl_gemm_prec == PREC_F32)) CHK(run_tail_leftover(s));
   } else if (!(tr && direct && mse_w != 0.f)) {
     if (mse_side) CHK(side_fork(e, s));
     CHK(sum_sqerr(e, y_hat, Do, y, Do, mask, N, Do, &e->sc()->s_mse, nullptr, 0, 0.f, mse_side ? e->side : s, early_fold ? &mse_blocks : nullptr));
@@ -1147,17 +1199,21 @@
       }
     }
   }
+  CHK(run_tail_leftover(s));
   const bool early_ok = e->early && !(tr && direct && mse_w != 0.f);
   const bool early_now = early_ok && !comm_on(e), comm_early = early_ok && comm_on(e) && e->opt_comm_early_g;
   int mge_blocks = 0;
   e->early_done = false;
+  TailFold fold;
+  bool fold_on = false;
   {
     const int nblk = (int)std::min<long>(1024, cdiv(N * Ds, RED_THREADS * 4));
     CHK(e->partial.ensure(4096 * sizeof(double)));
     float* gs = nullptr;
-    if (tr) { CHK(e->gs.ensure((size_t)N * Ds * sizeof(float))); gs = e->gs.as<float>(); }
     const float* leak = (tr && e->leak_pending) ? e->leak.as<float>() : nullptr;
-    GFinalize fin;
+    fold_on = (GT_TAIL_FOLD_PARTS & 1) && tr && riders && e->opt_tail_fold && e->g_used_mlpg && !is_i2o(G.d.arch) && !(leak && e->leak_unnorm);
+    if (tr && !fold_on) { CHK(e->gs.ensure((size_t)N * Ds * sizeof(float))); gs = e->gs.as<float>(); }
+    GFinalize& fin = fold.fin;
     memset(&fin, 0, sizeof(fin));
     const bool rid = riders || riders_dp;
     if (rid) {
@@ -1168,6 +1224,11 @@
       fin.hp = head_blocks ? e->headp.as<HeadPartials>() : (const HeadPartials*)nullptr; fin.n_hp = head_blocks;
       if (riders) { fin.ticket_value = take_ticket(e); fin.ticket = fin.ticket_value ? e->ticket_dev() : (unsigned*)nullptr; }
     }
+    if (fold_on) {
+      GsAssemble& ga = fold.ga;
+      ga.yhs = y_hat_static; ga.ys = y_static; ga.ld1 = Ds; ga.ld2 = Ds; ga.mask = mask; ga.adv_inv = e->d_adv_inv;
+      ga.leak = leak; ga.ldl = e->Da; ga.gadv = gadv; ga.lda = e->Da; ga.mge_w = mge_w; ga.adv_w = adv_w;
+    } else
     if (tr || !rid)
       hipLaunchKernelGGL(static_grad_kernel, dim3(nblk + (rid ? 1 : 0)), dim3(RED_THREADS), 0, s, y_hat_static, Ds,
                          y_static, Ds, mask, N, Ds, mge_w, e->d_adv_inv, leak, e->Da, gadv, e->Da, adv_w, gs, Ds,
@@ -1176,7 +1237,8 @@
       hipLaunchKernelGGL(finalize_g_rider_kernel, dim3(1), dim3(RED_THREADS), 0, s, fin);
     LAUNCH_CHECK();
     mge_blocks = nblk;
-    if (riders) CHK(post_early_results(e, s, fin.ticket_value));
+    if (fold_on) {}
+    else if (riders) CHK(post_early_results(e, s, fin.ticket_value));
     else if (!early_now && !riders_dp) {
       hipLaunchKernelGGL(sum_partials_kernel, dim3(1), dim3(256), 0, s, e->partial.as<double>(), nblk, &e->sc()->s_mge);
       LAUNCH_CHECK();
@@ -1192,7 +1254,7 @@
   }
   if (comm_early) CHK(comm_early_results(e, GT_ROLE_G, &e->sc()->s_adv, 3, adv_w, mse_w, mge_w, s));
   if (tr) {
-    CHK(generator_backward(e, e->last_x, y, y_hat, mask, mse_w, s));
+    CHK(generator_backward(e, e->last_x, y, y_hat, mask, mse_w, s, fold_on ? &fold : nullptr));
     e->leak_pending = false; e->leak_unnorm = false;
   }
   CHK(comm_finish_step(e, GT_ROLE_G, tr, &e->sc()->s_adv, comm_early ? 0 : 3, s));
@@ -1254,6 +1316,7 @@
   if (!G.bound || !G.d.grads || !e->g_pass_valid) return fail(GT_ERR_STATE, "no generator pass to back-propagate");
   hipStream_t s = (hipStream_t)stream;
   tl_gemm_prec = e->matmul_bf16 ? PREC_BF16 : PREC_F32;
+  tl_gemm_tail.n = 0;
   CHK(fault_seen(e));
   { SlabDefer& sd = e->sdefer[GT_ROLE_G]; sd.active = false; sd.jobs.n = 0; sd.blocks = 0; sd.used = 0; }
   const long N = e->N;
diff --git a/gantts_amd/csrc/engine_internal.hip.h b/gantts_amd/csrc/engine_internal.hip.h
--- a/gantts_amd/csrc/engine_internal.hip.h
+++ b/gantts_amd/csrc/engine_internal.hip.h
@@ -71,12 +71,14 @@
   double last_bytes[GT_PROFILE_SLOTS] = {};
   std::vector<Rec> recs;
   std::vector<hipEvent_t> pool;
+  int64_t tail_fold_launches = 0;
   hipEvent_t get() {
     if (!pool.empty()) { hipEvent_t e = pool.back(); pool.pop_back(); return e; }
     hipEvent_t e; (void)hipEventCreate(&e); return e;
   }
 };
 extern GemmProfiler g_prof;
+inline void tail_fold_count(int part) { if (g_prof.on && g_prof.only_kind == 8 + part) ++g_prof.tail_fold_launches; }
 
 struct Scratch {
   void* p = nullptr;
@@ -230,6 +232,7 @@
   bool d_unnorm = false, leak_unnorm = false;
   bool opt_poll_results = env_flag("GT_POLL_RESULTS", true);
   bool opt_launch_riders = env_flag("GT_LAUNCH_RIDERS", true);
+  bool opt_tail_fold = env_flag("GT_TAIL_FOLD", true);
   int ld_gx = 0, ld_cx = 0;
   Scratch gx_dense, cx_dense;
   bool gx_dense_on = false;
@@ -265,6 +268,7 @@
 gt::DropoutSpec drop_spec(gt_engine* e, int role, int pass, int layer, const float* stacked_mask, int ld, long half_rows = 0);
 
 extern thread_local int tl_gemm_prec;
+extern thread_local gt::GemmTail tl_gemm_tail;
 enum { GEMM_PATH_PAIR = 576, GEMM_PATH_TN_PAIR = 580, GEMM_PATH_REDUCE4 = 582, GEMM_PATH_REDUCE = 583, GEMM_PATH_REDUCE_SMALL = 584,
        GEMM_PATH_COLSUM_PARTIAL = 585, GEMM_PATH_COLSUM_FINALIZE = 586, GEMM_PATH_REDUCE_MULTI = 587 };
 static_assert(GEMM_PATH_REDUCE_MULTI + 1 == GT_GEMM_PATH_SLOTS, "gt_gemm_path_counts slots");
diff --git a/gantts_amd/csrc/frame_kernels.hip.h b/gantts_amd/csrc/frame_kernels.hip.h
--- a/gantts_amd/csrc/frame_kernels.hip.h
+++ b/gantts_amd/csrc/frame_kernels.hip.h
@@ -35,6 +35,17 @@
   __syncthreads();
   double r = 0.0;
   if (threadIdx.x == 0) for (int i = 0; i < (int)(blockDim.x >> 6); ++i) r += sh[i];
+  return r;
+}
+
+__device__ __forceinline__ double block_sum_d_n(double v, double* sh, int nthr) {
+  v = wave_sum_d(v);
+  const int lane = threadIdx.x & 63, w = threadIdx.x >> 6;
+  __syncthreads();
+  if (lane == 0) sh[w] = v;
+  __syncthreads();
+  double r = 0.0;
+  if (threadIdx.x == 0) for (int i = 0; i < (nthr >> 6); ++i) r += sh[i];
   return r;
 }
 
@@ -397,6 +408,176 @@
   }
 }
 
+struct GsAssemble {
+  const float* yhs; const float* ys; int ld1, ld2;
+  const float* mask;
+  const int* adv_inv;
+  const float* leak; int ldl;
+  const float* gadv; int lda;
+  float mge_w, adv_w;
+};
+__device__ __forceinline__ float static_grad_value(float yv, float tv, float m, float sc2, bool adv_col, bool has_leak, float lk,
+                                                   bool has_gadv, float adv_w, float ga) {
+  const float diff = __fmaf_rn(yv, m, -__fmul_rn(tv, m));
+  float v = __fmul_rn(__fmul_rn(sc2, diff), m);
+  if (adv_col) {
+    if (has_leak) v = __fadd_rn(v, lk);
+    if (has_gadv) v = __fmaf_rn(adv_w, ga, v);
+  }
+  return v;
+}
+template <int FPL, int TT, bool FOLD>
+__device__ __forceinline__ void mlpg_backward_body(
+    const float* __restrict__ gs, int ldgs, const float* __restrict__ band, int kb, int nW,
+    const int* __restrict__ scol, const int* __restrict__ sstride, int Ds,
+    float* __restrict__ gy, int ldgy, int B, int T,
+    float mse_w, const float* __restrict__ yhat, const float* __restrict__ ytgt, int ldt,
+    const float* __restrict__ mask, const StepScalars* __restrict__ sc, const GsAssemble& ga, float* sm) {
+  const int nb = 2 * kb + 1, nbp = nb + 2 * MLPG_PAD;
+  const int tiles_t = (T + TT - 1) / TT;
+  const int b = blockIdx.x / tiles_t, t0 = (blockIdx.x % tiles_t) * TT;
+  const int c0 = blockIdx.y * MLPG_CC;
+  const int nc = min(MLPG_CC, Ds - c0);
+  const int rows = TT + 2 * kb;
+  float* sb = sm + rows * MLPG_CC;
+  const float* gb = FOLD ? nullptr : gs + (long)b * T * ldgs;
+  const int lane = threadIdx.x & 63, wv = threadIdx.x >> 6, nwv = MLPG_THREADS / 64;
+  float vb0[16];
+  {
+    const long src_rows = (long)T * nW, base = (long)(t0 - kb) * nW;
+    const int jc = min(max(lane - MLPG_PAD, 0), nb - 1);
+#pragma unroll
+    for (int q = 0; q < 16; ++q) vb0[q] = band[min(max(base + wv + q * nwv, 0L), src_rows - 1) * nb + jc];
+  }
+  if constexpr (FOLD) {
+    const bool c_ok = lane < nc;
+    const int ccl = c_ok ? c0 + lane : c0;
+    const int jj = ga.adv_inv ? ga.adv_inv[ccl] : -1;
+    const float sc2 = 2.f * ga.mge_w * sc->inv_tv;
+    const bool has_leak = ga.leak != nullptr, has_gadv = ga.gadv != nullptr;
+    const int jc = max(jj, 0);
+    const long nb0 = (long)b * T;
+    for (int r0 = wv; r0 < rows; r0 += 4 * nwv) {
+      float m[4], yv[4], tv[4], lk[4], gv[4];
+#pragma unroll
+      for (int q = 0; q < 4; ++q) {
+        const int t = t0 - kb + r0 + q * nwv;
+        const long row = nb0 + min(max(t, 0), T - 1);
+        m[q] = ga.mask[row]; yv[q] = ga.yhs[row * ga.ld1 + ccl]; tv[q] = ga.ys[row * ga.ld2 + ccl];
+        lk[q] = (jj >= 0 && has_leak) ? ga.leak[row * ga.ldl + jc] : 0.f;
+        gv[q] = (jj >= 0 && has_gadv) ? ga.gadv[row * ga.lda + jc] : 0.f;
+      }
+#pragma unroll
+      for (int q = 0; q < 4; ++q) {
+        const int r = r0 + q * nwv;
+        const int t = t0 - kb + r;
+        const float v = static_grad_value(yv[q], tv[q], m[q], sc2, jj >= 0, has_leak, lk[q], has_gadv, ga.adv_w, gv[q]);
+        if (r < rows) sm[r * MLPG_CC + lane] = (c_ok && t >= 0 && t < T) ? v : 0.f;
+      }
+    }
+  } else {
+    const bool c_ok = lane < nc;
+    const int ccl = c_ok ? c0 + lane : c0;
+    for (int r0 = wv; r0 < rows; r0 += 8 * nwv) {
+      float v[8];
+#pragma unroll
+      for (int q = 0; q < 8; ++q) {
+        const int t = t0 - kb + r0 + q * nwv;
+        const int tc = min(max(t, 0), T - 1);
+        const float x = gb[(long)tc * ldgs + ccl];
+        v[q] = (c_ok && t >= 0 && t < T) ? x : 0.f;
+      }
+#pragma unroll
+      for (int q = 0; q < 8; ++q) {
+        const int r = r0 + q * nwv;
+        if (r < rows) sm[r * MLPG_CC + lane] = v[q];
+      }
+    }
+  }
+  {
+    const int nrow = rows * nW;
+    const long src_rows = (long)T * nW, base = (long)(t0 - kb) * nW;
+    if (lane < nbp) {
+      const int j = lane - MLPG_PAD;
+      const bool j_ok = j >= 0 && j < nb;
+#pragma unroll
+      for (int q = 0; q < 16; ++q) {
+        const int rw = wv + q * nwv;
+        const long row = base + rw;
+        if (rw < nrow) sb[rw * nbp + lane] = (j_ok && row >= 0 && row < src_rows) ? vb0[q] : 0.f;
+      }
+    }
+    for (int jp = lane; jp < nbp; jp += 64) {
+      const int j = jp - MLPG_PAD;
+      const bool j_ok = j >= 0 && j < nb;
+      const int jc = min(max(j, 0), nb - 1);
+      for (int rw0 = jp == lane ? wv + 16 * nwv : wv; rw0 < nrow; rw0 += 8 * nwv) {
+        float v[8];
+#pragma unroll
+        for (int q = 0; q < 8; ++q) {
+          const long row = base + rw0 + q * nwv;
+          const float x = band[min(max(row, 0L), src_rows - 1) * nb + jc];
+          v[q] = (j_ok && row >= 0 && row < src_rows) ? x : 0.f;
+        }
+#pragma unroll
+        for (int q = 0; q < 8; ++q) {
+          const int rw = rw0 + q * nwv;
+          if (rw < nrow) sb[rw * nbp + jp] = v[q];
+        }
+      }
+    }
+  }
+  __syncthreads();
+  static_assert(FPL >= 1 && FPL <= MLPG_PAD + 1, "the band rows are padded for at most MLPG_PAD + 1 frames per lane");
+  if (threadIdx.x >= TT * 32 / FPL) return;
+  const int cp = threadIdx.x & 31, fg = threadIdx.x >> 5;
+  const int tl0 = fg * FPL;
+  float acc[MLPG_MAXW][FPL][2];
+#pragma unroll
+  for (int w = 0; w < MLPG_MAXW; ++w)
+#pragma unroll
+    for (int i = 0; i < FPL; ++i) acc[w][i][0] = acc[w][i][1] = 0.f;
+  const int ntap = (FPL - 1) + nb;
+  const float* drow = sm + tl0 * MLPG_CC + 2 * cp;
+  const float* cfrow = sb + (long)tl0 * nW * nbp + MLPG_PAD + (nb - 1);
+#pragma unroll 4
+  for (int j0 = 0; j0 < ntap; ++j0) {
+    const float2 d = *reinterpret_cast<const float2*>(drow + j0 * MLPG_CC);
+    const float* cf = cfrow + (long)j0 * nW * nbp - j0;
+#pragma unroll
+    for (int w = 0; w < MLPG_MAXW; ++w) {
+      if (w >= nW) break;
+#pragma unroll
+      for (int i = 0; i < FPL; ++i) {
+        const float cfi = cf[w * nbp + i];
+        acc[w][i][0] = fmaf(cfi, d.x, acc[w][i][0]);
+        acc[w][i][1] = fmaf(cfi, d.y, acc[w][i][1]);
+      }
+    }
+  }
+  const float msk_scale = mse_w != 0.f ? 2.f * mse_w * sc->inv_tv : 0.f;
+#pragma unroll
+  for (int q = 0; q < 2; ++q) {
+    const int c = 2 * cp + q;
+    if (c >= nc) continue;
+    const int col0 = scol[c0 + c], st = sstride[c0 + c];
+#pragma unroll
+    for (int i = 0; i < FPL; ++i) {
+      const int tp = t0 + tl0 + i;
+      if (tp >= T) continue;
+      const long row = (long)b * T + tp;
+      const float m = msk_scale != 0.f ? mask[row] : 0.f;
+#pragma unroll
+      for (int w = 0; w < MLPG_MAXW; ++w) {
+        if (w >= nW || (st == 0 && w > 0)) break;
+        float out = st == 0 ? sm[(tl0 + i + kb) * MLPG_CC + c] : acc[w][i][q];
+        const int col = col0 + w * st;
+        if (msk_scale != 0.f) out += msk_scale * (yhat[row * ldt + col] * m - ytgt[row * ldt + col] * m) * m;
+        gy[row * ldgy + col] = out;
+      }
+    }
+  }
+}
 template <int FPL, int TT = MLPG_TT>
 __global__ __launch_bounds__(MLPG_THREADS) __attribute__((amdgpu_waves_per_eu(FPL <= 2 ? 8 : 4)))
 void mlpg_backward_kernel(
@@ -406,124 +587,7 @@
     float mse_w, const float* __restrict__ yhat, const float* __restrict__ ytgt, int ldt,
     const float* __restrict__ mask, const StepScalars* __restrict__ sc) {
   extern __shared__ __attribute__((aligned(16))) float sm[];
-  const int nb = 2 * kb + 1, nbp = nb + 2 * MLPG_PAD;
-  const int tiles_t = (T + TT - 1) / TT;
-  const int b = blockIdx.x / tiles_t, t0 = (blockIdx.x % tiles_t) * TT;
-  const int c0 = blockIdx.y * MLPG_CC;
-  const int nc = min(MLPG_CC, Ds - c0);
-  const int rows = TT + 2 * kb;
-  float* sb = sm + rows * MLPG_CC;
-  const float* gb = gs + (long)b * T * ldgs;
-  const int lane = threadIdx.x & 63, wv = threadIdx.x >> 6, nwv = MLPG_THREADS / 64;
-  float vb0[16];
-  {
-    const long src_rows = (long)T * nW, base = (long)(t0 - kb) * nW;
-    const int jc = min(max(lane - MLPG_PAD, 0), nb - 1);
-#pragma unroll
-    for (int q = 0; q < 16; ++q) vb0[q] = band[min(max(base + wv + q * nwv, 0L), src_rows - 1) * nb + jc];
-  }
-  {
-    const bool c_ok = lane < nc;
-    const int ccl = c_ok ? c0 + lane : c0;
-    for (int r0 = wv; r0 < rows; r0 += 8 * nwv) {
-      float v[8];
-#pragma unroll
-      for (int q = 0; q < 8; ++q) {
-        const int t = t0 - kb + r0 + q * nwv;
-        const int tc = min(max(t, 0), T - 1);
-        const float x = gb[(long)tc * ldgs + ccl];
-        v[q] = (c_ok && t >= 0 && t < T) ? x : 0.f;
-      }
-#pragma unroll
-      for (int q = 0; q < 8; ++q) {
-        const int r = r0 + q * nwv;
-        if (r < rows) sm[r * MLPG_CC + lane] = v[q];
-      }
-    }
-  }
-  {
-    const int nrow = rows * nW;
-    const long src_rows = (long)T * nW, base = (long)(t0 - kb) * nW;
-    if (lane < nbp) {
-      const int j = lane - MLPG_PAD;
-      const bool j_ok = j >= 0 && j < nb;
-#pragma unroll
-      for (int q = 0; q < 16; ++q) {
-        const int rw = wv + q * nwv;
-        const long row = base + rw;
-        if (rw < nrow) sb[rw * nbp + lane] = (j_ok && row >= 0 && row < src_rows) ? vb0[q] : 0.f;
-      }
-    }
-    for (int jp = lane; jp < nbp; jp += 64) {
-      const int j = jp - MLPG_PAD;
-      const bool j_ok = j >= 0 && j < nb;
-      const int jc = min(max(j, 0), nb - 1);
-      for (int rw0 = jp == lane ? wv + 16 * nwv : wv; rw0 < nrow; rw0 += 8 * nwv) {
-        float v[8];
-#pragma unroll
-        for (int q = 0; q < 8; ++q) {
-          const long row = base + rw0 + q * nwv;
-          const float x = band[min(max(row, 0L), src_rows - 1) * nb + jc];
-          v[q] = (j_ok && row >= 0 && row < src_rows) ? x : 0.f;
-        }
-#pragma unroll
-        for (int q = 0; q < 8; ++q) {
-          const int rw = rw0 + q * nwv;
-          if (rw < nrow) sb[rw * nbp + jp] = v[q];
-        }
-      }
-    }
-  }
-  __syncthreads();
-  static_assert(FPL >= 1 && FPL <= MLPG_PAD + 1, "the band rows are padded for at most MLPG_PAD + 1 frames per lane");
-  if (threadIdx.x >= TT * 32 / FPL) return;
-  const int cp = threadIdx.x & 31, fg = threadIdx.x >> 5;
-  const int tl0 = fg * FPL;
-  float acc[MLPG_MAXW][FPL][2];
-#pragma unroll
-  for (int w = 0; w < MLPG_MAXW; ++w)
-#pragma unroll
-    for (int i = 0; i < FPL; ++i) acc[w][i][0] = acc[w][i][1] = 0.f;
-  const int ntap = (FPL - 1) + nb;
-  const float* drow = sm + tl0 * MLPG_CC + 2 * cp;
-  const float* cfrow = sb + (long)tl0 * nW * nbp + MLPG_PAD + (nb - 1);
-#pragma unroll 4
-  for (int j0 = 0; j0 < ntap; ++j0) {
-    const float2 d = *reinterpret_cast<const float2*>(drow + j0 * MLPG_CC);
-    const float* cf = cfrow + (long)j0 * nW * nbp - j0;
-#pragma unroll
-    for (int w = 0; w < MLPG_MAXW; ++w) {
-      if (w >= nW) break;
-#pragma unroll
-      for (int i = 0; i < FPL; ++i) {
-        const float cfi = cf[w * nbp + i];
-        acc[w][i][0] = fmaf(cfi, d.x, acc[w][i][0]);
-        acc[w][i][1] = fmaf(cfi, d.y, acc[w][i][1]);
-      }
-    }
-  }
-  const float msk_scale = mse_w != 0.f ? 2.f * mse_w * sc->inv_tv : 0.f;
-#pragma unroll
-  for (int q = 0; q < 2; ++q) {
-    const int c = 2 * cp + q;
-    if (c >= nc) continue;
-    const int col0 = scol[c0 + c], st = sstride[c0 + c];
-#pragma unroll
-    for (int i = 0; i < FPL; ++i) {
-      const int tp = t0 + tl0 + i;
-      if (tp >= T) continue;
-      const long row = (long)b * T + tp;
-      const float m = msk_scale != 0.f ? mask[row] : 0.f;
-#pragma unroll
-      for (int w = 0; w < MLPG_MAXW; ++w) {
-        if (w >= nW || (st == 0 && w > 0)) break;
-        float out = st == 0 ? sm[(tl0 + i + kb) * MLPG_CC + c] : acc[w][i][q];
-        const int col = col0 + w * st;
-        if (msk_scale != 0.f) out += msk_scale * (yhat[row * ldt + col] * m - ytgt[row * ldt + col] * m) * m;
-        gy[row * ldgy + col] = out;
-      }
-    }
-  }
+  mlpg_backward_body<FPL, TT, false>(gs, ldgs, band, kb, nW, scol, sstride, Ds, gy, ldgy, B, T, mse_w, yhat, ytgt, ldt, mask, sc, GsAssemble{}, sm);
 }
 
 __device__ __forceinline__ double masked_sqerr_body(
@@ -833,6 +897,92 @@
   }
 }
 
+__device__ __forceinline__ void head_finalize_tail(const GemmTail& a, int blk, float* smem) {
+  float* shw = smem;
+  double* shd = reinterpret_cast<double*>(smem + 1024);
+  const int cgw = a.cgw, nparts = 1024 / cgw, nblk = a.nblk, K = a.K;
+  {
+    for (int c = 0; c < 4; ++c) {
+      const int vt = c * 256 + (int)threadIdx.x;
+      const int kl = vt % cgw, part = vt / cgw;
+      const int k = blk * cgw + kl;
+      float sa[16];
+#pragma unroll
+      for (int u = 0; u < 16; ++u) sa[u] = 0.f;
+      if (k < K) {
+        int i = part;
+        for (; i + 15 * nparts < nblk; i += 16 * nparts) {
+#pragma unroll
+          for (int u = 0; u < 16; ++u) sa[u] += a.dw_partial[(long)(i + nparts * u) * K + k];
+        }
+        for (; i < nblk; i += nparts) sa[0] += a.dw_partial[(long)i * K + k];
+      }
+#pragma unroll
+      for (int u = 0; u < 8; ++u) sa[u] += sa[u + 8];
+#pragma unroll
+      for (int u = 0; u < 4; ++u) sa[u] += sa[u + 4];
+      shw[part * cgw + kl] = (sa[0] + sa[1]) + (sa[2] + sa[3]);
+    }
+    __syncthreads();
+    const int kl = (int)threadIdx.x, k = blk * cgw + kl;
+    if (kl < cgw && k < K) {
+      float tot = 0.f;
+      for (int q = 0; q < nparts; ++q) tot += shw[q * cgw + kl];
+      a.dw[k] = a.accumulate ? a.dw[k] + tot : tot;
+    }
+  }
+  if (blk != a.scal_blk) return;
+  double v[4][5];
+#pragma unroll
+  for (int c = 0; c < 4; ++c) {
+#pragma unroll
+    for (int q = 0; q < 5; ++q) v[c][q] = 0.0;
+    for (int i = c * 256 + (int)threadIdx.x; i < nblk; i += 1024) {
+      v[c][0] += a.hp[i].s_real; v[c][1] += a.hp[i].s_fake; v[c][2] += a.hp[i].n_real_ok; v[c][3] += a.hp[i].n_fake_ok; v[c][4] += a.hp[i].db;
+    }
+  }
+  const int lane = threadIdx.x & 63, w = threadIdx.x >> 6;
+  double r[5];
+#pragma unroll
+  for (int q = 0; q < 5; ++q) {
+    double ws[4];
+#pragma unroll
+    for (int c = 0; c < 4; ++c) ws[c] = wave_sum_d(v[c][q]);
+    __syncthreads();
+    if (lane == 0) {
+#pragma unroll
+      for (int c = 0; c < 4; ++c) shd[c * 4 + w] = ws[c];
+    }
+    __syncthreads();
+    double t = 0.0;
+    if (threadIdx.x == 0) for (int i = 0; i < 16; ++i) t += shd[i];
+    r[q] = t;
+  }
+  if (threadIdx.x == 0) {
+    StepScalars* sc = a.sc;
+    sc->s_real = r[0]; sc->s_fake = r[1]; sc->n_real_ok = r[2]; sc->n_fake_ok = r[3];
+    if (a.early_res) {
+      const float T = sc->tv;
+      const float lr = -((float)r[0]) / T, lf = -((float)r[1]) / T;
+      a.early_res->loss_real_d = lr; a.early_res->loss_fake_d = lf; a.early_res->loss_d = lr + lf;
+      a.early_res->real_correct = (float)r[2]; a.early_res->fake_correct = (float)r[3];
+      a.early_res->gnorm_d = 0.f; a.early_res->tv = T;
+      publish_ticket(a.ticket, a.ticket_value);
+    }
+    if (a.db) a.db[0] = a.accumulate ? a.db[0] + (float)r[4] : (float)r[4];
+  }
+}
+__device__ __forceinline__ void gemm_tail_run(const GemmTail& t, int blk, float* smem) {
+  if (t.kind == GEMM_TAIL_HEAD_FIN) { head_finalize_tail(t, blk, smem); return; }
+  double* sh = reinterpret_cast<double*>(smem);
+  const bool first = blk < t.n1;
+  const int b = first ? blk : blk - t.n1, nb = first ? t.n1 : t.n - t.n1;
+  const double acc = first ? masked_sqerr_body(t.a1, t.D1, t.b1, t.D1, t.mask, t.rows, t.D1, nullptr, 0, 0.f, b, nb)
+                           : masked_sqerr_body(t.a2, t.D2, t.b2, t.D2, t.mask, t.rows, t.D2, nullptr, 0, 0.f, b, nb);
+  const double tot = block_sum_d(acc, sh);
+  if (threadIdx.x == 0) (first ? t.partial1 : t.partial2)[b] = tot;
+}
+
 
 struct GFinalize {
   int on;
@@ -849,24 +999,26 @@
                                                 int zero_gnorm, const double* __restrict__ part_mge, int n_mge,
                                                 const double* __restrict__ part_mse, int n_mse,
                                                 const HeadPartials* __restrict__ hp, int n_hp, double* shp ,
-                                                unsigned* ticket = nullptr, unsigned ticket_value = 0) {
+                                                unsigned* ticket = nullptr, unsigned ticket_value = 0,
+                                                int nthr = 0 ) {
+  const int bd = nthr > 0 ? nthr : (int)blockDim.x;
   if (part_mge || part_mse || hp) {
     if (part_mge) {
       double v = 0.0;
-      for (int i = threadIdx.x; i < n_mge; i += blockDim.x) v += __builtin_nontemporal_load(part_mge + i);
-      const double t = block_sum_d(v, shp);
+      for (int i = threadIdx.x; i < n_mge; i += bd) v += __builtin_nontemporal_load(part_mge + i);
+      const double t = block_sum_d_n(v, shp, bd);
       if (threadIdx.x == 0) sc->s_mge = t;
     }
     if (part_mse) {
       double v = 0.0;
-      for (int i = threadIdx.x; i < n_mse; i += blockDim.x) v += __builtin_nontemporal_load(part_mse + i);
-      const double t = block_sum_d(v, shp);
+      for (int i = threadIdx.x; i < n_mse; i += bd) v += __builtin_nontemporal_load(part_mse + i);
+      const double t = block_sum_d_n(v, shp, bd);
       if (threadIdx.x == 0) sc->s_mse = t;
     }
     if (hp) {
       double v = 0.0;
-      for (int i = threadIdx.x; i < n_hp; i += blockDim.x) v += hp[i].s_real;
-      const double t = block_sum_d(v, shp);
+      for (int i = threadIdx.x; i < n_hp; i += bd) v += hp[i].s_real;
+      const double t = block_sum_d_n(v, shp, bd);
       if (threadIdx.x == 0) sc->s_adv = t;
     }
     __syncthreads();
@@ -969,6 +1121,24 @@
   __shared__ double sh[16];
   finalize_g_body(fin.sc, fin.out, fin.adv_w, fin.mse_w, fin.mge_w, fin.has_adv, 1, fin.part_mge, fin.n_mge, fin.part_mse, fin.n_mse,
                   fin.hp, fin.n_hp, sh, fin.ticket, fin.ticket_value);
+}
+
+template <int FPL, int TT = MLPG_TT>
+__global__ __launch_bounds__(MLPG_THREADS) __attribute__((amdgpu_waves_per_eu(FPL <= 2 ? 8 : 4)))
+void mlpg_backward_fold_kernel(
+    const GsAssemble ga, const float* __restrict__ band, int kb, int nW,
+    const int* __restrict__ scol, const int* __restrict__ sstride, int Ds,
+    float* __restrict__ gy, int ldgy, int B, int T,
+    float mse_w, const float* __restrict__ yhat, const float* __restrict__ ytgt, int ldt,
+    const StepScalars* __restrict__ sc, const GFinalize fin) {
+  extern __shared__ __attribute__((aligned(16))) float sm[];
+  if (fin.on && blockIdx.x == gridDim.x - 1) {
+    if (blockIdx.y == 0 && threadIdx.x < RED_THREADS)
+      finalize_g_body(fin.sc, fin.out, fin.adv_w, fin.mse_w, fin.mge_w, fin.has_adv, 1, fin.part_mge, fin.n_mge, fin.part_mse, fin.n_mse,
+                      fin.hp, fin.n_hp, reinterpret_cast<double*>(sm), fin.ticket, fin.ticket_value, RED_THREADS);
+    return;
+  }
+  mlpg_backward_body<FPL, TT, true>(nullptr, 0, band, kb, nW, scol, sstride, Ds, gy, ldgy, B, T, mse_w, yhat, ytgt, ldt, ga.mask, sc, ga, sm);
 }
 
 static __global__ void scale_by_inv_tv_kernel(float* __restrict__ g, long n, const StepScalars* __restrict__ sc) {
diff --git a/gantts_amd/csrc/gemm_f32.hip.h b/gantts_amd/csrc/gemm_f32.hip.h
--- a/gantts_amd/csrc/gemm_f32.hip.h
+++ b/gantts_amd/csrc/gemm_f32.hip.h
@@ -748,11 +748,31 @@
   return (xcd < r ? xcd * (q + 1) : r * (q + 1) + (xcd - r) * q) + idx;
 }
 
+struct StepScalars;
+struct StepResults;
+struct HeadPartials;
+enum { GEMM_TAIL_HEAD_FIN = 1, GEMM_TAIL_G_LOSSES = 2 };
+struct GemmTail {
+  int n;
+  int kind;
+  const HeadPartials* hp; const float* dw_partial; int nblk, K; StepScalars* sc; float* dw; float* db; int accumulate;
+  StepResults* early_res; unsigned* ticket; unsigned ticket_value; int cgw, scal_blk;
+  const float* a1; const float* b1; int D1, n1; double* partial1;
+  const float* a2; const float* b2; int D2; double* partial2;
+  const float* mask; long rows;
+};
+__device__ __forceinline__ void gemm_tail_run(const GemmTail& t, int blk, float* smem);
+
 template <int PREC, int AMODE = GEMM_A_RUNTIME>
-__global__ __launch_bounds__(GEMM_THREADS, 4) void gemm_pair_kernel(const GemmArgs g1, const GemmArgs g2, const int n1, const int tn_first) {
+__global__ __launch_bounds__(GEMM_THREADS, 4) void gemm_pair_kernel(const GemmArgs g1, const GemmArgs g2, const int n1, const int tn_first, const GemmTail tail) {
   extern __shared__ __attribute__((aligned(16))) float smem[];
   int bid = blockIdx.x;
-  const int n2 = (int)gridDim.x - n1;
+  int ntile = (int)gridDim.x;
+  if constexpr (PREC == PREC_F32) {
+    ntile -= tail.n;
+    if (bid >= ntile) { gemm_tail_run(tail, bid - ntile, smem); return; }
+  }
+  const int n2 = ntile - n1;
   const bool is_nn = tn_first ? bid >= n2 : bid < n1;
   if (is_nn) {
     bid = gemm_xcd_order(tn_first ? bid - n2 : bid, n1);
@@ -805,4 +825,14 @@
   gemm_tile<KIND, BM, BN, VA, VB, PREC, BKT, AMODE>(g, slab, tile_m, tile_n, smem);
 }
 
-}
+template <int PREC>
+__global__ __launch_bounds__(GEMM_THREADS, GT_SEG_WGS) void gemm_seg_tail_kernel(const GemmArgs g, const GemmTail tail) {
+  extern __shared__ __attribute__((aligned(16))) float smem[];
+  const int ntile = (int)gridDim.x - tail.n;
+  if ((int)blockIdx.x >= ntile) { gemm_tail_run(tail, (int)blockIdx.x - ntile, smem); return; }
+  const int bid = gemm_xcd_order(blockIdx.x, ntile);
+  const int tile_m = bid / g.n_tiles_n, tile_n = bid - tile_m * g.n_tiles_n;
+  gemm_tile<GEMM_NT, 64, 64, true, true, PREC, 32, GEMM_A_LEAKY_PHILOX_SEG>(g, 0, tile_m, tile_n, smem);
+}
+
+}
diff --git a/gantts_amd/csrc/gemm_f32_launch.hip.h b/gantts_amd/csrc/gemm_f32_launch.hip.h
--- a/gantts_amd/csrc/gemm_f32_launch.hip.h
+++ b/gantts_amd/csrc/gemm_f32_launch.hip.h
@@ -26,7 +26,18 @@
     HIPCHK(hipEventRecord(rec.e0, s));
   }
   gemm_path_count(gemm_path_slot(KIND, BM, BN, VA, VB, PREC, AM));
-  hipLaunchKernelGGL((gemm_f32_kernel<KIND, BM, BN, VA, VB, PREC, 32, AM>), dim3(grid), dim3(GEMM_THREADS), lds, s, g);
+  bool launched = false;
+  if constexpr (KIND == GEMM_NT && BM == 64 && BN == 64 && VA && VB && PREC == PREC_F32 && AM == GEMM_A_LEAKY_PHILOX_SEG) {
+    if (tl_gemm_tail.n > 0 && tl_gemm_tail.kind == GEMM_TAIL_G_LOSSES && nslab == 1 && lds >= 16 * sizeof(double)) {
+      const GemmTail tail = tl_gemm_tail;
+      tl_gemm_tail.n = 0;
+      CHK(ensure_dyn_lds((const void*)gemm_seg_tail_kernel<PREC>, lds));
+      hipLaunchKernelGGL((gemm_seg_tail_kernel<PREC>), dim3(grid + tail.n), dim3(GEMM_THREADS), lds, s, g, tail);
+      tail_fold_count(2);
+      launched = true;
+    }
+  }
+  if (!launched) hipLaunchKernelGGL((gemm_f32_kernel<KIND, BM, BN, VA, VB, PREC, 32, AM>), dim3(grid), dim3(GEMM_THREADS), lds, s, g);
   LAUNCH_CHECK();
   if (g_prof.wants(KIND)) { HIPCHK(hipEventRecord(rec.e1, s)); g_prof.recs.push_back(rec); }
   return GT_OK;
diff --git a/gantts_amd/engine.py b/gantts_amd/engine.py
--- a/gantts_amd/engine.py
+++ b/gantts_amd/engine.py
@@ -225,7 +225,8 @@
                 "comm_d_one_msg": L.OPT_COMM_D_ONE_MSG, "comm_early_g": L.OPT_COMM_EARLY_G, "comm_group": L.OPT_COMM_GROUP,
                 "comm_force": L.OPT_COMM_FORCE, "launch_riders": L.OPT_LAUNCH_RIDERS,
                 "comm_close_inline": L.OPT_COMM_CLOSE_INLINE, "poll_results": L.OPT_POLL_RESULTS,
-                "comm_tv_in_sums": L.OPT_COMM_TV_IN_SUMS, "comm_ipc": L.OPT_COMM_IPC, "fused_dstack": L.OPT_FUSED_DSTACK}
+                "comm_tv_in_sums": L.OPT_COMM_TV_IN_SUMS, "comm_ipc": L.OPT_COMM_IPC, "fused_dstack": L.OPT_FUSED_DSTACK,
+                "tail_fold": L.OPT_TAIL_FOLD}
         if name not in opts:
             raise ValueError("unknown engine option %r" % (name,))
         check(lib.gt_set_option(self._h, opts[name], int(value)))
diff --git a/include/gantts_hip.h b/include/gantts_hip.h
--- a/include/gantts_hip.h
+++ b/include/gantts_hip.h
@@ -128,6 +128,7 @@
 #define GT_OPT_COMM_TV_IN_SUMS 17
 #define GT_OPT_COMM_IPC 18
 #define GT_OPT_FUSED_DSTACK 19
+#define GT_OPT_TAIL_FOLD 20
 int gt_set_option(gt_engine* e, int option, int value);
 int gt_set_tuning(const char* name, int value);
 int gt_set_x_pitch(gt_engine* e, int ld_generator_input, int ld_condition);
```

Result: no change. 12.93 million frames/s, median of 6 (+1.0%).
